# jhoobergs/Thesis-pbrt-v3

Hardware: AMD Instinct MI355X
Metric: Mrays/s (higher is better)
Workload: dtype f32; 1 GPU; Sponza-class atrium STAND-IN (311,728 tris, matte+plastic, point light; the reference ships no Sponza geometry) 700x700, halton 1024 spp, path maxdepth 5, bvh; spp_total=1024, tiles=16x16 round-robin over 1 GPU(s), parallelism=tile-dp1, film_merge=none (single GPU)

## Files before the change

thesis-pbrt-v3_amd/csrc/capi_device.hip:

```cpp
#include <hip/hip_runtime.h>
#include <algorithm>
#include <cassert>
#include <chrono>
#include <cmath>
#include <cstring>
#include <functional>
#include <map>
#include <memory>
#include <string>
#include <vector>
#include "../../include/hprt.h"
#include "device/kernels.h"
#include "halton_tables.h"
#include "host_transform.h"
#include "hprt_internal.h"
#include "device_state.h"
#include "scene_layout.h"
#include "wide_bvh.h"

using namespace hprt;


namespace {

int CheckDevice(int device, int *chosen) {
    int n = 0;
    hipError_t e = hipGetDeviceCount(&n);
    if (e != hipSuccess || n <= 0) return SetError(HPRT_E_NO_DEVICE, "no HIP device available (hprt has no CPU fallback)");
    if (device < 0) { if (hipGetDevice(&device) != hipSuccess) device = 0; }
    if (device >= n) return SetError(HPRT_E_INVALID, "device ordinal out of range");
    if (hipSetDevice(device) != hipSuccess) return SetError(HPRT_E_DEVICE, "hipSetDevice failed");
    *chosen = device;
    return HPRT_OK;
}

struct PlaneAllocator {
    char *base; size_t off = 0, cap;
    template <typename T> T *take(size_t n) { off = (off + 255) & ~(size_t)255; T *p = (T *)(base + off); off += n * sizeof(T); return p; }
};
struct Workspace {
    PathStream path[2];
    HitStream hit;
    VertexStreams vs;
    float4 *Lfinal;
};
const size_t kPlaneBytesPerSlot = 16 * (2 * 4 + 1 + 2 + 2 + 1 + 3 + 1) + 1, kInstancePlaneBytesPerSlot = 8 + 8;
size_t PlaneBytesPerSlot(bool instances) { return kPlaneBytesPerSlot + (instances ? kInstancePlaneBytesPerSlot : 0); }
size_t PlaneBytes(size_t n, bool instances) { return n * PlaneBytesPerSlot(instances) + 32 * 256; }

void CarvePlanes(char *base, size_t n, bool instances, Workspace *w) {
    PlaneAllocator a{base, 0, 0};
    auto rays = [&](RayStream &r) { r.a = a.take<float4>(n); r.b = a.take<float4>(n); };
    for (int k = 0; k < 2; ++k) { rays(w->path[k].ray); w->path[k].beta = a.take<float4>(n); w->path[k].L = a.take<float4>(n); }
    w->hit.a = a.take<float4>(n); w->hit.b = instances ? a.take<float2>(n) : nullptr;
    rays(w->vs.shadow); w->vs.occluded = a.take<uint8_t>(n);
    rays(w->vs.mis); w->vs.misHit.a = a.take<float4>(n); w->vs.misHit.b = instances ? a.take<float2>(n) : nullptr;
    w->vs.pendLight = a.take<float4>(n); w->vs.pendMis = a.take<float4>(n); w->vs.pendBeta = a.take<float4>(n);
    w->Lfinal = a.take<float4>(n);
}

struct EventTimer {
    std::vector<hipEvent_t> pool; size_t used = 0;
    ~EventTimer() { for (hipEvent_t e : pool) (void)hipEventDestroy(e); }
    hipEvent_t get() {
        if (used == pool.size()) { hipEvent_t e; if (hipEventCreate(&e) != hipSuccess) return nullptr; pool.push_back(e); }
        return pool[used++];
    }
    void reset() { used = 0; }
};

void MakeCamera(const HprtRenderOptions &o, DevCamera *cam) {
    Xform camToScreen = xf_perspective(o.fov, 1e-2f, 1000.f);
    const float *sw = o.screen_window;
    Xform screenToRaster = xf_scale((float)o.xres, (float)o.yres, 1) * xf_scale(1 / (sw[1] - sw[0]), 1 / (sw[2] - sw[3]), 1) *
                           xf_translate(vec3(-sw[0], -sw[3], 0));
    Xform rasterToScreen = screenToRaster.inverse();
    Xform rasterToCamera = camToScreen.inverse() * rasterToScreen;
    cam->rasterToCamera = rasterToCamera.m;
    memcpy(cam->cameraToWorld.m, o.camera_to_world, 64);
    cam->lensRadius = o.lens_radius; cam->focalDistance = o.focal_distance;
    cam->dxCamera = xf_point(cam->rasterToCamera, vec3(1, 0, 0)) - xf_point(cam->rasterToCamera, vec3(0, 0, 0));
    cam->dyCamera = xf_point(cam->rasterToCamera, vec3(0, 1, 0)) - xf_point(cam->rasterToCamera, vec3(0, 0, 0));
}

int CheckDepth(int maxDepth) {
    if (5 + 8 * ((int64_t)maxDepth + 1) > 1000)
        return SetError(HPRT_E_UNSUPPORTED, "maxdepth above 123: a path could pass the 1,000 sampler dimensions of the reference's Halton tables");
    return HPRT_OK;
}

struct FrameSetup {
    FilmGeom fg; int ntx, nty; HaltonLayout hal; RenderParams rp;
    std::vector<uint32_t> pixelXY; std::vector<uint64_t> pixelOffset;
    std::vector<int32_t> localIndex;
    int W, H;
    uint64_t offX[128], offY[128];
};
int SetupFrame(const HprtRenderOptions &o, FrameSetup *f) {
    if (o.xres <= 0 || o.yres <= 0 || o.xres > 32768 || o.yres > 32768) return SetError(HPRT_E_INVALID, "film resolution out of range");
    if (o.filter_radius[0] != 0.5f || o.filter_radius[1] != 0.5f)
        return SetError(HPRT_E_UNSUPPORTED, "only the box filter with radius 0.5 is in the hot-path scope (SURVEY.md §2)");
    FilmGeom &fg = f->fg;
    fg.cx0 = (int)std::ceil(o.xres * o.crop[0]); fg.cx1 = (int)std::ceil(o.xres * o.crop[1]);
    fg.cy0 = (int)std::ceil(o.yres * o.crop[2]); fg.cy1 = (int)std::ceil(o.yres * o.crop[3]);
    fg.rx = o.filter_radius[0]; fg.ry = o.filter_radius[1];
    fg.sx0 = (int)std::floor((float)fg.cx0 + 0.5f - fg.rx); fg.sy0 = (int)std::floor((float)fg.cy0 + 0.5f - fg.ry);
    fg.sx1 = (int)std::ceil((float)fg.cx1 - 0.5f + fg.rx); fg.sy1 = (int)std::ceil((float)fg.cy1 - 0.5f + fg.ry);
    fg.maxSampleLuminance = o.max_sample_luminance;
    f->W = fg.cx1 - fg.cx0; f->H = fg.cy1 - fg.cy0;
    if (f->W <= 0 || f->H <= 0) return SetError(HPRT_E_INVALID, "empty crop window");
    f->ntx = (fg.sx1 - fg.sx0 + 15) / 16; f->nty = (fg.sy1 - fg.sy0 + 15) / 16;
    f->hal = MakeHaltonLayout(fg.sx1 - fg.sx0, fg.sy1 - fg.sy0);
    const uint64_t base = (uint64_t)HaltonPixelOffset(f->hal, 0, 0), stride = (uint64_t)std::max(1, f->hal.sampleStride);
    for (int m = 0; m < 128; ++m) {
        f->offX[m] = (uint64_t)HaltonPixelOffset(f->hal, m, 0);
        f->offY[m] = ((uint64_t)HaltonPixelOffset(f->hal, 0, m) + stride - base) % stride;
    }
    return HPRT_OK;
}
void AddTilePixels(FrameSetup *f, int tile) {
    const FilmGeom &fg = f->fg;
    int tx = tile % f->ntx, ty = tile / f->ntx;
    int x0 = fg.sx0 + tx * 16, x1 = std::min(x0 + 16, fg.sx1), y0 = fg.sy0 + ty * 16, y1 = std::min(y0 + 16, fg.sy1);
    const uint64_t stride = (uint64_t)std::max(1, f->hal.sampleStride);
    for (int y = y0; y < y1; ++y)
        for (int x = x0; x < x1; ++x) {
            f->localIndex[(size_t)(y - fg.cy0) * f->W + (x - fg.cx0)] = (int32_t)f->pixelXY.size();
            f->pixelXY.push_back((uint32_t)x | ((uint32_t)y << 16));
            f->pixelOffset.push_back(f->hal.sampleStride > 1 ? (f->offX[((x % 128) + 128) % 128] + f->offY[((y % 128) + 128) % 128]) % stride : 0ull);
        }
}

}

extern "C" {

int hprt_scene_create(const HprtSceneDesc *d, int device, HprtScene **out) try {
    if (!d || !out) return SetError(HPRT_E_INVALID, "hprt_scene_create: null argument");
    SceneLayout L;
    if (int rc = BuildSceneLayout(*d, &L)) return rc;
    int dev;
    if (int rc = CheckDevice(device, &dev)) return rc;
    std::unique_ptr<HprtScene> sc(new HprtScene());
    sc->device = dev; sc->nPrims = L.nPrims;
    sc->topOrder = std::move(L.topOrder); sc->objectOrder = std::move(L.objectOrder); sc->objectPrimBase = std::move(L.objectPrimBase);
    sc->instanceObject = std::move(L.instanceObject); sc->instanced = L.instanced; sc->hasSubstrateBin = L.hasSubstrateBin;
    const std::vector<uint16_t> &perms = HaltonPermutations();
    std::vector<int32_t> primes(PrimeTable().begin(), PrimeTable().end()), primeSums(PrimeSumTable().begin(), PrimeSumTable().end());
    std::vector<uint64_t> magic(primes.size());
    for (size_t i = 0; i < primes.size(); ++i) magic[i] = 0xffffffffffffffffull / (uint64_t)primes[i] + 1ull;
    HIP_TRY(upload(sc->nodes, L.pairs)); HIP_TRY(upload(sc->tris, L.tris)); HIP_TRY(upload(sc->primVtx, L.primVtx));
    HIP_TRY(upload(sc->primN, L.primN)); HIP_TRY(upload(sc->vUV, L.vUV)); HIP_TRY(upload(sc->vS, L.vS));
    HIP_TRY(upload(sc->shapes, L.shapes)); HIP_TRY(upload(sc->materials, L.materials)); HIP_TRY(upload(sc->lights, L.lights));
    HIP_TRY(upload(sc->spheres, L.spheres)); HIP_TRY(upload(sc->instances, L.instances)); HIP_TRY(upload(sc->topEntry, L.topEntry));
    HIP_TRY(upload(sc->topEntryWide, L.topEntryWide)); HIP_TRY(upload(sc->lightFunc, L.lightFunc)); HIP_TRY(upload(sc->lightCdf, L.lightCdf));
    HIP_TRY(upload(sc->perms, perms)); HIP_TRY(upload(sc->primes, primes)); HIP_TRY(upload(sc->primeSums, primeSums));
    HIP_TRY(upload(sc->primeMagic, magic));
    HIP_TRY(upload(sc->textures, L.textures)); HIP_TRY(upload(sc->mipLevels, L.mipLevels)); HIP_TRY(upload(sc->texels, L.texels)); HIP_TRY(upload(sc->weightLut, L.weightLut));
    HIP_TRY(upload(sc->wide, L.wide)); HIP_TRY(upload(sc->leafBox, L.leafBox));
    HIP_TRY(upload(sc->envLights, L.envLights)); HIP_TRY(upload(sc->envData, L.envData));
    HIP_TRY(sc->counters.alloc(sizeof(DevCounters)));
    HIP_TRY(hipMemset(sc->counters.p, 0, sizeof(DevCounters)));
    HIP_TRY(sc->deepStack.alloc((size_t)HPRT_SPILL_STACK * HPRT_DEEP_THREADS * sizeof(uint2)));
    HIP_TRY(sc->workCounter.alloc(256));
    DevScene &dv = sc->dev;
    dv.pairs = sc->nodes.as<DevPair>(); dv.nPairs = (uint32_t)L.pairs.size();
    dv.wide = L.wide.empty() ? nullptr : sc->wide.as<DevWide>(); dv.nWide = (uint32_t)L.wide.size(); dv.leafBox = sc->leafBox.as<float4>();
    dv.tris = sc->tris.as<float4>(); dv.nPrims = L.nPrims;
    dv.primVtx = sc->primVtx.as<uint32_t>();
    dv.primN = sc->primN.as<float4>(); dv.vUV = sc->vUV.as<float>(); dv.vS = sc->vS.as<float>();
    dv.shapes = sc->shapes.as<DevShape>(); dv.nShapes = d->n_shapes;
    dv.materials = sc->materials.as<DevMaterial>();
    dv.lights = sc->lights.as<DevLight>(); dv.nLights = d->n_lights;
    dv.spheres = sc->spheres.as<DevSphere>(); dv.nSpheres = (uint32_t)L.spheres.size();
    dv.envLights = sc->envLights.as<DevEnvLight>(); dv.envData = sc->envData.as<float>(); dv.nEnvLights = (uint32_t)L.envLights.size();
    dv.textures = d->n_textures ? sc->textures.as<DevTexture>() : nullptr; dv.mipLevels = sc->mipLevels.as<DevMipLevel>();
    dv.texels = sc->texels.as<float>(); dv.weightLut = sc->weightLut.as<float>();
    dv.instances = sc->instances.as<DevInstance>(); dv.nInstances = d->n_instances;
    dv.topEntry = L.topEntry.empty() ? nullptr : sc->topEntry.as<float4>(); dv.nTopPrims = (uint32_t)L.topEntry.size();
    dv.topEntryWide = L.topEntryWide.empty() ? nullptr : sc->topEntryWide.as<float4>();
    dv.lightFunc = sc->lightFunc.as<float>(); dv.lightCdf = sc->lightCdf.as<float>(); dv.lightFuncInt = L.funcInt;
    dv.deepStack = sc->deepStack.as<uint2>();
    dv.perms = sc->perms.as<uint16_t>(); dv.primes = sc->primes.as<int32_t>(); dv.primeSums = sc->primeSums.as<int32_t>();
    dv.primeMagic = sc->primeMagic.as<uint64_t>();
    dv.worldRadius = L.worldRadius;
    dv.spatial = 0; dv.voxFunc = dv.voxCdf = dv.voxFuncInt = nullptr;
    dv.voxSlot = nullptr; dv.voxRequest = nullptr; dv.voxRequestCount = nullptr;
    for (int a = 0; a < 3; ++a) { dv.voxN[a] = L.voxN[a]; dv.wbMin[a] = L.wbMin[a]; dv.wbMax[a] = L.wbMax[a]; }
    if (L.lightStrategy == 2) {
        const uint64_t nVox = (uint64_t)dv.voxN[0] * (uint64_t)dv.voxN[1] * (uint64_t)dv.voxN[2];
        const uint64_t denseMaxFloats = [] { const char *e = getenv("HPRT_VOXEL_DENSE_MAX_MB"); return e ? (uint64_t)atoll(e) * (1ull << 18) : (1ull << 28); }();
        const uint64_t rowFloats = 2ull * d->n_lights + 2ull;
        const bool dense = nVox * rowFloats <= denseMaxFloats;
        uint64_t rows = nVox;
        if (!dense) {
            const uint64_t poolFloats = [] { const char *e = getenv("HPRT_VOXEL_POOL_MB"); return (e ? (uint64_t)atoll(e) : 4096ull) * (1ull << 18); }();
            rows = std::max<uint64_t>(1, std::min<uint64_t>(nVox, poolFloats / rowFloats));
        }
        HIP_TRY(sc->voxFunc.alloc(rows * d->n_lights * sizeof(float)));
        HIP_TRY(sc->voxCdf.alloc(rows * (d->n_lights + 1ull) * sizeof(float)));
        HIP_TRY(sc->voxFuncInt.alloc(rows * sizeof(float)));
        std::vector<float> ri(5 * 128);
        VoxelSamplePoints(ri.data());
        HIP_TRY(upload(sc->voxRi, ri));
        dv.spatial = 1;
        dv.voxFunc = sc->voxFunc.as<float>(); dv.voxCdf = sc->voxCdf.as<float>(); dv.voxFuncInt = sc->voxFuncInt.as<float>();
        sc->nVoxels = (uint32_t)nVox; sc->voxRows = (uint32_t)rows; sc->voxRowsUsed = 0;
        if (dense) LaunchVoxelDistributions(nullptr, dv, sc->voxRi.as<float>(), (uint32_t)nVox, sc->voxFunc.as<float>(), sc->voxCdf.as<float>(), sc->voxFuncInt.as<float>());
        else {
            HIP_TRY(sc->voxSlot.alloc(nVox * sizeof(int32_t)));
            HIP_TRY(hipMemset(sc->voxSlot.p, 0xff, nVox * sizeof(int32_t)));
            HIP_TRY(sc->voxRequest.alloc(nVox * sizeof(uint32_t)));
            HIP_TRY(sc->voxRequestCount.alloc(256));
            HIP_TRY(hipMemset(sc->voxRequestCount.p, 0, 256));
            dv.voxSlot = sc->voxSlot.as<int32_t>(); dv.voxRequest = sc->voxRequest.as<uint32_t>(); dv.voxRequestCount = sc->voxRequestCount.as<uint32_t>();
        }
        HIP_TRY(hipGetLastError());
        HIP_TRY(hipDeviceSynchronize());
    }
    HIP_TRY(hipHostMalloc((void **)&sc->hostCounts, (4096 + 256) * sizeof(uint32_t)));
    *out = sc.release();
    return HPRT_OK;
} catch (...) { return hprt::HandleException(); }

__attribute__((visibility("default"))) int hprt_debug_scene_walk(HprtScene *s) { return s && s->walk == HprtScene::Walk::Bvh && hprt::WideWalkInUse(s->dev) ? 1 : 0; }
__attribute__((visibility("default"))) int hprt_debug_shade_counts(HprtScene *s, int on, uint64_t *out2) {
    if (!s) return HPRT_E_INVALID;
    if (out2) { out2[0] = s->shadeDeferred; out2[1] = s->shadeRetried; }
    if (on && !s->shadeCountsOn) s->shadeDeferred = s->shadeRetried = s->shadeSpeculated = s->shadeRepaired = s->shadeFull = 0;
    s->shadeCountsOn = on != 0;
    return HPRT_OK;
}
__attribute__((visibility("default"))) int hprt_debug_speculated_counts(HprtScene *s, uint64_t *out3) {
    if (!s || !out3) return HPRT_E_INVALID;
    out3[0] = s->shadeSpeculated; out3[1] = s->shadeRepaired; out3[2] = s->shadeFull;
    return HPRT_OK;
}
static int g_speculateLight = -1;
static bool SpeculateLightEnabled() {
    static const bool fromEnv = [] { const char *e = getenv("HPRT_SPECULATE_LIGHT"); return !(e && atoi(e) == 0); }();
    return g_speculateLight < 0 ? fromEnv : g_speculateLight != 0;
}
__attribute__((visibility("default"))) int hprt_debug_speculate_light(int on) { const int was = SpeculateLightEnabled() ? 1 : 0; g_speculateLight = on; return was; }
__attribute__((visibility("default"))) int hprt_debug_poison_workspace(HprtScene *s, int byte) { if (!s) return HPRT_E_INVALID; s->poisonByte = byte < 0 ? -1 : (byte & 255); return HPRT_OK; }
__attribute__((visibility("default"))) int hprt_debug_capture_rays(HprtScene *s, int bounce, int kind, float *d_out7, size_t cap) {
    if (!s || kind < 0 || kind > 2 || cap > 0x7fffffffull) return HPRT_E_INVALID;
    s->capture.bounce = bounce; s->capture.kind = kind; s->capture.out7 = d_out7; s->capture.cap = cap; s->capture.n = 0;
    return HPRT_OK;
}
static int ApiStreams(HprtScene *s, size_t n, RayStream *rays, HitStream *hits);
static bool CountsKdShare(const HprtScene *s) {
    return s->walk == HprtScene::Walk::RbspKd || s->walk == HprtScene::Walk::BspPaperKd || s->walk == HprtScene::Walk::RbspKdInst ||
           s->walk == HprtScene::Walk::BspPaperKdInst;
}
static void Trace(HprtScene *s, hipStream_t st, bool anyHit, bool count, const uint32_t *queue, const uint32_t *countPtr, uint32_t countImm,
                  uint32_t gridItems, const RayStream &rays, const HitStream &hits, uint8_t *occ, DevCounters *counters, uint32_t *workCounter,
                  uint4 *rayStats = nullptr) {
    switch (s->walk) {
    case HprtScene::Walk::Kd: LaunchKdTrace(st, s->dev, s->kd, anyHit, count, queue, countPtr, countImm, gridItems, rays, hits, occ, counters, workCounter, rayStats); break;
    case HprtScene::Walk::Rbsp: LaunchRbspTrace(st, s->dev, s->rbsp, anyHit, count, queue, countPtr, countImm, gridItems, rays, hits, occ, counters, workCounter, rayStats); break;
    case HprtScene::Walk::RbspKd:
        LaunchRbspKdTrace(st, s->dev, DevRbspKd{s->rbsp, s->kdShare.as<unsigned long long>()}, anyHit, count, queue, countPtr, countImm, gridItems, rays,
                          hits, occ, counters, workCounter, rayStats);
        break;
    case HprtScene::Walk::BspPaper:
        LaunchBspPaperTrace(st, s->dev, s->bsppaper, anyHit, count, queue, countPtr, countImm, gridItems, rays, hits, occ, counters, workCounter, rayStats);
        break;
    case HprtScene::Walk::BspPaperKd:
        LaunchBspPaperKdTrace(st, s->dev, DevBspPaperKd{s->bsppaper, s->kdShare.as<unsigned long long>()}, anyHit, count, queue, countPtr, countImm,
                              gridItems, rays, hits, occ, counters, workCounter, rayStats);
        break;
    case HprtScene::Walk::KdInst:
        LaunchKdInstTrace(st, s->dev, s->kdinst, anyHit, count, queue, countPtr, countImm, gridItems, rays, hits, occ, counters, workCounter, rayStats);
        break;
    case HprtScene::Walk::RbspInst:
    case HprtScene::Walk::RbspKdInst:
        LaunchRbspInstTrace(st, s->dev, s->rbspinst, s->walk == HprtScene::Walk::RbspKdInst, anyHit, count, queue, countPtr, countImm, gridItems, rays, hits, occ,
                            counters, workCounter, rayStats);
        break;
    case HprtScene::Walk::BspPaperInst:
    case HprtScene::Walk::BspPaperKdInst:
        LaunchBspPaperInstTrace(st, s->dev, s->bsppaperinst, s->walk == HprtScene::Walk::BspPaperKdInst, anyHit, count, queue, countPtr, countImm, gridItems, rays,
                                hits, occ, counters, workCounter, rayStats);
        break;
    case HprtScene::Walk::Bvh: LaunchTrace(st, s->dev, anyHit, count, queue, countPtr, countImm, gridItems, rays, hits, occ, counters, workCounter, rayStats); break;
    }
}
__attribute__((visibility("default"))) int hprt_debug_trace_queued(HprtScene *s, size_t n, const float *d_rays7, const uint32_t *d_queue, int anyHit,
                                                                    float *d_scratch7, float ms[2]) try {
    if (!s || !d_rays7 || !d_queue || !d_scratch7 || !ms || n == 0 || n > 0x7ffffff0ull) return SetError(HPRT_E_INVALID, "hprt_debug_trace_queued: bad argument");
    HIP_TRY(hipSetDevice(s->device));
    SceneCall call(s, nullptr);
    RayStream rays; HitStream hits;
    if (int rc = ApiStreams(s, n, &rays, &hits)) return rc;
    DevBuf occ; HIP_TRY(occ.alloc(n));
    hipEvent_t e[3];
    for (auto &x : e) HIP_TRY(hipEventCreate(&x));
    LaunchPackRays(nullptr, d_rays7, (uint32_t)n, rays);
    HIP_TRY(hipEventRecord(e[0], nullptr));
    LaunchCaptureRays(nullptr, d_queue, (uint32_t)n, rays, d_scratch7, (uint32_t)n);
    HIP_TRY(hipEventRecord(e[1], nullptr));
    HitStream none; none.a = nullptr; none.b = nullptr;
    Trace(s, nullptr, anyHit != 0, false, d_queue, nullptr, (uint32_t)n, (uint32_t)n, rays, anyHit ? none : hits, anyHit ? occ.as<uint8_t>() : nullptr, nullptr, s->workCounter.as<uint32_t>());
    HIP_TRY(hipEventRecord(e[2], nullptr));
    HIP_TRY(hipDeviceSynchronize());
    HIP_TRY(hipEventElapsedTime(&ms[0], e[0], e[1])); HIP_TRY(hipEventElapsedTime(&ms[1], e[1], e[2]));
    for (auto &x : e) (void)hipEventDestroy(x);
    return HPRT_OK;
} catch (...) { return hprt::HandleException(); }
__attribute__((visibility("default"))) long long hprt_debug_captured(HprtScene *s) { return s ? (long long)s->capture.n : -1; }
__attribute__((visibility("default"))) int hprt_debug_stream_copy(int device, size_t bytes, int iters, double *best_gbs, double *mean_gbs) try {
    if (!best_gbs || !mean_gbs || iters < 1 || iters > 1000 || bytes < (1u << 20) || bytes > (64ull << 30)) return SetError(HPRT_E_INVALID, "hprt_debug_stream_copy: bad argument");
    int dev = 0;
    if (int rc = CheckDevice(device, &dev)) return rc;
    HIP_TRY(hipSetDevice(dev));
    DevBuf a, b;
    HIP_TRY(a.alloc(bytes)); HIP_TRY(b.alloc(bytes));
    HIP_TRY(hipMemset(a.p, 1, bytes)); HIP_TRY(hipMemset(b.p, 2, bytes));
    const size_t n = bytes / 16;
    hipEvent_t e0, e1;
    HIP_TRY(hipEventCreate(&e0)); HIP_TRY(hipEventCreate(&e1));
    LaunchStreamCopy(nullptr, a.as<float4>(), b.as<float4>(), n);
    HIP_TRY(hipDeviceSynchronize());
    double best = 0, sum = 0;
    for (int i = 0; i < iters; ++i) {
        HIP_TRY(hipEventRecord(e0, nullptr));
        LaunchStreamCopy(nullptr, a.as<float4>(), b.as<float4>(), n);
        HIP_TRY(hipEventRecord(e1, nullptr));
        HIP_TRY(hipEventSynchronize(e1));
        float ms = 0; HIP_TRY(hipEventElapsedTime(&ms, e0, e1));
        const double g = 2.0 * (double)(n * 16) / ((double)ms * 1e-3) / 1e9;
        best = std::max(best, g); sum += g;
    }
    (void)hipEventDestroy(e0); (void)hipEventDestroy(e1);
    *best_gbs = best; *mean_gbs = sum / iters;
    return HPRT_OK;
} catch (...) { return hprt::HandleException(); }
__attribute__((visibility("default"))) int hprt_debug_gather_probe(int device, int log2_records, int iters_per_lane, int launches, double *best_grecords_s, double *mean_grecords_s) try {
    if (!best_grecords_s || !mean_grecords_s || log2_records < 8 || log2_records > 26 || iters_per_lane < 1 || iters_per_lane > 100000 || launches < 1 || launches > 100)
        return SetError(HPRT_E_INVALID, "hprt_debug_gather_probe: bad argument");
    int dev = 0;
    if (int rc = CheckDevice(device, &dev)) return rc;
    HIP_TRY(hipSetDevice(dev));
    hipDeviceProp_t prop;
    HIP_TRY(hipGetDeviceProperties(&prop, dev));
    const uint32_t blocks = (uint32_t)prop.multiProcessorCount * 6u * 4u;
    DevBuf table, sink;
    const size_t bytes = (size_t)64 << log2_records;
    HIP_TRY(table.alloc(bytes)); HIP_TRY(sink.alloc(16));
    HIP_TRY(hipMemset(table.p, 0x5b, bytes));
    hipEvent_t e0, e1;
    HIP_TRY(hipEventCreate(&e0)); HIP_TRY(hipEventCreate(&e1));
    LaunchGatherProbe(nullptr, table.as<uint4>(), (uint32_t)log2_records, std::max(1, iters_per_lane / 10), blocks, sink.as<uint32_t>());
    HIP_TRY(hipDeviceSynchronize());
    double best = 0, sum = 0;
    for (int i = 0; i < launches; ++i) {
        HIP_TRY(hipEventRecord(e0, nullptr));
        LaunchGatherProbe(nullptr, table.as<uint4>(), (uint32_t)log2_records, iters_per_lane, blocks, sink.as<uint32_t>());
        HIP_TRY(hipEventRecord(e1, nullptr));
        HIP_TRY(hipEventSynchronize(e1));
        float ms = 0; HIP_TRY(hipEventElapsedTime(&ms, e0, e1));
        const double g = (double)blocks * 256.0 * (double)iters_per_lane / ((double)ms * 1e-3) / 1e9;
        best = std::max(best, g); sum += g;
    }
    (void)hipEventDestroy(e0); (void)hipEventDestroy(e1);
    *best_grecords_s = best; *mean_grecords_s = sum / launches;
    return HPRT_OK;
} catch (...) { return hprt::HandleException(); }

__global__ void k_debug_math(int fn, const float *x, const float *y, size_t n, double *o0, double *o1) {
    const size_t i = (size_t)blockIdx.x * blockDim.x + threadIdx.x;
    if (i >= n) return;
    double a = 0, b = 0;
    if (fn == 0) { float s, c; det_sincosf(x[i], &s, &c); a = (double)s; b = (double)c; }
    else if (fn == 1) a = (double)det_acosf(x[i]);
    else if (fn == 2) a = (double)det_atan2f(y[i], x[i]);
    else if (fn == 3) a = (double)det_logf(x[i]);
    else det_sincos_glibc_d((double)x[i], &a, &b);
    o0[i] = a; o1[i] = b;
}
__attribute__((visibility("default"))) int hprt_debug_device_math(int device, int fn, const float *x, const float *y, size_t n, double *out0, double *out1) try {
    if (fn < 0 || fn > 4 || !x || !y || !out0 || !out1 || n == 0 || n > ((size_t)1 << 28)) return SetError(HPRT_E_INVALID, "hprt_debug_device_math: bad argument");
    HIP_TRY(hipSetDevice(device));
    float *dx = nullptr, *dy = nullptr; double *d0 = nullptr, *d1 = nullptr;
    auto release = [&]() { (void)hipFree(dx); (void)hipFree(dy); (void)hipFree(d0); (void)hipFree(d1); };
    hipError_t e = hipMalloc((void **)&dx, n * 4);
    if (e == hipSuccess) e = hipMalloc((void **)&dy, n * 4);
    if (e == hipSuccess) e = hipMalloc((void **)&d0, n * 8);
    if (e == hipSuccess) e = hipMalloc((void **)&d1, n * 8);
    if (e == hipSuccess) e = hipMemcpy(dx, x, n * 4, hipMemcpyHostToDevice);
    if (e == hipSuccess) e = hipMemcpy(dy, y, n * 4, hipMemcpyHostToDevice);
    if (e == hipSuccess) {
        k_debug_math<<<dim3((unsigned)((n + 255) / 256)), dim3(256)>>>(fn, dx, dy, n, d0, d1);
        e = hipGetLastError();
    }
    if (e == hipSuccess) e = hipMemcpy(out0, d0, n * 8, hipMemcpyDeviceToHost);
// ... 245 lines not shown
    auto sameLayout = [kd](const BspPaperTree &b) {
        return b.kdAware == kd ? std::string() : std::string(b.kdAware ? "its tree holds BSPKdNode's flags, the handle is not kd-aware" : "its tree holds BSPNode's flags, the handle is kd-aware");
    };
    if (t->top.kdAware != kd) return SetError(HPRT_E_INVALID, "the top-level tree's node layout is not the handle's");
    const TwoLevelView<BspPaperTree> view{kd ? "bsppaperkd tree" : "bsppaper tree", *t, kd ? CheckBspPaperKdTree : CheckBspPaperTree,
                                          kd ? (uint32_t)BSPPAPERKD_OFF : (uint32_t)BSPPAPER_OFF, kd ? (uint32_t)BSPPAPERKD_MASK : (uint32_t)BSPPAPER_MASK,
                                          kd ? (uint32_t)BSPPAPERKD_LEAF : 1u, kd ? (uint32_t)BSPPAPERKD_TODO_MAX : (uint32_t)BSPPAPER_TODO_MAX, sameLayout,
                                          [](const BspPaperTree &b) -> const std::vector<float> & { return b.axes; }};
    DevBspPaperInst &d = s->bsppaperinst;
    if (int rc = AttachTwoLevel(s, view, d)) return rc;
    if (kd)
        if (int rc = ResetKdShare(s)) return rc;
    d.axes = s->treeAxes.as<float4>();
    d.kdCounters = kd ? s->kdShare.as<unsigned long long>() : nullptr;
    s->walk = kd ? HprtScene::Walk::BspPaperKdInst : HprtScene::Walk::BspPaperInst;
    return HPRT_OK;
} catch (...) { return hprt::HandleException(); }

int hprt_scene_kd_counters(HprtScene *s, uint64_t out[2]) try {
    if (!s || !out) return SetError(HPRT_E_INVALID, "hprt_scene_kd_counters: null argument");
    HIP_TRY(hipSetDevice(s->device));
    SceneCall call(s, nullptr);
    out[0] = out[1] = 0;
    if (!CountsKdShare(s)) return HPRT_OK;
    unsigned long long c[2];
    HIP_TRY(hipMemcpy(c, s->kdShare.p, sizeof(c), hipMemcpyDeviceToHost));
    out[0] = c[0]; out[1] = c[1];
    return HPRT_OK;
} catch (...) { return hprt::HandleException(); }

void hprt_scene_destroy(HprtScene *s) {
    if (!s) return;
    (void)hipSetDevice(s->device);
    delete s;
}

static void ReadCounters(HprtScene *s, bool anyHit, uint64_t out[4]) {
    DevCounters c;
    (void)hipMemcpy(&c, s->counters.p, sizeof(c), hipMemcpyDeviceToHost);
    if (!anyHit) { out[0] = c.nodesFetched; out[1] = c.nodesEntered; out[2] = c.triTests; out[3] = c.sphereTests; }
    else { out[0] = c.nodesFetchedP; out[1] = c.nodesEnteredP; out[2] = c.triTestsP; out[3] = c.sphereTestsP; }
}
static int ApiStreams(HprtScene *s, size_t n, RayStream *rays, HitStream *hits) {
    HIP_TRY(s->apiRays.alloc(32 * n + 256));
    HIP_TRY(s->apiHits.alloc(24 * n + 256));
    rays->a = s->apiRays.as<float4>(); rays->b = rays->a + n;
    hits->a = s->apiHits.as<float4>(); hits->b = (float2 *)(hits->a + n);
    return HPRT_OK;
}

int hprt_intersect_device(HprtScene *s, size_t n, const float *d_rays7, float *d_t, int32_t *d_prim, float *d_bary3, void *stream) try {
    if (!s || (n && (!d_rays7 || !d_t || !d_prim))) return SetError(HPRT_E_INVALID, "hprt_intersect_device: null argument");
    if (n > 0x7ffffff0ull) return SetError(HPRT_E_INVALID, "too many rays in one call");
    if (n == 0) return HPRT_OK;
    HIP_TRY(hipSetDevice(s->device));
    hipStream_t st = (hipStream_t)stream;
    SceneCall call(s, st);
    RayStream rays; HitStream hits;
    int rc = ApiStreams(s, n, &rays, &hits);
    if (rc != HPRT_OK) return rc;
    LaunchPackRays(st, d_rays7, (uint32_t)n, rays);
    Trace(s, st, false, false, nullptr, nullptr, (uint32_t)n, (uint32_t)n, rays, hits, nullptr, nullptr, s->workCounter.as<uint32_t>());
    LaunchUnpackHits(st, hits, (uint32_t)n, d_t, d_prim, d_bary3);
    call.leave_async();
    HIP_TRY(hipGetLastError());
    return HPRT_OK;
} catch (...) { return hprt::HandleException(); }
int hprt_occluded_device(HprtScene *s, size_t n, const float *d_rays7, uint8_t *d_occ, void *stream) try {
    if (!s || (n && (!d_rays7 || !d_occ))) return SetError(HPRT_E_INVALID, "hprt_occluded_device: null argument");
    if (n > 0x7ffffff0ull) return SetError(HPRT_E_INVALID, "too many rays in one call");
    if (n == 0) return HPRT_OK;
    HIP_TRY(hipSetDevice(s->device));
    hipStream_t st = (hipStream_t)stream;
    SceneCall call(s, st);
    RayStream rays; HitStream hits;
    int rc = ApiStreams(s, n, &rays, &hits);
    if (rc != HPRT_OK) return rc;
    LaunchPackRays(st, d_rays7, (uint32_t)n, rays);
    HitStream none; none.a = nullptr; none.b = nullptr;
    Trace(s, st, true, false, nullptr, nullptr, (uint32_t)n, (uint32_t)n, rays, none, d_occ, nullptr, s->workCounter.as<uint32_t>());
    call.leave_async();
    HIP_TRY(hipGetLastError());
    return HPRT_OK;
} catch (...) { return hprt::HandleException(); }


static int TraceHost(HprtScene *s, bool anyHit, size_t n, const float *o, const float *d, const float *tmax, float *t_out,
                     int32_t *prim_out, int32_t *inst_out, float *bary_out, uint8_t *occ_out, uint64_t counters[4]) {
    if (!s || (n && (!o || !d || !tmax))) return SetError(HPRT_E_INVALID, "trace: null argument");
    if (n > 0x7ffffff0ull) return SetError(HPRT_E_INVALID, "too many rays in one call");
    if (n == 0) { if (counters) memset(counters, 0, 32); return HPRT_OK; }
    HIP_TRY(hipSetDevice(s->device));
    SceneCall call(s, nullptr);
    std::vector<float4> ra(n), rb(n);
    for (size_t i = 0; i < n; ++i) {
        ra[i] = make_float4(o[3 * i], o[3 * i + 1], o[3 * i + 2], tmax[i]);
        rb[i] = make_float4(d[3 * i], d[3 * i + 1], d[3 * i + 2], 0.f);
    }
    RayStream rays; HitStream hits;
    int rc = ApiStreams(s, n, &rays, &hits);
    if (rc != HPRT_OK) return rc;
    HIP_TRY(hipMemcpy(rays.a, ra.data(), 16 * n, hipMemcpyHostToDevice));
    HIP_TRY(hipMemcpy(rays.b, rb.data(), 16 * n, hipMemcpyHostToDevice));
    HIP_TRY(hipMemset(s->counters.p, 0, sizeof(DevCounters)));
    if (CountsKdShare(s)) HIP_TRY(hipMemset(s->kdShare.p, 0, 2 * sizeof(unsigned long long)));
    const bool count = counters != nullptr;
    if (!anyHit) {
        Trace(s, nullptr, false, count, nullptr, nullptr, (uint32_t)n, (uint32_t)n, rays, hits, nullptr, s->counters.as<DevCounters>(), s->workCounter.as<uint32_t>());
        HIP_TRY(hipGetLastError()); HIP_TRY(hipDeviceSynchronize());
        std::vector<float4> ha(n); std::vector<float2> hb(n);
        HIP_TRY(hipMemcpy(ha.data(), hits.a, 16 * n, hipMemcpyDeviceToHost));
        HIP_TRY(hipMemcpy(hb.data(), hits.b, 8 * n, hipMemcpyDeviceToHost));
        for (size_t i = 0; i < n; ++i) {
            if (t_out) t_out[i] = hit_t(hb[i]);
            if (prim_out) prim_out[i] = hit_prim(hit_word(ha[i]));
            if (inst_out) inst_out[i] = hit_inst(hb[i]);
            if (bary_out) { bary_out[3 * i] = hit_b0(ha[i]); bary_out[3 * i + 1] = hit_b1(ha[i]); bary_out[3 * i + 2] = hit_b2(ha[i]); }
        }
    } else {
        DevBuf outOcc;
        HIP_TRY(outOcc.alloc(n));
        HitStream none; none.a = nullptr; none.b = nullptr;
        Trace(s, nullptr, true, count, nullptr, nullptr, (uint32_t)n, (uint32_t)n, rays, none, outOcc.as<uint8_t>(), s->counters.as<DevCounters>(), s->workCounter.as<uint32_t>());
        HIP_TRY(hipGetLastError()); HIP_TRY(hipDeviceSynchronize());
        if (occ_out) HIP_TRY(hipMemcpy(occ_out, outOcc.p, n, hipMemcpyDeviceToHost));
    }
    if (counters) ReadCounters(s, anyHit, counters);
    return HPRT_OK;
}
int hprt_intersect(HprtScene *s, size_t n, const float *o, const float *d, const float *tmax, float *t_out, int32_t *prim_out,
                   float *bary_out, uint64_t counters[4]) try {
    return TraceHost(s, false, n, o, d, tmax, t_out, prim_out, nullptr, bary_out, nullptr, counters);
} catch (...) { return hprt::HandleException(); }
int hprt_intersect_instanced(HprtScene *s, size_t n, const float *o, const float *d, const float *tmax, float *t_out, int32_t *prim_out,
                             int32_t *inst_out, float *bary_out, uint64_t counters[4]) try {
    return TraceHost(s, false, n, o, d, tmax, t_out, prim_out, inst_out, bary_out, nullptr, counters);
} catch (...) { return hprt::HandleException(); }
int hprt_occluded(HprtScene *s, size_t n, const float *o, const float *d, const float *tmax, uint8_t *occ, uint64_t counters[4]) try {
    return TraceHost(s, true, n, o, d, tmax, nullptr, nullptr, nullptr, nullptr, occ, counters);
} catch (...) { return hprt::HandleException(); }

namespace {

constexpr size_t kSpecCountsAt = 1024;
struct BatchTimers { double extendMs = 0, occludedMs = 0; uint64_t extendLaunches = 0, occludedLaunches = 0, extendRays = 0, occludedRays = 0; };

int RunBatch(HprtScene *s, hipStream_t st, const RenderParams &rpIn, const Workspace &w, const QueueSet &qa, const QueueSet &qb,
             const BinSet &bins, uint32_t s0, uint32_t nSlots, bool count, EventTimer &ev, BatchTimers *bt, HprtRenderStats *stats,
             uint32_t *pixelStats = nullptr, const IrregularSink *irregular = nullptr) {
    uint4 *rayStats = pixelStats ? s->rayStats.as<uint4>() : nullptr;
    RenderParams rp = rpIn;
    rp.speculate = SpeculateLightEnabled() && !pixelStats && !rayStats && nSlots <= SPEC_MAX_PATHS ? 1 : 0;
    assert(!rp.speculate || nSlots <= SPEC_MAX_PATHS);
    uint32_t *specCounts = rp.speculate && s->shadeCountsOn ? s->queueCounts.as<uint32_t>() + kSpecCountsAt : nullptr;
    if (specCounts) HIP_TRY(hipMemsetAsync(specCounts, 0, 2 * sizeof(uint32_t), st));
    uint32_t *pixelKd = pixelStats && CountsKdShare(s) ? s->pixelKdLocal.as<uint32_t>() : nullptr;
    uint32_t *wcPath = s->workCounter.as<uint32_t>();
    LaunchGenerate(st, s->dev, rp, w.path[0], s0, nSlots, irregular);
    const uint32_t *activeQ = nullptr; uint32_t active = nSlots;
    QueueSet q[2] = {qa, qb};
    DevCounters *ctr = s->counters.as<DevCounters>();
    std::vector<std::pair<hipEvent_t, hipEvent_t>> evExt, evOcc;
    auto tracePath = [&](int bounce) -> int {
        const PathStream &in = w.path[bounce & 1];
        hipEvent_t e0 = ev.get(), e1 = ev.get();
        HIP_TRY(hipEventRecord(e0, st));
        Trace(s, st, false, count, activeQ, nullptr, active, active, in.ray, w.hit, nullptr, ctr, wcPath, rayStats);
        if (pixelStats) LaunchPixelStats(st, rayStats, bounce == 0 ? nullptr : in.beta, activeQ, nullptr, active, active, rp.nPix, false, pixelStats);
        if (pixelKd) LaunchPixelKdStats(st, rayStats, bounce == 0 ? nullptr : in.beta, activeQ, nullptr, active, active, rp.nPix, false, pixelKd);
        HIP_TRY(hipEventRecord(e1, st));
        evExt.push_back({e0, e1}); bt->extendRays += active; ++bt->extendLaunches;
        stats->rays += active;
        return HPRT_OK;
    };
    if (active > 0) { int rc = tracePath(0); if (rc != HPRT_OK) return rc; }
    for (int bounce = 0; active > 0; ++bounce) {
        const QueueSet &cur = q[bounce & 1];
        const PathStream &in = w.path[bounce & 1], &out = w.path[(bounce + 1) & 1];
        HIP_TRY(hipMemsetAsync(cur.nextCount, 0, 256 * sizeof(uint32_t), st));
        HIP_TRY(hipMemsetAsync(bins.count, 0, 8 * BIN_STRIDE * sizeof(uint32_t), st));
        LaunchBin(st, s->dev, in, w.hit, activeQ, nullptr, active, active, rp.maxDepth, bounce, bins, w.Lfinal);
        HIP_TRY(hipMemcpyAsync(bins.count + 5 * BIN_STRIDE, bins.count + 2 * BIN_STRIDE, sizeof(uint32_t), hipMemcpyDeviceToDevice, st));
        static const int order[5] = {BIN_MATTE, BIN_PLASTIC, BIN_SUBSTRATE, BIN_GENERIC, BIN_TEXTURED};
        for (int k = 0; k < (s->dev.textures ? 5 : 4); ++k) {
            const int mode = order[k];
            if (mode == (int)BIN_SUBSTRATE && !s->hasSubstrateBin) continue;
            LaunchShade(st, mode, s->dev, rp, in, w.hit, active, s0, out, w.vs, cur, bins, w.Lfinal, bounce == 0);
        }
        HIP_TRY(hipMemcpyAsync(s->hostCounts + 4096, cur.nextCount, 256 * sizeof(uint32_t), hipMemcpyDeviceToHost, st));
        if (s->shadeCountsOn) {
            HIP_TRY(hipMemcpyAsync(s->hostCounts + 12, bins.count + 2 * BIN_STRIDE, sizeof(uint32_t), hipMemcpyDeviceToHost, st));
            HIP_TRY(hipMemcpyAsync(s->hostCounts + 13, bins.count + 5 * BIN_STRIDE, sizeof(uint32_t), hipMemcpyDeviceToHost, st));
        }
        if (s->dev.voxSlot) {
            HIP_TRY(hipMemcpyAsync(s->hostCounts + 16, bins.count + 6 * BIN_STRIDE, 2 * BIN_STRIDE * sizeof(uint32_t), hipMemcpyDeviceToHost, st));
            HIP_TRY(hipMemcpyAsync(s->hostCounts + 15, s->dev.voxRequestCount, sizeof(uint32_t), hipMemcpyDeviceToHost, st));
            HIP_TRY(hipStreamSynchronize(st));
            const uint32_t nRetry[2] = {s->hostCounts[16], s->hostCounts[16 + BIN_STRIDE]}, nReq = s->hostCounts[15];
            if (s->shadeCountsOn) s->shadeRetried += (uint64_t)nRetry[0] + nRetry[1];
            if (nRetry[0] + nRetry[1] > 0) {
                if ((uint64_t)s->voxRowsUsed + nReq > s->voxRows)
                    return SetError(HPRT_E_UNSUPPORTED, "spatial light distribution: the paths touch more voxels than the row pool holds (" + std::to_string(s->voxRows) +
                                                        " rows of " + std::to_string(s->dev.nLights) + " lights; HPRT_VOXEL_POOL_MB raises it, or use \"power\" / \"uniform\")");
                LaunchVoxelFill(st, s->dev, s->voxRi.as<float>(), nReq, s->voxRowsUsed, s->voxFunc.as<float>(), s->voxCdf.as<float>(), s->voxFuncInt.as<float>());
                s->voxRowsUsed += nReq;
                HIP_TRY(hipMemsetAsync(s->dev.voxRequestCount, 0, sizeof(uint32_t), st));
                for (int r = 0; r < 2; ++r)
                    if (nRetry[r]) LaunchShade(st, 2 + r, s->dev, rp, in, w.hit, nRetry[r], s0, out, w.vs, cur, bins, w.Lfinal, bounce == 0, true);
                HIP_TRY(hipMemcpyAsync(s->hostCounts + 4096, cur.nextCount, 256 * sizeof(uint32_t), hipMemcpyDeviceToHost, st));
            }
        }
        HIP_TRY(hipStreamSynchronize(st));
        if (s->shadeCountsOn) s->shadeDeferred += s->hostCounts[12] - s->hostCounts[13];
        const uint32_t nNext = s->hostCounts[4096], nShadow = s->hostCounts[4096 + 64], nMis = s->hostCounts[4096 + 128], nResolve = s->hostCounts[4096 + 192];
        if (s->capture.out7 && s->capture.bounce == bounce && s0 == 0) {
            const uint32_t *cq = s->capture.kind == 0 ? cur.next : s->capture.kind == 1 ? cur.shadow : cur.mis;
            const uint32_t cn = s->capture.kind == 0 ? nNext : s->capture.kind == 1 ? nShadow : nMis;
            const RayStream &cs = s->capture.kind == 0 ? out.ray : s->capture.kind == 1 ? w.vs.shadow : w.vs.mis;
            LaunchCaptureRays(st, cq, cn, cs, s->capture.out7, (uint32_t)s->capture.cap);
            s->capture.n = std::min<size_t>(cn, s->capture.cap);
        }
        if (nShadow) {
            hipEvent_t a = ev.get(), b = ev.get();
            HIP_TRY(hipEventRecord(a, st));
            HitStream none; none.a = nullptr; none.b = nullptr;
            Trace(s, st, true, count, cur.shadow, nullptr, nShadow, nShadow, w.vs.shadow, none, w.vs.occluded, ctr, wcPath, rayStats);
            if (pixelStats) LaunchPixelStats(st, rayStats, w.vs.pendBeta, cur.shadow, nullptr, nShadow, nShadow, rp.nPix, true, pixelStats);
            if (pixelKd) LaunchPixelKdStats(st, rayStats, w.vs.pendBeta, cur.shadow, nullptr, nShadow, nShadow, rp.nPix, true, pixelKd);
            HIP_TRY(hipEventRecord(b, st));
            evOcc.push_back({a, b}); bt->occludedRays += nShadow; ++bt->occludedLaunches;
            stats->shadow_rays += nShadow;
        }
        if (nMis) {
            hipEvent_t a = ev.get(), b = ev.get();
            HIP_TRY(hipEventRecord(a, st));
            Trace(s, st, false, count, cur.mis, nullptr, nMis, nMis, w.vs.mis, w.vs.misHit, nullptr, ctr, wcPath, rayStats);
            if (pixelStats) LaunchPixelStats(st, rayStats, w.vs.pendBeta, cur.mis, nullptr, nMis, nMis, rp.nPix, false, pixelStats);
            if (pixelKd) LaunchPixelKdStats(st, rayStats, w.vs.pendBeta, cur.mis, nullptr, nMis, nMis, rp.nPix, false, pixelKd);
            HIP_TRY(hipEventRecord(b, st));
            evExt.push_back({a, b}); bt->extendRays += nMis; ++bt->extendLaunches;
            stats->rays += nMis;
        }
        activeQ = cur.next; active = nNext;
        if (active > 0 && bounce > rp.maxDepth) return SetError(HPRT_E_DEVICE, "internal error: paths are still active beyond maxdepth");
        if (nResolve) LaunchResolve(st, s->dev, w.vs, out.L, w.Lfinal, cur.resolve, cur.resolveCount, nResolve);
        if (rp.speculate && nShadow) LaunchRepair(st, w.vs, out.L, w.Lfinal, cur.shadow, nShadow, specCounts);
        if (s->shadeCountsOn) s->shadeFull += nResolve;
        if (active > 0) { int rc = tracePath(bounce + 1); if (rc != HPRT_OK) return rc; }
    }
    HIP_TRY(hipGetLastError());
    if (specCounts) HIP_TRY(hipMemcpyAsync(s->hostCounts + 256, specCounts, 2 * sizeof(uint32_t), hipMemcpyDeviceToHost, st));
    HIP_TRY(hipStreamSynchronize(st));
    if (specCounts) { s->shadeSpeculated += s->hostCounts[256]; s->shadeRepaired += s->hostCounts[257]; }
    for (auto &p : evExt) { float ms = 0; if (hipEventElapsedTime(&ms, p.first, p.second) == hipSuccess) bt->extendMs += ms; }
    for (auto &p : evOcc) { float ms = 0; if (hipEventElapsedTime(&ms, p.first, p.second) == hipSuccess) bt->occludedMs += ms; }
    ev.reset();
    return HPRT_OK;
}

constexpr size_t kQueueWordsPerSlot = 8 + 1 + 2 * N_BINS;
int EnsureWorkspace(HprtScene *s, size_t nSlots, Workspace *ps, QueueSet *qa, QueueSet *qb, BinSet *bins) {
    const bool instances = s->dev.nInstances != 0u;
    HIP_TRY(s->planes.alloc(PlaneBytes(nSlots, instances)));
    CarvePlanes(s->planes.as<char>(), nSlots, instances, ps);
    HIP_TRY(s->queues.alloc(kQueueWordsPerSlot * nSlots * sizeof(uint32_t) + 4096));
    HIP_TRY(s->queueCounts.alloc(2048 * sizeof(uint32_t)));
    uint32_t *qbase = s->queues.as<uint32_t>(), *cbase = s->queueCounts.as<uint32_t>();
    QueueSet *qs[2] = {qa, qb};
    for (int k = 0; k < 2; ++k) {
        qs[k]->next = qbase + (4 * k + 0) * nSlots; qs[k]->shadow = qbase + (4 * k + 1) * nSlots;
        qs[k]->mis = qbase + (4 * k + 2) * nSlots; qs[k]->resolve = qbase + (4 * k + 3) * nSlots;
        qs[k]->nextCount = cbase + 256 * k; qs[k]->shadowCount = cbase + 256 * k + 64; qs[k]->misCount = cbase + 256 * k + 128; qs[k]->resolveCount = cbase + 256 * k + 192;
    }
    bins->aux = qbase + 8 * nSlots;
    for (int k = 0; k < (int)N_BINS; ++k) bins->q[k] = reinterpret_cast<uint2 *>(qbase + (9 + 2 * k) * nSlots + (nSlots & 1u));
    bins->count = cbase + 512;
    bins->retry[0] = bins->retry[1] = nullptr;
    if (s->dev.voxSlot) {
        HIP_TRY(s->retryQueues.alloc(2 * nSlots * sizeof(uint2) + 256));
        bins->retry[0] = s->retryQueues.as<uint2>(); bins->retry[1] = bins->retry[0] + nSlots;
    }
    return HPRT_OK;
}

int PoisonWorkspace(HprtScene *s) {
    if (s->poisonByte < 0) return HPRT_OK;
    hprt::DevBuf *bufs[] = {&s->planes, &s->queues, &s->Lall, &s->deepStack, &s->rayStats, &s->irregular};
    for (hprt::DevBuf *b : bufs) if (b->p && b->bytes) HIP_TRY(hipMemset(b->p, s->poisonByte, b->bytes));
    HIP_TRY(hipDeviceSynchronize());
    return HPRT_OK;
}

int ChooseBatch(HprtScene *s, int32_t sppChunk, uint32_t nPix, uint32_t spp, uint32_t *out) {
    uint32_t chunk;
    if (sppChunk > 0) chunk = (uint32_t)sppChunk;
    else {
        size_t freeB = 0, totalB = 0;
        HIP_TRY(hipMemGetInfo(&freeB, &totalB));
        freeB += s->planes.bytes + s->queues.bytes;
        const size_t perPath = PlaneBytesPerSlot(s->dev.nInstances != 0u) + kQueueWordsPerSlot * sizeof(uint32_t);
        static const size_t capM = [] { const char *e = getenv("HPRT_BATCH_MPATHS"); return e ? (size_t)atoi(e) : (size_t)256; }();
        const size_t budget = std::min<size_t>(capM << 20, std::max<size_t>(freeB / 2 / perPath, 1ull << 20));
        chunk = std::max<uint32_t>(1u, (uint32_t)(budget / std::max<uint32_t>(nPix, 1u)));
        if ((uint64_t)chunk * nPix > 0x7fffffffull) chunk = (uint32_t)(0x7fffffffull / nPix);
        chunk = std::max(1u, std::min(chunk, spp));
        const uint32_t nBatches = (spp + chunk - 1) / chunk;
        chunk = (spp + nBatches - 1) / nBatches;
    }
    chunk = std::min(chunk, spp);
    if ((uint64_t)chunk * nPix > 0x7fffffffull) chunk = (uint32_t)(0x7fffffffull / nPix);
    *out = chunk;
    return HPRT_OK;
}

struct ExtraEntry { uint32_t dest; uint32_t srcTile; uint32_t srcPos; uint32_t sample; uint32_t srcPix; uint8_t pre; };

}

int hprt_render(HprtScene *s, const HprtRenderDesc *desc, float *d_film_xyzw, void *stream, HprtRenderStats *stats) try {
    if (!s || !desc) return SetError(HPRT_E_INVALID, "hprt_render: null argument");
    HIP_TRY(hipSetDevice(s->device));
    hipStream_t st = (hipStream_t)stream;
    SceneCall call(s, st);
    const HprtRenderOptions &o = desc->opt;
    int rc0;
    if (o.spp <= 0 || o.max_depth < 0) return SetError(HPRT_E_INVALID, "spp must be positive and max_depth non-negative");
    if ((rc0 = CheckDepth(o.max_depth)) != HPRT_OK) return rc0;
    FrameSetup f;
    int rc = SetupFrame(o, &f);
    if (rc != HPRT_OK) return rc;
    HprtRenderStats localStats; if (!stats) stats = &localStats;
    memset(stats, 0, sizeof(*stats));
    const int nTiles = f.ntx * f.nty;
    int tb = std::max(0, desc->tile_begin), te = desc->tile_end <= 0 ? nTiles : std::min(desc->tile_end, nTiles), ts = std::max(1, desc->tile_stride);
    f.localIndex.assign((size_t)f.W * f.H, -1);
    f.pixelXY.reserve((size_t)f.W * f.H / (size_t)ts + 256); f.pixelOffset.reserve((size_t)f.W * f.H / (size_t)ts + 256);
    std::vector<uint8_t> tileIsLocal(nTiles, 0);
    for (int t = tb; t < te; t += ts) { tileIsLocal[t] = 1; AddTilePixels(&f, t); }
    const uint32_t nPix = (uint32_t)f.pixelXY.size();
    const uint32_t spp = (uint32_t)o.spp;
    s->filmPixels = (size_t)f.W * f.H;
    s->filmW = f.W; s->filmH = f.H;
    s->nForeignRecords = 0; s->foreignExported = (desc->flags & HPRT_RENDER_EXPORT_FOREIGN) != 0;
    float *film = d_film_xyzw;
    if (!film) { HIP_TRY(s->film.alloc(16 * s->filmPixels)); film = s->film.as<float>(); }
    s->lastFilm = film;
    HIP_TRY(hipMemsetAsync(film, 0, 16 * s->filmPixels, st));
    if (nPix == 0) { HIP_TRY(hipStreamSynchronize(st)); return HPRT_OK; }
    const size_t lallBytes = 3ull * spp * nPix * sizeof(float);
    if (lallBytes > (96ull << 30)) return SetError(HPRT_E_UNSUPPORTED, "per-sample radiance store would exceed 96 GiB; render in several tile ranges");
    uint32_t chunk = 0;
    if ((rc = ChooseBatch(s, desc->spp_chunk, nPix, spp, &chunk)) != HPRT_OK) return rc;
    const size_t maxSlots = (size_t)chunk * nPix;
    Workspace ps; QueueSet qa, qb; BinSet bins;
    rc = EnsureWorkspace(s, maxSlots, &ps, &qa, &qb, &bins);
    if (rc != HPRT_OK) return rc;
    HIP_TRY(s->Lall.alloc(lallBytes));
    if ((rc = PoisonWorkspace(s)) != HPRT_OK) return rc;
    float *LallR = s->Lall.as<float>(), *LallG = LallR + (size_t)spp * nPix, *LallB = LallG + (size_t)spp * nPix;
    HIP_TRY(upload(s->pixelXY, f.pixelXY)); HIP_TRY(upload(s->pixelOffset, f.pixelOffset));
    RenderParams rp;
    MakeCamera(o, &rp.cam);
    rp.hal.baseScale1 = f.hal.baseScales[1]; rp.hal.baseExp0 = f.hal.baseExponents[0]; rp.hal.sampleStride = f.hal.sampleStride;
    rp.hal.samplePixelCenter = o.sample_pixel_center;
    rp.pixelXY = s->pixelXY.as<uint32_t>(); rp.pixelOffset = s->pixelOffset.as<uint64_t>(); rp.nPix = nPix;
    rp.maxDepth = o.max_depth; rp.rrThreshold = o.rr_threshold;
    rp.invSqrtSpp = 1 / std::sqrt((float)spp);
    const bool wantPixelStats = (desc->flags & HPRT_RENDER_PIXEL_STATS) != 0;
    const bool count = (desc->flags & HPRT_RENDER_COUNT_WORK) != 0 || wantPixelStats;
    rp.speculate = 0;
    rp.cullMis = (!count || (desc->flags & HPRT_RENDER_COUNT_TRACED) != 0) && !(desc->flags & HPRT_RENDER_TRACE_ALL) ? 1 : 0;
    uint32_t *pixelStats = nullptr;
    if (wantPixelStats) {
        HIP_TRY(s->rayStats.alloc(sizeof(uint4) * maxSlots));
        HIP_TRY(s->pixelStatsLocal.alloc(6ull * nPix * sizeof(uint32_t)));
        HIP_TRY(hipMemsetAsync(s->pixelStatsLocal.p, 0, 6ull * nPix * sizeof(uint32_t), st));
        HIP_TRY(s->pixelStatsFilm.alloc(7ull * s->filmPixels * sizeof(uint64_t)));
        HIP_TRY(hipMemsetAsync(s->pixelStatsFilm.p, 0, 7ull * s->filmPixels * sizeof(uint64_t), st));
        pixelStats = s->pixelStatsLocal.as<uint32_t>();
        if (CountsKdShare(s)) {
            HIP_TRY(s->pixelKdLocal.alloc(2ull * nPix * sizeof(uint32_t)));
            HIP_TRY(hipMemsetAsync(s->pixelKdLocal.p, 0, 2ull * nPix * sizeof(uint32_t), st));
            HIP_TRY(s->pixelKdFilm.alloc(2ull * s->filmPixels * sizeof(uint64_t)));
            HIP_TRY(hipMemsetAsync(s->pixelKdFilm.p, 0, 2ull * s->filmPixels * sizeof(uint64_t), st));
        }
    }
    s->pixelStatsValid = false; s->pixelKdValid = false;
    HIP_TRY(hipMemsetAsync(s->counters.p, 0, sizeof(DevCounters), st));
    if (CountsKdShare(s)) HIP_TRY(hipMemsetAsync(s->kdShare.p, 0, 2 * sizeof(unsigned long long), st));

    auto wall0 = std::chrono::high_resolution_clock::now();
    static const uint32_t capHint = [] { const char *e = getenv("HPRT_IRREGULAR_CAP"); return e ? (uint32_t)std::max(1, atoi(e)) : (1u << 24); }();
    uint32_t irrCap = (uint32_t)std::min<uint64_t>((uint64_t)nPix * spp, capHint);
    HIP_TRY(s->irregularCount.alloc(16));
    HIP_TRY(s->irregular.alloc((size_t)irrCap * sizeof(IrregularSample)));
    HIP_TRY(hipMemsetAsync(s->irregularCount.p, 0, 16, st));
    const IrregularSink sink = {f.fg, s->irregularCount.as<uint32_t>(), irrCap, s->irregular.as<IrregularSample>()};
    EventTimer ev; BatchTimers bt;
    for (uint32_t s0 = 0; s0 < spp; s0 += chunk) {
        const uint32_t c = std::min(chunk, spp - s0), nSlots = c * nPix;
        rc = RunBatch(s, st, rp, ps, qa, qb, bins, s0, nSlots, count, ev, &bt, stats, pixelStats, &sink);
        if (rc != HPRT_OK) return rc;
        LaunchStoreRadiance(st, ps.Lfinal, LallR, LallG, LallB, nPix, s0, nSlots);
    }
    HIP_TRY(hipMemcpyAsync(s->hostCounts + 8, s->irregularCount.p, 4, hipMemcpyDeviceToHost, st));
    HIP_TRY(hipStreamSynchronize(st));
    uint32_t nIrr = s->hostCounts[8];
    if (nIrr > irrCap) {
        if ((uint64_t)nIrr * sizeof(IrregularSample) > (8ull << 30)) return SetError(HPRT_E_UNSUPPORTED, "too many irregular film samples");
        irrCap = nIrr;
        HIP_TRY(s->irregular.alloc((size_t)irrCap * sizeof(IrregularSample)));
        HIP_TRY(hipMemsetAsync(s->irregularCount.p, 0, 16, st));
        LaunchFindIrregular(st, s->dev, rp, f.fg, spp, s->irregularCount.as<uint32_t>(), irrCap, s->irregular.as<IrregularSample>());
        HIP_TRY(hipMemcpyAsync(s->hostCounts + 8, s->irregularCount.p, 4, hipMemcpyDeviceToHost, st));
        HIP_TRY(hipStreamSynchronize(st));
        if (s->hostCounts[8] != nIrr) return SetError(HPRT_E_DEVICE, "internal error: irregular film samples counted differently");
    }
    std::vector<IrregularSample> irr(nIrr);
    if (nIrr) HIP_TRY(hipMemcpy(irr.data(), s->irregular.p, (size_t)nIrr * sizeof(IrregularSample), hipMemcpyDeviceToHost));
    std::vector<ExtraEntry> own, foreign;
    for (const IrregularSample &r : irr) {
        const uint32_t pxy = f.pixelXY[r.pix];
        const int qx = (int)(pxy & 0xffffu), qy = (int)(pxy >> 16);
        const int qtx = (qx - f.fg.sx0) / 16, qty = (qy - f.fg.sy0) / 16;
        const uint32_t qTile = (uint32_t)(qty * f.ntx + qtx);
        const uint32_t qPos = (uint32_t)((qy - (f.fg.sy0 + qty * 16)) * 16 + (qx - (f.fg.sx0 + qtx * 16)));
        for (int y = r.y0; y < r.y1; ++y)
            for (int x = r.x0; x < r.x1; ++x) {
                if (x == qx && y == qy) continue;
                const int dtx = (x - f.fg.sx0) / 16, dty = (y - f.fg.sy0) / 16;
                const uint32_t filmIdx = (uint32_t)((size_t)(y - f.fg.cy0) * f.W + (x - f.fg.cx0));
                ExtraEntry e; e.srcTile = qTile; e.srcPos = qPos; e.sample = r.sample; e.srcPix = r.pix;
                if (dtx == qtx && dty == qty) {
                    e.dest = (uint32_t)f.localIndex[filmIdx];
                    e.pre = (qy < y || (qy == y && qx < x)) ? 1 : 0;
                    own.push_back(e);
                } else { e.dest = filmIdx; e.pre = 0; foreign.push_back(e); }
            }
    }
    std::sort(own.begin(), own.end(), [](const ExtraEntry &a, const ExtraEntry &b) {
        if (a.dest != b.dest) return a.dest < b.dest;
        if (a.srcPos != b.srcPos) return a.srcPos < b.srcPos;
        return a.sample < b.sample;
    });
    std::sort(foreign.begin(), foreign.end(), [](const ExtraEntry &a, const ExtraEntry &b) {
        if (a.dest != b.dest) return a.dest < b.dest;
        if (a.srcTile != b.srcTile) return a.srcTile < b.srcTile;
        if (a.srcPos != b.srcPos) return a.srcPos < b.srcPos;
        return a.sample < b.sample;
    });
    FilmExtras ex; memset(&ex, 0, sizeof(ex));
    std::vector<uint32_t> groupDest, groupTile;
    {
        std::vector<uint32_t> begin(nPix + 1, 0), src(own.size()), smp(own.size()); std::vector<uint8_t> pre(own.size());
        for (const ExtraEntry &e : own) ++begin[e.dest + 1];
        for (uint32_t i = 0; i < nPix; ++i) begin[i + 1] += begin[i];
        for (size_t i = 0; i < own.size(); ++i) { src[i] = own[i].srcPix; smp[i] = own[i].sample; pre[i] = own[i].pre; }
        HIP_TRY(upload(s->exOwnBegin, begin)); HIP_TRY(upload(s->exOwnSrc, src)); HIP_TRY(upload(s->exOwnSample, smp)); HIP_TRY(upload(s->exOwnPre, pre));
        ex.ownBegin = s->exOwnBegin.as<uint32_t>(); ex.ownSrcPix = s->exOwnSrc.as<uint32_t>(); ex.ownSample = s->exOwnSample.as<uint32_t>(); ex.ownIsPre = s->exOwnPre.as<uint8_t>();
        std::vector<uint32_t> dest, destBegin, groupBegin, fsrc(foreign.size()), fsmp(foreign.size());
        for (size_t i = 0; i < foreign.size(); ++i) {
            const bool newDest = i == 0 || foreign[i].dest != foreign[i - 1].dest;
            const bool newGroup = newDest || foreign[i].srcTile != foreign[i - 1].srcTile;
            if (newDest) { dest.push_back(foreign[i].dest); destBegin.push_back((uint32_t)groupBegin.size()); }
            if (newGroup) { groupBegin.push_back((uint32_t)i); groupDest.push_back(foreign[i].dest); groupTile.push_back(foreign[i].srcTile); }
            fsrc[i] = foreign[i].srcPix; fsmp[i] = foreign[i].sample;
        }
        destBegin.push_back((uint32_t)groupBegin.size()); groupBegin.push_back((uint32_t)foreign.size());
        HIP_TRY(upload(s->exFDest, dest)); HIP_TRY(upload(s->exFDestBegin, destBegin)); HIP_TRY(upload(s->exFGroupBegin, groupBegin));
        HIP_TRY(upload(s->exFSrc, fsrc)); HIP_TRY(upload(s->exFSample, fsmp));
        ex.nForeignDest = (uint32_t)dest.size();
        ex.foreignDestFilmIndex = s->exFDest.as<uint32_t>(); ex.foreignDestBegin = s->exFDestBegin.as<uint32_t>(); ex.foreignGroupBegin = s->exFGroupBegin.as<uint32_t>();
        ex.foreignSrcPix = s->exFSrc.as<uint32_t>(); ex.foreignSample = s->exFSample.as<uint32_t>();
    }
    LaunchFilmOwn(st, rp, f.fg, LallR, LallG, LallB, spp, ex, film);
    if (desc->flags & HPRT_RENDER_EXPORT_FOREIGN) {
        const uint32_t nGroups = (uint32_t)groupDest.size();
        HIP_TRY(upload(s->exGroupDest, groupDest)); HIP_TRY(upload(s->exGroupTile, groupTile));
        HIP_TRY(s->foreignRecords.alloc(std::max<size_t>(1, nGroups) * sizeof(FilmRecord)));
        LaunchFilmForeignExport(st, rp, f.fg, LallR, LallG, LallB, ex, nGroups, s->exGroupDest.as<uint32_t>(), s->exGroupTile.as<uint32_t>(),
                                s->foreignRecords.as<FilmRecord>());
        s->nForeignRecords = nGroups;
    } else
        LaunchFilmForeign(st, rp, f.fg, LallR, LallG, LallB, ex, film);
    if (pixelStats) {
        LaunchPixelStatsToFilm(st, pixelStats, rp.pixelXY, nPix, spp, f.fg.cx0, f.fg.cy0, f.W, s->pixelStatsFilm.as<unsigned long long>());
        s->pixelStatsValid = true;
        if (CountsKdShare(s)) {
            LaunchPixelKdStatsToFilm(st, s->pixelKdLocal.as<uint32_t>(), rp.pixelXY, nPix, f.fg.cx0, f.fg.cy0, f.W, s->filmPixels,
                                     s->pixelKdFilm.as<unsigned long long>());
            s->pixelKdValid = true;
        }
    }
    HIP_TRY(hipGetLastError());
    HIP_TRY(hipStreamSynchronize(st));
    stats->render_seconds = std::chrono::duration<double>(std::chrono::high_resolution_clock::now() - wall0).count();
    stats->camera_rays = (uint64_t)nPix * spp;
    stats->extend_seconds = bt.extendMs * 1e-3; stats->occluded_seconds = bt.occludedMs * 1e-3;
    stats->extend_launches = bt.extendLaunches; stats->occluded_launches = bt.occludedLaunches;
    stats->extend_rays = bt.extendRays; stats->occluded_rays = bt.occludedRays;
    if (count) {
        DevCounters c;
        HIP_TRY(hipMemcpy(&c, s->counters.p, sizeof(c), hipMemcpyDeviceToHost));
        stats->nodes_fetched = c.nodesFetched; stats->nodes_entered = c.nodesEntered; stats->tri_tests = c.triTests; stats->sphere_tests = c.sphereTests;
        stats->nodes_fetched_p = c.nodesFetchedP; stats->nodes_entered_p = c.nodesEnteredP; stats->tri_tests_p = c.triTestsP; stats->sphere_tests_p = c.sphereTestsP;
    }
    return HPRT_OK;
} catch (...) { return hprt::HandleException(); }

int hprt_scene_reserve(HprtScene *s, const HprtRenderDesc *desc) try {
    if (!s || !desc) return SetError(HPRT_E_INVALID, "hprt_scene_reserve: null argument");
    const HprtRenderOptions &o = desc->opt;
    if (o.spp <= 0 || o.max_depth < 0) return SetError(HPRT_E_INVALID, "spp must be positive and max_depth non-negative");
    HIP_TRY(hipSetDevice(s->device));
    SceneCall call(s, nullptr);
    FrameSetup f;
    int rc = SetupFrame(o, &f);
    if (rc != HPRT_OK) return rc;
    const int nTiles = f.ntx * f.nty;
    const int tb = std::max(0, desc->tile_begin), te = desc->tile_end <= 0 ? nTiles : std::min(desc->tile_end, nTiles), ts = std::max(1, desc->tile_stride);
    uint64_t nPix64 = 0;
    for (int t = tb; t < te; t += ts) {
        const int tx = t % f.ntx, ty = t / f.ntx;
        const int x0 = f.fg.sx0 + tx * 16, x1 = std::min(x0 + 16, f.fg.sx1), y0 = f.fg.sy0 + ty * 16, y1 = std::min(y0 + 16, f.fg.sy1);
        nPix64 += (uint64_t)(x1 - x0) * (uint64_t)(y1 - y0);
    }
    if (nPix64 == 0) return HPRT_OK;
    const uint32_t nPix = (uint32_t)nPix64, spp = (uint32_t)o.spp;
    const size_t lallBytes = 3ull * spp * nPix * sizeof(float);
    if (lallBytes > (96ull << 30)) return SetError(HPRT_E_UNSUPPORTED, "per-sample radiance store would exceed 96 GiB; render in several tile ranges");
    uint32_t chunk = 0;
    if ((rc = ChooseBatch(s, desc->spp_chunk, nPix, spp, &chunk)) != HPRT_OK) return rc;
    Workspace ps; QueueSet qa, qb; BinSet bins;
    if ((rc = EnsureWorkspace(s, (size_t)chunk * nPix, &ps, &qa, &qb, &bins)) != HPRT_OK) return rc;
    HIP_TRY(s->Lall.alloc(lallBytes));
    HIP_TRY(s->pixelXY.alloc((size_t)nPix * sizeof(uint32_t))); HIP_TRY(s->pixelOffset.alloc((size_t)nPix * sizeof(uint64_t)));
    HIP_TRY(hipDeviceSynchronize());
    return HPRT_OK;
} catch (...) { return hprt::HandleException(); }

int hprt_pixel_stats_read(HprtScene *s, uint64_t *out7, size_t n_pixels) try {
    if (!s || !out7) return SetError(HPRT_E_INVALID, "hprt_pixel_stats_read: null argument");
    SceneCall call(s, nullptr);
    if (!s->pixelStatsValid) return SetError(HPRT_E_INVALID, "no per-pixel statistics: render with HPRT_RENDER_PIXEL_STATS first");
    if (n_pixels != s->filmPixels) return SetError(HPRT_E_INVALID, "hprt_pixel_stats_read: pixel count differs from the last render's film");
    HIP_TRY(hipSetDevice(s->device));
    HIP_TRY(hipMemcpy(out7, s->pixelStatsFilm.p, 7 * n_pixels * sizeof(uint64_t), hipMemcpyDeviceToHost));
    return HPRT_OK;
} catch (...) { return hprt::HandleException(); }
int hprt_pixel_kd_stats_read(HprtScene *s, uint64_t *out2, size_t n_pixels) try {
    if (!s || !out2) return SetError(HPRT_E_INVALID, "hprt_pixel_kd_stats_read: null argument");
    SceneCall call(s, nullptr);
    if (!s->pixelKdValid && (s->walk == HprtScene::Walk::RbspInst || s->walk == HprtScene::Walk::BspPaperInst) && s->pixelStatsValid) {
        if (n_pixels != s->filmPixels) return SetError(HPRT_E_INVALID, "hprt_pixel_kd_stats_read: pixel count differs from the last render's film");
        memset(out2, 0, 2 * n_pixels * sizeof(uint64_t));
        return HPRT_OK;
    }
    if (!s->pixelKdValid) return SetError(HPRT_E_INVALID, "no per-pixel kd statistics: render an rbspkd or bsppaperkd scene with HPRT_RENDER_PIXEL_STATS first");
    if (n_pixels != s->filmPixels) return SetError(HPRT_E_INVALID, "hprt_pixel_kd_stats_read: pixel count differs from the last render's film");
    HIP_TRY(hipSetDevice(s->device));
    HIP_TRY(hipMemcpy(out2, s->pixelKdFilm.p, 2 * n_pixels * sizeof(uint64_t), hipMemcpyDeviceToHost));
    return HPRT_OK;
} catch (...) { return hprt::HandleException(); }
int hprt_film_read(HprtScene *s, float *xyzw_out, size_t n_pixels) try {
    if (!s || !xyzw_out) return SetError(HPRT_E_INVALID, "hprt_film_read: null argument");
    SceneCall call(s, nullptr);
    if (!s->film.p || s->lastFilm != s->film.as<float>() || n_pixels != s->filmPixels)
        return SetError(HPRT_E_INVALID, "hprt_film_read: the last render did not write a library-owned film of that size (render with d_film_xyzw == NULL first)");
    HIP_TRY(hipSetDevice(s->device));
    HIP_TRY(hipMemcpy(xyzw_out, s->film.p, 16 * n_pixels, hipMemcpyDeviceToHost));
    return HPRT_OK;
} catch (...) { return hprt::HandleException(); }

int hprt_sample_radiance(HprtScene *s, const HprtRenderOptions *opt, size_t n, const int32_t *px, const int32_t *py, const int64_t *sample,
                         float *L_out) try {
    if (!s || !opt || (n && (!px || !py || !sample || !L_out))) return SetError(HPRT_E_INVALID, "hprt_sample_radiance: null argument");
    if (n == 0) return HPRT_OK;
    if (n > (1u << 26)) return SetError(HPRT_E_INVALID, "hprt_sample_radiance: too many samples in one call");
    if (opt->max_depth < 0) return SetError(HPRT_E_INVALID, "max_depth must be non-negative");
    if (int rcd = CheckDepth(opt->max_depth)) return rcd;
    HIP_TRY(hipSetDevice(s->device));
    SceneCall call(s, nullptr);
    FrameSetup f;
    int rc = SetupFrame(*opt, &f);
    if (rc != HPRT_OK) return rc;
    std::vector<uint32_t> xy(n); std::vector<uint64_t> off(n);
    for (size_t i = 0; i < n; ++i) {
        if (px[i] < f.fg.sx0 || px[i] >= f.fg.sx1 || py[i] < f.fg.sy0 || py[i] >= f.fg.sy1 || sample[i] < 0)
            return SetError(HPRT_E_INVALID, "hprt_sample_radiance: pixel outside the sample bounds");
        xy[i] = (uint32_t)px[i] | ((uint32_t)py[i] << 16);
        off[i] = (uint64_t)HaltonPixelOffset(f.hal, px[i], py[i]) + (uint64_t)sample[i] * (uint64_t)f.hal.sampleStride;
    }
    Workspace ps; QueueSet qa, qb; BinSet bins;
    rc = EnsureWorkspace(s, n, &ps, &qa, &qb, &bins);
    if (rc != HPRT_OK) return rc;
    HIP_TRY(upload(s->pixelXY, xy)); HIP_TRY(upload(s->pixelOffset, off));
    HIP_TRY(s->Lall.alloc(12 * n));
    if ((rc = PoisonWorkspace(s)) != HPRT_OK) return rc;
    RenderParams rp;
    MakeCamera(*opt, &rp.cam);
    rp.hal.baseScale1 = f.hal.baseScales[1]; rp.hal.baseExp0 = f.hal.baseExponents[0]; rp.hal.sampleStride = f.hal.sampleStride;
    rp.hal.samplePixelCenter = opt->sample_pixel_center;
    rp.pixelXY = s->pixelXY.as<uint32_t>(); rp.pixelOffset = s->pixelOffset.as<uint64_t>(); rp.nPix = (uint32_t)n;
    rp.maxDepth = opt->max_depth; rp.rrThreshold = opt->rr_threshold;
    rp.invSqrtSpp = 1 / std::sqrt((float)std::max(1, opt->spp)); rp.cullMis = 1; rp.speculate = 0;
    EventTimer ev; BatchTimers bt; HprtRenderStats stats; memset(&stats, 0, sizeof(stats));
    rc = RunBatch(s, nullptr, rp, ps, qa, qb, bins, 0, (uint32_t)n, false, ev, &bt, &stats);
    if (rc != HPRT_OK) return rc;
    float *LR = s->Lall.as<float>();
    LaunchStoreRadiance(nullptr, ps.Lfinal, LR, LR + n, LR + 2 * n, (uint32_t)n, 0, (uint32_t)n);
    HIP_TRY(hipGetLastError()); HIP_TRY(hipDeviceSynchronize());
    std::vector<float> planes(3 * n);
    HIP_TRY(hipMemcpy(planes.data(), LR, 12 * n, hipMemcpyDeviceToHost));
    for (size_t i = 0; i < n; ++i) { L_out[3 * i] = planes[i]; L_out[3 * i + 1] = planes[n + i]; L_out[3 * i + 2] = planes[2 * n + i]; }
    return HPRT_OK;
} catch (...) { return hprt::HandleException(); }

}
```

thesis-pbrt-v3_amd/csrc/device/kernels.h:

```cpp
#pragma once
#include <hip/hip_runtime.h>
#include <algorithm>
#include <type_traits>
#include "dev_shading.h"

namespace hprt {

struct RayStream { float4 *a, *b; };
struct HitStream { float4 *a; float2 *b; };
__device__ __forceinline__ void hit_store(const HitStream &h, uint32_t slot, int32_t word, float b0, float b1, float b2, float t, int32_t inst) {
    h.a[slot] = make_float4(b0, b1, b2, __int_as_float(word));
    if (h.b) h.b[slot] = make_float2(t, __int_as_float(inst));
}
__device__ __forceinline__ void hit_store_miss(const HitStream &h, uint32_t slot, float tMax) { hit_store(h, slot, -1, 0.f, 0.f, 0.f, tMax, -1); }
__device__ __forceinline__ float4 hit_load(const HitStream &h, uint32_t slot) { return h.a[slot]; }
__device__ __forceinline__ float2 hit_load_aux(const HitStream &h, uint32_t slot) { return h.b[slot]; }
__device__ __forceinline__ float2 hit_no_aux() { return make_float2(0.f, __int_as_float(-1)); }
__host__ __device__ __forceinline__ int32_t hit_word(const float4 &rec) { return __builtin_bit_cast(int32_t, rec.w); }
__host__ __device__ __forceinline__ float hit_b0(const float4 &rec) { return rec.x; }
__host__ __device__ __forceinline__ float hit_b1(const float4 &rec) { return rec.y; }
__host__ __device__ __forceinline__ float hit_b2(const float4 &rec) { return rec.z; }
__host__ __device__ __forceinline__ float hit_t(const float2 &aux) { return aux.x; }
__host__ __device__ __forceinline__ int32_t hit_inst(const float2 &aux) { return __builtin_bit_cast(int32_t, aux.y); }
struct PathStream {
    RayStream ray;
    float4 *beta;
    float4 *L;
};
struct VertexStreams {
    RayStream shadow; uint8_t *occluded;
    RayStream mis; HitStream misHit;
    float4 *pendLight;
    float4 *pendMis;
    float4 *pendBeta;
};
enum : uint32_t { SPEC_RECORD = 0x80000000u, SPEC_END = 0x40000000u, SPEC_ID_MASK = 0x0fffffffu, SPEC_MAX_PATHS = 1u << 28 };
struct QueueSet {
    uint32_t *next, *shadow, *mis, *resolve;
    uint32_t *nextCount, *shadowCount, *misCount, *resolveCount;
};
enum : uint32_t { BIN_STRIDE = 64u };
struct BinSet { uint2 *q[5]; uint32_t *aux; uint32_t *count; uint2 *retry[2]; };
struct RenderParams {
    DevCamera cam;
    DevHalton hal;
    const uint32_t *pixelXY;
    const uint64_t *pixelOffset;
    uint32_t nPix;
    int32_t maxDepth;
    float rrThreshold;
    float invSqrtSpp;
    int32_t cullMis;
    int32_t speculate;
};
struct FilmGeom {
    int32_t cx0, cy0, cx1, cy1;
    int32_t sx0, sy0, sx1, sy1;
    float rx, ry;
    float maxSampleLuminance;
};
struct IrregularSample { uint32_t pix, sample; int16_t x0, x1, y0, y1; };
struct IrregularSink { FilmGeom fg; uint32_t *count; uint32_t capacity; IrregularSample *out; };
struct FilmExtras {
    const uint32_t *ownBegin; const uint32_t *ownSrcPix; const uint32_t *ownSample; const uint8_t *ownIsPre;
    uint32_t nForeignDest;
    const uint32_t *foreignDestFilmIndex; const uint32_t *foreignDestBegin; const uint32_t *foreignGroupBegin;
    const uint32_t *foreignSrcPix; const uint32_t *foreignSample;
};

struct FilmRecord { uint32_t dest, srcTile; float xyz[3]; float w; };

bool WideWalkInUse(const DevScene &sc);
void LaunchTrace(hipStream_t st, const DevScene &sc, bool anyHit, bool count, const uint32_t *queue, const uint32_t *countPtr,
                 uint32_t countImm, uint32_t gridItems, const RayStream &rays, const HitStream &hits, uint8_t *occ,
                 DevCounters *counters, uint32_t *workCounter, uint4 *rayStats = nullptr);
template <uint32_t BLOCK, uint32_t WAVES, uint32_t QUAD_WAVES, typename Launch>
void LaunchTreeWalk(hipStream_t st, const DevScene &sc, bool anyHit, bool count, uint32_t gridItems, uint32_t *workCounter, Launch launch) {
    if (gridItems == 0) return;
    (void)hipMemsetAsync(workCounter, 0, sizeof(uint32_t), st);
    const bool quad = sc.nSpheres != 0u;
    const dim3 grid(std::min((uint32_t)(((size_t)gridItems + BLOCK - 1) / BLOCK), 256u * (quad ? QUAD_WAVES : WAVES))), block(BLOCK);
    auto pickQuad = [&](auto a, auto c) { if (quad) launch(grid, block, a, c, std::true_type{}); else launch(grid, block, a, c, std::false_type{}); };
    auto pickCount = [&](auto a) { if (count) pickQuad(a, std::true_type{}); else pickQuad(a, std::false_type{}); };
    if (anyHit) pickCount(std::true_type{}); else pickCount(std::false_type{});
}
void LaunchPixelStats(hipStream_t st, const uint4 *rayStats, const float4 *ids, const uint32_t *queue, const uint32_t *countPtr,
                      uint32_t countImm, uint32_t gridItems, uint32_t nPix, bool anyHit, uint32_t *pix);
void LaunchPixelStatsToFilm(hipStream_t st, const uint32_t *pix, const uint32_t *pixelXY, uint32_t nPix, uint32_t spp, int cx0, int cy0, int width,
                            unsigned long long *out7);
void LaunchGenerate(hipStream_t st, const DevScene &sc, const RenderParams &rp, const PathStream &out, uint32_t s0, uint32_t nSlots,
                    const IrregularSink *irr = nullptr);
void LaunchBin(hipStream_t st, const DevScene &sc, const PathStream &in, const HitStream &hit, const uint32_t *queue,
               const uint32_t *countPtr, uint32_t countImm, uint32_t gridItems, int32_t maxDepth, int32_t bounces, const BinSet &bins,
               float4 *Lfinal);
void LaunchShade(hipStream_t st, int mode, const DevScene &sc, const RenderParams &rp, const PathStream &in, const HitStream &hit,
                 uint32_t gridItems, uint32_t s0, const PathStream &out, const VertexStreams &vs, const QueueSet &q,
                 const BinSet &bins, float4 *Lfinal, bool firstBounce, bool retryPass = false);
void LaunchResolve(hipStream_t st, const DevScene &sc, const VertexStreams &vs, float4 *L, float4 *Lfinal, const uint32_t *queue,
                   const uint32_t *countPtr, uint32_t gridItems);
void LaunchRepair(hipStream_t st, const VertexStreams &vs, float4 *L, float4 *Lfinal, const uint32_t *queue, uint32_t n, uint32_t *counts);
void LaunchStoreRadiance(hipStream_t st, const float4 *Lfinal, float *LallR, float *LallG, float *LallB, uint32_t nPix, uint32_t s0,
                         uint32_t nSlots);
void LaunchPackRays(hipStream_t st, const float *rays7, uint32_t n, const RayStream &out);
void LaunchUnpackHits(hipStream_t st, const HitStream &hits, uint32_t n, float *t, int32_t *prim, float *bary3);
void LaunchFindIrregular(hipStream_t st, const DevScene &sc, const RenderParams &rp, const FilmGeom &fg, uint32_t spp, uint32_t *count,
                         uint32_t capacity, IrregularSample *out);
void LaunchFilmOwn(hipStream_t st, const RenderParams &rp, const FilmGeom &fg, const float *LallR, const float *LallG, const float *LallB,
                   uint32_t spp, const FilmExtras &ex, float *film);
void LaunchFilmForeign(hipStream_t st, const RenderParams &rp, const FilmGeom &fg, const float *LallR, const float *LallG,
                       const float *LallB, const FilmExtras &ex, float *film);
void LaunchFilmForeignExport(hipStream_t st, const RenderParams &rp, const FilmGeom &fg, const float *LallR, const float *LallG,
                             const float *LallB, const FilmExtras &ex, uint32_t nGroups, const uint32_t *groupDest, const uint32_t *groupTile,
                             FilmRecord *out);
void LaunchVoxelDistributions(hipStream_t st, const DevScene &sc, const float *ri, uint32_t nVox, float *func, float *cdf, float *funcInt);
void LaunchVoxelFill(hipStream_t st, const DevScene &sc, const float *ri, uint32_t n, uint32_t rowBase, float *func, float *cdf, float *funcInt);
void LaunchStreamCopy(hipStream_t st, const float4 *src, float4 *dst, size_t n);
void LaunchGatherProbe(hipStream_t st, const uint4 *records, uint32_t log2Records, int itersPerLane, uint32_t blocks, uint32_t *sink);
void LaunchCaptureRays(hipStream_t st, const uint32_t *queue, uint32_t n, const RayStream &rays, float *out7, uint32_t cap);
void LaunchFilmApplyRecords(hipStream_t st, const FilmRecord *rec, const uint32_t *destBegin, uint32_t nDest, float *film);

}
```

thesis-pbrt-v3_amd/csrc/device/kernels.hip:

```cpp
#include <hip/hip_runtime.h>
#include <algorithm>
#include <cstdio>
#include <cstdlib>
#include <string>
#include "dev_shading.h"
#include "kernels.h"
#ifndef HPRT_QUAD_ANY_WAVES
#define HPRT_QUAD_ANY_WAVES 5
#endif
#define HPRT_QUAD_CLOSEST_WAVES 4
#ifndef HPRT_LDS_STACK_QUAD_ANY
#define HPRT_LDS_STACK_QUAD_ANY 12
#endif
#define HPRT_LDS_STACK_INST_ANY 7
#define HPRT_LDS_STACK_INST_CLOSEST 9
#ifndef HPRT_ANY_WAVES
#define HPRT_ANY_WAVES 7
#endif
#ifndef HPRT_CLOSEST_WAVES
#define HPRT_CLOSEST_WAVES 6
#endif
#ifndef HPRT_LDS_STACK_CLOSEST
#define HPRT_LDS_STACK_CLOSEST 12
#endif

namespace hprt {

typedef unsigned int u32x4 __attribute__((ext_vector_type(4)));
typedef unsigned int u32x2 __attribute__((ext_vector_type(2)));
typedef float f32x2 __attribute__((ext_vector_type(2)));

__device__ __forceinline__ uint32_t wave_append(uint32_t *counter, bool pred) {
    const unsigned long long mask = __ballot(pred);
    if (mask == 0ull) return 0u;
    const uint32_t lane = __lane_id();
    const uint32_t prefix = __builtin_amdgcn_mbcnt_hi((uint32_t)(mask >> 32), __builtin_amdgcn_mbcnt_lo((uint32_t)mask, 0u));
    const int leader = __ffsll((long long)mask) - 1;
    uint32_t base = 0u;
    if ((int)lane == leader) base = atomicAdd(counter, (uint32_t)__popcll(mask));
    base = __shfl(base, leader);
    return base + prefix;
}

struct BlockAppendLds { uint32_t waveCount[4][16]; uint32_t base[4]; };
template <int NQ>
__device__ __forceinline__ void block_append(BlockAppendLds *lds, uint32_t *const counter[NQ], const bool pred[NQ], uint32_t pos[NQ]) {
    const uint32_t lane = __lane_id(), wave = threadIdx.x >> 6, nWaves = (blockDim.x + 63) >> 6;
    unsigned long long mask[NQ];
#pragma unroll
    for (int k = 0; k < NQ; ++k) {
        mask[k] = __ballot(pred[k]);
        if (lane == 0) lds->waveCount[k][wave] = (uint32_t)__popcll(mask[k]);
    }
    __syncthreads();
    if (threadIdx.x < NQ) {
        const int k = threadIdx.x;
        uint32_t total = 0;
        for (uint32_t w = 0; w < nWaves; ++w) { const uint32_t c = lds->waveCount[k][w]; lds->waveCount[k][w] = total; total += c; }
        lds->base[k] = total ? atomicAdd(counter[k], total) : 0u;
    }
    __syncthreads();
#pragma unroll
    for (int k = 0; k < NQ; ++k)
        pos[k] = lds->base[k] + lds->waveCount[k][wave] +
                 __builtin_amdgcn_mbcnt_hi((uint32_t)(mask[k] >> 32), __builtin_amdgcn_mbcnt_lo((uint32_t)mask[k], 0u));
}

struct TraceTune { int refillBelow, parkLimit, stepLimit, sphereLimit, primMin; };
static TraceTune DefaultTraceTune(bool anyHit) {
    TraceTune t = anyHit ? TraceTune{40, 24, 10, 4, 3} : TraceTune{52, 24, 6, 4, 8};
    if (const char *e = getenv(anyHit ? "HPRT_TRACE_TUNE_ANY" : "HPRT_TRACE_TUNE"))
        sscanf(e, "%d,%d,%d,%d,%d", &t.refillBelow, &t.parkLimit, &t.stepLimit, &t.sphereLimit, &t.primMin);
    return t;
}

__device__ __forceinline__ bool slab_test(float lox, float hix, float loy, float hiy, float loz, float hiz, vec3 ro, vec3 invDir,
                                          bool negX, bool negY, bool negZ, float robust, float *tEntry) {
    float tMin = ((negX ? hix : lox) - ro.x) * invDir.x;
    float tMax = ((negX ? lox : hix) - ro.x) * invDir.x;
    const float tyMin = ((negY ? hiy : loy) - ro.y) * invDir.y;
    float tyMax = ((negY ? loy : hiy) - ro.y) * invDir.y;
    tMax *= robust; tyMax *= robust;
    bool ok = !(tMin > tyMax || tyMin > tMax);
    if (tyMin > tMin) tMin = tyMin;
    if (tyMax < tMax) tMax = tyMax;
    const float tzMin = ((negZ ? hiz : loz) - ro.z) * invDir.z;
    float tzMax = ((negZ ? loz : hiz) - ro.z) * invDir.z;
    tzMax *= robust;
    ok = ok && !(tMin > tzMax || tzMin > tMax);
    if (tzMin > tMin) tMin = tzMin;
    if (tzMax < tMax) tMax = tzMax;
    *tEntry = tMin;
    return ok && (tMax > 0);
}

__device__ __forceinline__ void slab_test_pair(f32x2 nx, f32x2 fx, f32x2 ny, f32x2 fy, f32x2 nz, f32x2 fz, float rox, float roy, float roz,
                                               float ivx, float ivy, float ivz, float robust, bool *s0, bool *s1, float *t0, float *t1) {
    f32x2 tMin = (nx - rox) * ivx;
    f32x2 tMax = (fx - rox) * ivx;
    const f32x2 tyMin = (ny - roy) * ivy;
    f32x2 tyMax = (fy - roy) * ivy;
    tMax = tMax * robust; tyMax = tyMax * robust;
    const f32x2 tzMin = (nz - roz) * ivz;
    f32x2 tzMax = (fz - roz) * ivz;
    tzMax = tzMax * robust;
    bool ok0 = !(tMin.x > tyMax.x || tyMin.x > tMax.x), ok1 = !(tMin.y > tyMax.y || tyMin.y > tMax.y);
    if (tyMin.x > tMin.x) tMin.x = tyMin.x;
    if (tyMin.y > tMin.y) tMin.y = tyMin.y;
    if (tyMax.x < tMax.x) tMax.x = tyMax.x;
    if (tyMax.y < tMax.y) tMax.y = tyMax.y;
    ok0 = ok0 && !(tMin.x > tzMax.x || tzMin.x > tMax.x); ok1 = ok1 && !(tMin.y > tzMax.y || tzMin.y > tMax.y);
    if (tzMin.x > tMin.x) tMin.x = tzMin.x;
    if (tzMin.y > tMin.y) tMin.y = tzMin.y;
    if (tzMax.x < tMax.x) tMax.x = tzMax.x;
    if (tzMax.y < tMax.y) tMax.y = tzMax.y;
    *t0 = tMin.x; *t1 = tMin.y;
    *s0 = ok0 && (tMax.x > 0); *s1 = ok1 && (tMax.y > 0);
}

__device__ unsigned long long g_traceProf[32];
#ifdef HPRT_SHADE_PROF
__device__ unsigned long long g_shadeProf[4 * 8];
__device__ unsigned long long g_shadeLanes[4 * 8 * 2];
#define SP_MARK(k) do { asm volatile("s_waitcnt vmcnt(0) lgkmcnt(0)" ::: "memory"); const unsigned long long t_ = clock64(); spT[k] += t_ - spLast; spLast = t_; \
                        const unsigned long long m_ = __ballot(1); if (__lane_id() == (uint32_t)(__ffsll((long long)m_) - 1)) { atomicAdd(&g_shadeLanes[(MODE * 8 + k) * 2], (unsigned long long)__popcll(m_)); atomicAdd(&g_shadeLanes[(MODE * 8 + k) * 2 + 1], 1ull); } } while (0)
#else
#define SP_MARK(k) do { } while (0)
#endif

template <bool ANY_HIT, int MODE, bool INST, bool QUAD>
__global__ __launch_bounds__(HPRT_TRACE_BLOCK, MODE == 0 ? (QUAD ? (ANY_HIT ? HPRT_QUAD_ANY_WAVES : HPRT_QUAD_CLOSEST_WAVES) : ANY_HIT ? HPRT_ANY_WAVES : HPRT_CLOSEST_WAVES) : 1024 / HPRT_TRACE_BLOCK) void k_trace(DevScene sc, const uint32_t *queue, const uint32_t *countPtr,
                                                            uint32_t countImm, RayStream rays, HitStream hits, uint8_t *occ,
                                                            DevCounters *counters, uint4 *rayStats, uint32_t *workCounter, uint32_t chunk,
                                                            TraceTune tune) {
    constexpr bool COUNT = MODE == 1, PROF = MODE == 2;
    constexpr bool PACKED = !QUAD;
    constexpr bool FREE_ORDER = ANY_HIT && MODE == 0;
#ifdef HPRT_DEFER_LEAF
    constexpr bool DEFER = FREE_ORDER && !INST && !QUAD;
#else
    constexpr bool DEFER = false;
#endif
    int pend = REF_NONE;
    constexpr bool HPRT_INLINE_PRETEST = true;
    unsigned long long pf[13] = {0, 0, 0, 0, 0, 0, 0, 0, 0, 0, 0, 0, 0};
    unsigned int pfPush = 0u, pfSpill = 0u;
    const unsigned long long pfStart = PROF ? clock64() : 0ull;
    constexpr int LDS_N = MODE != 0 ? HPRT_LDS_STACK
                        : !INST ? (QUAD ? (ANY_HIT ? HPRT_LDS_STACK_QUAD_ANY : HPRT_LDS_STACK) : ANY_HIT ? HPRT_LDS_STACK_ANY : HPRT_LDS_STACK_CLOSEST)
                                : (QUAD ? HPRT_LDS_STACK_QUAD_ANY : ANY_HIT ? HPRT_LDS_STACK_INST_ANY : HPRT_LDS_STACK_INST_CLOSEST);
    __shared__ uint2 stackMem[LDS_N * HPRT_TRACE_BLOCK];
    uint2 *const ldsStack = &stackMem[threadIdx.x];
    __shared__ float worldRayMem[INST ? 6 * HPRT_TRACE_BLOCK : 1];
    float *const worldRay = &worldRayMem[INST ? threadIdx.x : 0];
    const uint32_t n = countPtr ? *countPtr : countImm;
    const uint32_t lane = __lane_id();
    const auto pairRsrc = __builtin_amdgcn_make_buffer_rsrc((void *)sc.pairs, 0, (int)(sc.nPairs * 64u), 0x00020000);
    const auto triRsrc = __builtin_amdgcn_make_buffer_rsrc((void *)sc.tris, 0, (int)(sc.nPrims * 48u), 0x00020000);
    const auto entryRsrc = __builtin_amdgcn_make_buffer_rsrc((void *)(INST ? sc.topEntry : nullptr), 0, (int)(INST ? sc.nTopPrims * 16u : 0u), 0x00020000);
    const float robust = 1 + 2 * gamma_n(3);
    TraceCount cnt = {0u, 0u, 0u, 0u, 0u};
    unsigned int snapEntered = 0u, snapLeaf = 0u, snapPrim = 0u;
    bool active = false, hit = false;
    uint32_t slot = 0;
    vec3 ro, invDir;
    float rayTMax = 0.f;
    RayShear shear; shear.k0 = shear.k1 = false; shear.Sx = shear.Sy = shear.Sz = 0.f;
    bool ngX = false, ngY = false, ngZ = false;
    uint32_t negMask = 0u;
    int sp = 0, cur = REF_NONE;
    int32_t prim = -1; float hb0 = 0.f, hb1 = 0.f, hb2 = 0.f;
    uint32_t wait = 0u, waitInfo = 0u;
    int inst = -1, hitInst = -1;
    bool instHit = false;
    uint32_t instPrim = 0u;
    float savedTMax = 0.f;
    auto deepSlot = [&](int entry) -> volatile unsigned long long * {
        return (volatile unsigned long long *)sc.deepStack + (size_t)(entry - LDS_N) * HPRT_DEEP_THREADS + (blockIdx.x * HPRT_TRACE_BLOCK + threadIdx.x);
    };
    bool moreWork = n > 0 && sc.nPairs > 0;

    auto pop = [&]() -> int {
        while (sp > 0) {
            --sp;
            uint2 e;
            if (sp < LDS_N) e = ldsStack[sp * HPRT_TRACE_BLOCK]; else { const unsigned long long w = *deepSlot(sp); e = make_uint2((uint32_t)w, (uint32_t)(w >> 32)); }
            if (INST && (int)e.x == REF_EXIT) { savedTMax = __uint_as_float(e.y); return REF_EXIT; }
            if (COUNT) ++cnt.fetched;
            if (FREE_ORDER || __uint_as_float(e.y) < rayTMax) { if (COUNT) { ++cnt.entered; if ((int)e.x < 0) ++cnt.leaf; } return (int)e.x; }
        }
        return REF_NONE;
    };

    uint32_t localNext = 0u, localEnd = 0u;
    uint32_t window = 0u, windowBase = 0xffffffffu;
    if (sc.nPairs == 0 && n > 0) {
        for (uint32_t i = blockIdx.x * blockDim.x + threadIdx.x; i < n; i += gridDim.x * blockDim.x) {
// ... 524 lines not shown
                                    if (tag & TAG_LAST) leave = true; else cur = (int)((~(pi + 1u)) & ~WIDE_LEAF_FIRST);
                                } else {
                                    bool ok = true;
                                    if (c & WIDE_LEAF_FIRST) {
                                        if (!entrySingle) { x0 = __builtin_amdgcn_raw_buffer_load_b128(boxRsrc, pi * 32, 0, 0); x1 = __builtin_amdgcn_raw_buffer_load_b128(boxRsrc, pi * 32 + 16, 0, 0); }
                                        if (PROF) ++pfLeaf;
                                        ok = leaf_reached(entrySingle, x0, x1);
                                        if (PROF && ok) ++pfLeafOk;
                                    }
                                    if (ok) { hit = true; cur = REF_NONE; } else leave = true;
                                }
                            } else if (tag & TAG_LAST) leave = true;
                            else if (!ANY_HIT) cur = (int)((~(pi + 1u)) & ~WIDE_LEAF_FIRST);
                            else {
                                cur = (int)((~(pi + 1u)) & ~WIDE_LEAF_BOXED);
                            }
                        } else if (INST && (tag & TAG_KIND_MASK) == TAG_INSTANCE) {
                            inst = (int)v2.w;
                            instPrim = pi | ((tag & TAG_LAST) ? 0x80000000u : 0u);
                            instHit = false;
                            mat4 W;
                            int root;
                            if (tag & TAG_INST_INLINE) {
                                W.m[0][0] = __uint_as_float(v0.x); W.m[0][1] = __uint_as_float(v0.y); W.m[0][2] = __uint_as_float(v0.z); W.m[0][3] = __uint_as_float(ve.x);
                                W.m[1][0] = __uint_as_float(v1.x); W.m[1][1] = __uint_as_float(v1.y); W.m[1][2] = __uint_as_float(v1.z); W.m[1][3] = __uint_as_float(ve.y);
                                W.m[2][0] = __uint_as_float(v2.x); W.m[2][1] = __uint_as_float(v2.y); W.m[2][2] = __uint_as_float(v2.z); W.m[2][3] = __uint_as_float(ve.z);
                                W.m[3][0] = 0.f; W.m[3][1] = 0.f; W.m[3][2] = 0.f; W.m[3][3] = 1.f;
                                root = (int)ve.w;
                            } else { const DevInstance &in = sc.instances[inst]; W = in.w2i; root = (int)in.pad[0]; }
                            vec3 oErr;
                            vec3 o2 = xf_point_err(W, ro, &oErr);
                            const vec3 d2 = xf_vector(W, vec3(worldRay[3 * HPRT_TRACE_BLOCK], worldRay[4 * HPRT_TRACE_BLOCK], worldRay[5 * HPRT_TRACE_BLOCK]));
                            const float lengthSquared = d2.x * d2.x + d2.y * d2.y + d2.z * d2.z;
                            float tm = rayTMax;
                            if (lengthSquared > 0) {
                                const float dt = dot(vabs(d2), oErr) / lengthSquared;
                                o2 = o2 + d2 * dt;
                                tm -= dt;
                            }
                            savedTMax = rayTMax;
                            push(REF_EXIT, 0.f);
                            rayTMax = tm;
                            set_ray(o2, d2);
                            cur = root;
                        } else if (QUAD) {
                            DRay rr; rr.o = ro; rr.tMax = rayTMax; rr.d = ray_dir();
                            const bool maybe = sphere_may_hit(sc.spheres[v2.w], rr);
                            if (maybe) { wait = 1u; waitInfo = v2.w | ((tag & TAG_LAST) ? 0x80000000u : 0u) | ((tag & TAG_BIN_MASK) == (BIN_TEXTURED << TAG_BIN_SHIFT) ? 0x40000000u : 0u) | (boxKnown ? 0x20000000u : 0u); }
                            else if (tag & TAG_LAST) leave = true;
                            else cur = (int)((~(pi + 1u)) & ~(boxKnown ? WIDE_LEAF_FIRST : WIDE_LEAF_BOXED));
                        }
                        if (leave) cur = pop();
                    }
                    continue;
                }
                if (!QUAD) break;
                const bool slow = active && wait != 0u;
                const int nWait = __popcll(__ballot(slow));
                if (nWait == 0) break;
                const bool canWalk = __ballot(active && cur >= 0) != 0ull;
                if (nWait < tune.sphereLimit && canWalk) break;
                const unsigned long long pfT3 = PROF ? clock64() : 0ull;
                if (wait == 1u) {
                    const uint32_t pi = ~((uint32_t)cur | (WIDE_LEAF_BOXED | WIDE_LEAF_FIRST));
                    wait = 0u;
                    DRay rr; rr.o = ro; rr.tMax = rayTMax; rr.d = ray_dir();
                    DRay robj; vec3 ph; float phi, t;
                    bool done = false, leave = false;
                    if (sphere_test(sc.spheres[waitInfo & 0x1fffffffu], rr, &robj, &ph, &phi, &t)) {
                        bool ok = true;
                        if (ANY_HIT && !(waitInfo & 0x20000000u)) {
                            const u32x4 x0 = __builtin_amdgcn_raw_buffer_load_b128(boxRsrc, pi * 32, 0, 0), x1 = __builtin_amdgcn_raw_buffer_load_b128(boxRsrc, pi * 32 + 16, 0, 0);
                            float tEn;
                            ok = slab_test(__uint_as_float(x0.x), __uint_as_float(x0.w), __uint_as_float(x0.y), __uint_as_float(x1.x), __uint_as_float(x0.z), __uint_as_float(x1.y),
                                           ro, invDir, ngX, ngY, ngZ, robust, &tEn) && tEn < rayTMax;
                        }
                        if (!ok) leave = true;
                        else if (ANY_HIT) { hit = true; done = true; }
                        else {
                            hit = true; rayTMax = t;
                            hit_store(hits, slot, (int32_t)(pi | (((waitInfo & 0x40000000u) ? BIN_TEXTURED : BIN_GENERIC) << HIT_BIN_SHIFT)), 0.f, 0.f, 0.f, t, INST ? inst : -1);
                            if (INST) instHit = inst >= 0;
                        }
                    }
                    if (done) cur = REF_NONE;
                    else if (leave || (waitInfo & 0x80000000u)) cur = pop();
                    else cur = (int)((~(pi + 1u)) & ~(((waitInfo & 0x20000000u) || !ANY_HIT) ? WIDE_LEAF_FIRST : WIDE_LEAF_BOXED));
                }
                if (PROF) pfSphere += clock64() - pfT3;
            }
            if (PROF) { pf[3] += clock64() - pfT2 - pfSphere; pf[4] += pfSphere; }
            if (active && cur == REF_NONE) {
                if (ANY_HIT) occ[slot] = hit ? 1 : 0;
                else if (!hit) hit_store_miss(hits, slot, rayTMax);
                active = false;
            }
            const int busy = __popcll(__ballot(active));
            if (busy == 0) break;
            if (moreWork && busy < tune.refillBelow) break;
        }
    }
    if (PROF) {
        for (int off = 32; off > 0; off >>= 1) { pfPush += __shfl_down(pfPush, off); pfSpill += __shfl_down(pfSpill, off); pfLeaf += __shfl_down(pfLeaf, off); pfLeafOk += __shfl_down(pfLeafOk, off); }
        if (lane == 0) {
            pf[0] = clock64() - pfStart; pf[11] = pfLeaf; pf[12] = pfLeafOk;
            for (int k = 0; k < 13; ++k) atomicAdd(&g_traceProf[(ANY_HIT ? 16 : 0) + k], pf[k]);
            atomicAdd(&g_traceProf[(ANY_HIT ? 16 : 0) + 13], 1ull);
            atomicAdd(&g_traceProf[(ANY_HIT ? 16 : 0) + 14], (unsigned long long)pfPush); atomicAdd(&g_traceProf[(ANY_HIT ? 16 : 0) + 15], (unsigned long long)pfSpill);
        }
    }
}

__device__ __forceinline__ void footprint(const FilmGeom &fg, int px, int py, float fx, float fy, int *x0, int *x1, int *y0, int *y1) {
    const int tx0 = fg.sx0 + ((px - fg.sx0) / 16) * 16, ty0 = fg.sy0 + ((py - fg.sy0) / 16) * 16;
    const int tx1 = sel_min(tx0 + 16, fg.sx1), ty1 = sel_min(ty0 + 16, fg.sy1);
    const int bx0 = sel_max((int)ceilf((float)tx0 - 0.5f - fg.rx), fg.cx0), by0 = sel_max((int)ceilf((float)ty0 - 0.5f - fg.ry), fg.cy0);
    const int bx1 = sel_min((int)floorf((float)tx1 - 0.5f + fg.rx) + 1, fg.cx1), by1 = sel_min((int)floorf((float)ty1 - 0.5f + fg.ry) + 1, fg.cy1);
    const float dxf = fx - 0.5f, dyf = fy - 0.5f;
    *x0 = sel_max((int)ceilf(dxf - fg.rx), bx0); *y0 = sel_max((int)ceilf(dyf - fg.ry), by0);
    *x1 = sel_min((int)floorf(dxf + fg.rx) + 1, bx1); *y1 = sel_min((int)floorf(dyf + fg.ry) + 1, by1);
}
__global__ __launch_bounds__(256) void k_generate(DevScene sc, RenderParams rp, PathStream out, uint32_t s0, uint32_t nSlots, IrregularSink irr) {
    const uint32_t slot = blockIdx.x * blockDim.x + threadIdx.x;
    bool irregular = false;
    IrregularSample rec;
    if (slot < nSlots) {
        const uint32_t pix = slot % rp.nPix, sIdx = slot / rp.nPix;
        const uint32_t pxy = rp.pixelXY[pix];
        const int px = (int)(pxy & 0xffffu), py = (int)(pxy >> 16);
        const uint64_t index = (uint64_t)rp.pixelOffset[pix] + (uint64_t)(s0 + sIdx) * (uint64_t)rp.hal.sampleStride;
        const float u0 = halton_dim(sc, rp.hal, index, 0), u1 = halton_dim(sc, rp.hal, index, 1);
        const float fx = (float)px + u0, fy = (float)py + u1;
        float lu = 0.f, lv = 0.f;
        if (rp.cam.lensRadius > 0) { lu = halton_dim(sc, rp.hal, index, 3); lv = halton_dim(sc, rp.hal, index, 4); }
        DRay ray;
        camera_ray(rp.cam, fx, fy, lu, lv, &ray);
        out.ray.a[slot] = make_float4(ray.o.x, ray.o.y, ray.o.z, ray.tMax);
        out.ray.b[slot] = make_float4(ray.d.x, ray.d.y, ray.d.z, __uint_as_float(5u));
        if (irr.count) {
            int x0, x1, y0, y1;
            footprint(irr.fg, px, py, fx, fy, &x0, &x1, &y0, &y1);
            irregular = !(x0 == px && x1 == px + 1 && y0 == py && y1 == py + 1);
            rec.pix = pix; rec.sample = s0 + sIdx; rec.x0 = (int16_t)x0; rec.x1 = (int16_t)x1; rec.y0 = (int16_t)y0; rec.y1 = (int16_t)y1;
        }
    }
    if (irr.count) {
        const uint32_t pos = wave_append(irr.count, irregular);
        if (irregular && pos < irr.capacity) irr.out[pos] = rec;
    }
}

#define HPRT_BIN_ITEMS 4
__global__ __launch_bounds__(1024) void k_bin(DevScene sc, PathStream in, HitStream hit, const uint32_t *queue, const uint32_t *countPtr,
                                              uint32_t countImm, int32_t maxDepth, int32_t bounces, BinSet bins, float4 *Lfinal) {
    __shared__ uint32_t waveCount[N_BINS][HPRT_BIN_ITEMS * 16];
    __shared__ uint32_t binBase[N_BINS];
    const uint32_t n = countPtr ? *countPtr : countImm;
    const uint32_t first = blockIdx.x * (HPRT_BIN_ITEMS * 1024u);
    if (first >= n) return;
    const uint32_t lane = __lane_id(), wave = threadIdx.x >> 6;
    int bin[HPRT_BIN_ITEMS];
    uint32_t slot[HPRT_BIN_ITEMS];
    float4 hitA[HPRT_BIN_ITEMS];
#pragma unroll
    for (int k = 0; k < HPRT_BIN_ITEMS; ++k) {
        const uint32_t i = first + k * 1024u + threadIdx.x;
        slot[k] = i < n ? (queue ? queue[i] : i) : 0u;
    }
#pragma unroll
    for (int k = 0; k < HPRT_BIN_ITEMS; ++k) {
        const uint32_t i = first + k * 1024u + threadIdx.x;
        if (i < n) hitA[k] = hit_load(hit, slot[k]);
    }
    unsigned long long mask[HPRT_BIN_ITEMS][N_BINS];
#pragma unroll
    for (int k = 0; k < HPRT_BIN_ITEMS; ++k) {
        const uint32_t i = first + k * 1024u + threadIdx.x;
        bin[k] = -1;
        if (i < n) {
            const int32_t word = hit_word(hitA[k]);
            if (word >= 0) {
                const int code = (int)(((uint32_t)word >> HIT_BIN_SHIFT) & 7u);
                const bool generic = code == (int)BIN_GENERIC || code == (int)BIN_TEXTURED;
                if (bounces >= maxDepth) { if (generic && (bounces == 0 || (__float_as_uint(in.ray.b[slot[k]].w) >> 31))) bin[k] = code; }
                else bin[k] = code;
            }
            if (word < 0 && sc.nEnvLights != 0u && (bounces == 0 || (__float_as_uint(in.ray.b[slot[k]].w) >> 31))) bin[k] = 2;
            if (bin[k] < 0) {
                if (bounces == 0) Lfinal[slot[k]] = make_float4(0.f, 0.f, 0.f, 1.f);
                else {
                    const float4 b4 = in.beta[slot[k]];
                    float4 L4 = in.L[slot[k]];
                    if (word >= 0 && (__float_as_uint(in.ray.b[slot[k]].w) >> 31)) { L4.x += b4.x * 0.f; L4.y += b4.y * 0.f; L4.z += b4.z * 0.f; }
                    Lfinal[__float_as_uint(b4.w)] = L4;
                }
            }
        }
#pragma unroll
        for (int b = 0; b < (int)N_BINS; ++b) {
            mask[k][b] = __ballot(bin[k] == b);
            if (lane == 0) waveCount[b][k * 16 + wave] = (uint32_t)__popcll(mask[k][b]);
        }
    }
    __syncthreads();
    if (wave < N_BINS) {
        const uint32_t c = waveCount[wave][lane];
        uint32_t incl = c;
#pragma unroll
        for (int off = 1; off < 64; off <<= 1) { const uint32_t t = __shfl_up(incl, off); if ((int)lane >= off) incl += t; }
        waveCount[wave][lane] = incl - c;
        if (lane == 63) binBase[wave] = incl ? atomicAdd(bins.count + wave * BIN_STRIDE, incl) : 0u;
    }
    __syncthreads();
#pragma unroll
    for (int k = 0; k < HPRT_BIN_ITEMS; ++k) {
        if (bin[k] < 0) continue;
        const int b = bin[k];
        const unsigned long long m = b == 0 ? mask[k][0] : b == 1 ? mask[k][1] : b == 2 ? mask[k][2] : b == 3 ? mask[k][3] : mask[k][4];
        const uint32_t pos = binBase[b] + waveCount[b][k * 16 + wave] + __builtin_amdgcn_mbcnt_hi((uint32_t)(m >> 32), __builtin_amdgcn_mbcnt_lo((uint32_t)m, 0u));
        bins.q[b][pos] = make_uint2(slot[k], (uint32_t)hit_word(hitA[k]));
    }
}

#ifndef HPRT_SHADE_WAVES_MATTE
#define HPRT_SHADE_WAVES_MATTE 4
#endif
#ifndef HPRT_SHADE_WAVES_PLASTIC
#define HPRT_SHADE_WAVES_PLASTIC 4
#endif
#ifndef HPRT_SHADE_WAVES_GENERIC
#define HPRT_SHADE_WAVES_GENERIC 3
#endif
#ifndef HPRT_SHADE_WAVES_SUBSTRATE
#define HPRT_SHADE_WAVES_SUBSTRATE 4
#endif
template <int MODE, int BS, bool TEX = false, bool INSTS = false>
__global__ __launch_bounds__(BS, MODE == 0 ? HPRT_SHADE_WAVES_MATTE : MODE == 1 ? HPRT_SHADE_WAVES_PLASTIC : MODE == 3 ? HPRT_SHADE_WAVES_SUBSTRATE : HPRT_SHADE_WAVES_GENERIC) void k_shade(DevScene sc, RenderParams rp, PathStream in, HitStream hit, uint32_t s0,
                                               PathStream out, VertexStreams vs, QueueSet q, BinSet bins, float4 *Lfinal, uint32_t firstBounce, uint32_t retryPass) {
    __shared__ HaltonLds hl;
    __shared__ BlockAppendLds al;
    constexpr int BIN = MODE == 2 ? (TEX ? (int)BIN_TEXTURED : (int)BIN_GENERIC) : MODE == 3 ? (int)BIN_SUBSTRATE : MODE;
    constexpr int RETRY = BIN == (int)BIN_TEXTURED ? 1 : 0;
    const uint32_t n = retryPass ? bins.count[(6 + RETRY) * BIN_STRIDE] : bins.count[BIN * BIN_STRIDE];
    if (blockIdx.x * blockDim.x >= n) return;
    const uint32_t i = blockIdx.x * blockDim.x + threadIdx.x;
#ifdef HPRT_SHADE_PROF
    unsigned long long spT[8] = {0, 0, 0, 0, 0, 0, 0, 0}, spLast = clock64();
    bool spFull = false;
#endif
    bool wantNext = false, wantShadow = false, wantMis = false, wantResolve = false, defer = false, voxelMiss = false;
    bool speculated = false;
    uint32_t slot = 0;
    uint32_t j = 0;
    float4 rayA = make_float4(0.f, 0.f, 0.f, 0.f), rayB = rayA, hitA = rayA, beta4 = rayA, L4 = rayA, tv0 = rayA, tv1 = rayA, tv2 = rayA;
    float2 hitB = hit_no_aux();
    int32_t word = -1;
    const bool oneLight = sc.nLights == 1u && !sc.spatial;
    DevLight light0 = {};
    if (oneLight) light0 = sc.lights[0];
    if (i < n) {
        const uint2 e = (retryPass ? bins.retry[RETRY] : bins.q[BIN])[i];
        slot = e.x;
        word = retryPass ? hit_word(hit_load(hit, slot)) : (int32_t)e.y;
        if (retryPass) j = e.y;
        else {
            j = (BIN == (int)BIN_MATTE ? 0u : BIN == (int)BIN_PLASTIC ? bins.count[0] : BIN == (int)BIN_SUBSTRATE ? bins.count[0] + bins.count[BIN_STRIDE]
                 : BIN == (int)BIN_GENERIC ? bins.count[0] + bins.count[BIN_STRIDE] + bins.count[4 * BIN_STRIDE]
                 : bins.count[0] + bins.count[BIN_STRIDE] + bins.count[4 * BIN_STRIDE] + bins.count[5 * BIN_STRIDE]) + i;
            if (BIN == (int)BIN_GENERIC && i >= bins.count[5 * BIN_STRIDE]) j = bins.aux[i];
        }
        const int32_t p = hit_prim(word);
        if (MODE != 2 || p >= 0) { tv0 = sc.tris[3 * p]; tv1 = sc.tris[3 * p + 1]; tv2 = sc.tris[3 * p + 2]; }
        hitA = hit_load(hit, slot); rayA = in.ray.a[slot]; rayB = in.ray.b[slot];
        if ((MODE == 2 || INSTS) && hit.b) hitB = hit_load_aux(hit, slot);
        beta4 = firstBounce ? make_float4(1.f, 1.f, 1.f, __uint_as_float(slot)) : in.beta[slot];
        L4 = firstBounce ? make_float4(0.f, 0.f, 0.f, 1.f) : in.L[slot];
    }
    halton_lds_load(sc, &hl);
    if (i < n) {
        SP_MARK(6);
        const uint32_t st = __float_as_uint(rayB.w);
        int dim = (int)(st & 0xffffu);
        const int bounces = (int)((st >> 16) & 0x7fffu);
        const bool specularBounce = (st >> 31) != 0u;
        const uint32_t pathId = __float_as_uint(beta4.w);
        const uint32_t pix = pathId % rp.nPix, sIdx = pathId / rp.nPix;
        const uint64_t index = (uint64_t)rp.pixelOffset[pix] + (uint64_t)(s0 + sIdx) * (uint64_t)rp.hal.sampleStride;
        const int32_t prim = hit_prim(word);
        const vec3 rayO(rayA.x, rayA.y, rayA.z);
        const vec3 rayD(rayB.x, rayB.y, rayB.z);
        rgb beta(beta4.x, beta4.y, beta4.z);
        rgb L(L4.x, L4.y, L4.z), Ldark(0.f);
        float etaScale = L4.w;
        const bool found = prim >= 0;
        DevSI si;
        DevTexGeom tg;
        constexpr bool texScene = MODE == 2 && TEX;
        if (found) {
            const float4 v0 = tv0;
            const int inst = (MODE == 2 || INSTS) ? hit_inst(hitB) : -1;
            DRay r0; r0.o = rayO; r0.d = rayD; r0.tMax = rayA.w;
            if ((MODE == 2 || INSTS) && inst >= 0) {
                const DevInstance &in = sc.instances[inst];
                vec3 oErr;
                r0.o = xf_point_err(in.w2i, rayO, &oErr);
                r0.d = xf_vector(in.w2i, rayD);
                const float lengthSquared = r0.d.x * r0.d.x + r0.d.y * r0.d.y + r0.d.z * r0.d.z;
                if (lengthSquared > 0) {
                    const float dt = dot(vabs(r0.d), oErr) / lengthSquared;
                    r0.o = r0.o + r0.d * dt;
                    r0.tMax -= dt;
                }
            }
            if (MODE != 2 || (__float_as_uint(v0.w) & TAG_KIND_MASK) == 0u)
                fill_triangle(sc, (uint32_t)prim, tv0, tv1, tv2, hit_b0(hitA), hit_b1(hitA), hit_b2(hitA), r0.d, &si, texScene ? &tg : nullptr);
            else {
                float tt;
                fill_sphere(sc, (int)__float_as_uint(tv1.w), r0, &si, &tt, texScene ? &tg : nullptr);
            }
            if ((MODE == 2 || INSTS) && inst >= 0 && !sc.instances[inst].identity) {
                const DevInstance &in = sc.instances[inst];
                vec3 pErr;
                si.p = xf_point_err_in(in.i2w, si.p, si.pErr, &pErr); si.pErr = pErr;
                si.n = normalize(xf_normal(in.w2i, si.n));
                si.wo = normalize(xf_vector(in.i2w, si.wo));
                si.ns = normalize(xf_normal(in.w2i, si.ns));
                si.sdpdu = xf_vector(in.i2w, si.sdpdu);
                si.ns = face_forward(si.ns, si.n);
                if (texScene) { tg.dpdu = xf_vector(in.i2w, tg.dpdu); tg.dpdv = xf_vector(in.i2w, tg.dpdv); }
            }
            if (MODE == 2 && (bounces == 0 || specularBounce)) {
                const int al = prim_area_light(sc, prim);
                if (al >= 0) {
                    rgb Le = area_L(sc.lights[al], si.n, -rayD);
                    rgb add = beta * Le;
                    L = rgb(L.r + add.r, L.g + add.g, L.b + add.b);
                } else if (specularBounce) {
                    L = rgb(L.r + beta.r * 0.f, L.g + beta.g * 0.f, L.b + beta.b * 0.f);
                }
            } else if (MODE != 2 && specularBounce) L = rgb(L.r + beta.r * 0.f, L.g + beta.g * 0.f, L.b + beta.b * 0.f);
        }
        SP_MARK(0);
        if (MODE == 2 && !found && (bounces == 0 || specularBounce))
            for (uint32_t e = 0; e < sc.nEnvLights; ++e) { const rgb add = beta * env_Le(sc, sc.envLights[e], rayD); L = rgb(L.r + add.r, L.g + add.g, L.b + add.b); }
        if (found && bounces < rp.maxDepth) {
#ifdef HPRT_SHADE_PROF
            spFull = true;
#endif
            DevBsdf bsdf;
            bool useKd = false, useKs = false, useOp = false;
            rgb kdTex, ksTex, opTex;
            if (texScene) {
                const DevMaterial m = sc.materials[si_material(sc, si)];
                const int opTexId = m.type == 6 ? m.opTex : -1;
                if (m.KdTex >= 0 || m.KsTex >= 0 || opTexId >= 0) {
                    DevUvDiff uvd; uvd.dudx = uvd.dvdx = uvd.dudy = uvd.dvdy = 0.f;
                    if (bounces == 0) {
                        const float u0 = halton_dim(sc, rp.hal, index, 0, &hl), u1 = halton_dim(sc, rp.hal, index, 1, &hl);
                        const uint32_t pxy = rp.pixelXY[pix];
                        const float fx = (float)(int)(pxy & 0xffffu) + u0, fy = (float)(int)(pxy >> 16) + u1;
                        float lu = 0.f, lv = 0.f;
                        if (rp.cam.lensRadius > 0) { lu = halton_dim(sc, rp.hal, index, 3, &hl); lv = halton_dim(sc, rp.hal, index, 4, &hl); }
                        DevRayDiff rd;
                        camera_ray_diff(rp.cam, fx, fy, lu, lv, &rd);
                        const float s = rp.invSqrtSpp;
                        rd.rxO = rayO + (rd.rxO - rayO) * s; rd.ryO = rayO + (rd.ryO - rayO) * s;
                        rd.rxD = rayD + (rd.rxD - rayD) * s; rd.ryD = rayD + (rd.ryD - rayD) * s;
                        compute_differentials(si, tg, rd, &uvd);
                    }
#pragma unroll 1
                    for (int k = 0; k < 3; ++k) {
                        const int id = k == 0 ? m.KdTex : k == 1 ? m.KsTex : opTexId;
                        if (id < 0) continue;
                        const rgb r = eval_image_texture(sc, id, tg, uvd);
                        if (k == 0) { kdTex = r; useKd = true; } else if (k == 1) { ksTex = r; useKs = true; } else { opTex = r; useOp = true; }
                    }
                }
            }
            bsdf_init(sc, si, &bsdf, useKd ? &kdTex : nullptr, useKs ? &ksTex : nullptr, useOp ? &opTex : nullptr);
            if (MODE == 0) { bsdf.hasS = false; bsdf.Rs = rgb(0.f); bsdf.alpha = 0.f; }
            if (MODE != 2) { bsdf.hasR = false; bsdf.hasT = false; bsdf.oren = false; bsdf.kind = 0; }
            if (MODE == 3) { bsdf.kind = 2; bsdf.hasD = false; }
            SP_MARK(1);
            if (bsdf_num(bsdf) > 0 && sc.nLights > 0) {
                float pickPdf;
                int lightNum = 0;
                if (oneLight) pickPdf = (sc.lightFuncInt > 0) ? sc.lightFunc[0] / (sc.lightFuncInt * 1) : 0;
                else lightNum = light_pick(sc, si.p, sc.nLights > 1u ? halton_dim(sc, rp.hal, index, dim, &hl) : 0.f, &pickPdf, &voxelMiss);
                dim += 1;
                if (voxelMiss) defer = true;
                if (pickPdf != 0) {
                    const DevLight light = oneLight ? light0 : sc.lights[lightNum];
                    const bool isDelta = light.type < 2;
                    float ul0 = 0.f, ul1 = 0.f, us0 = 0.f, us1 = 0.f;
                    if (!isDelta) {
                        ul0 = halton_dim(sc, rp.hal, index, dim, &hl); ul1 = halton_dim(sc, rp.hal, index, dim + 1, &hl);
                        us0 = halton_dim(sc, rp.hal, index, dim + 2, &hl); us1 = halton_dim(sc, rp.hal, index, dim + 3, &hl);
                    }
                    dim += 4;
                    vec3 wi;
                    float lightPdf = 0, scatteringPdf = 0;
                    DevIt it; it.p = si.p; it.pErr = si.pErr; it.n = si.n;
                    DevIt pl;
                    if (MODE != 2 && !isDelta && (light.type >= 3 || sphere_ref_inside(sc.spheres[light.sphere], it))) defer = true;
                    SP_MARK(2);
                    if (!defer) {
                    rgb Li = light_sample<MODE == 2>(sc, light, it, ul0, ul1, &wi, &lightPdf, &pl);
                    rgb pendLight(0.f), pendMis(0.f);
                    if (lightPdf > 0 && !is_black(Li)) {
                        rgb f = bsdf_f(bsdf, si.wo, wi) * absdot(wi, si.ns);
                        scatteringPdf = bsdf_pdf(bsdf, si.wo, wi);
                        if (!is_black(f)) {
                            vec3 origin = offset_ray_origin(it.p, it.pErr, it.n, pl.p - it.p);
                            vec3 target = offset_ray_origin(pl.p, pl.pErr, pl.n, origin - pl.p);
                            vec3 d = target - origin;
                            vs.shadow.a[j] = make_float4(origin.x, origin.y, origin.z, 1 - HPRT_SHADOW_EPS);
                            vs.shadow.b[j] = make_float4(d.x, d.y, d.z, 0.f);
                            if (isDelta) pendLight = f * Li / lightPdf;
                            else { float w = power_heuristic(lightPdf, scatteringPdf); pendLight = f * Li * w / lightPdf; }
                            wantShadow = true;
                        }
                    }
                    SP_MARK(3);
                    if (!isDelta) {
                        int sampledType = 0;
                        rgb f = bsdf_sample(bsdf, si.wo, &wi, us0, us1, &scatteringPdf, &sampledType);
                        f = f * absdot(wi, si.ns);
                        if (!is_black(f) && scatteringPdf > 0) {
                            const vec3 o = offset_ray_origin(si.p, si.pErr, si.n, wi);
                            DRay mr; mr.o = o; mr.d = wi; mr.tMax = HPRT_INF;
                            float tb0, tb1, tb2, tt;
                            if (!rp.cullMis || (MODE == 2 && light.type == 4) ||
                                (MODE == 2 && light.type == 3 ? triangle_may_hit(sc, light.prim, mr, &tb0, &tb1, &tb2, &tt)
                                                              : sphere_may_hit(sc.spheres[light.sphere], mr))) {
                                const float lp = light_pdf<MODE == 2>(sc, light, it, wi);
                                if (lp != 0) {
                                    const float w = power_heuristic(scatteringPdf, lp);
                                    vs.mis.a[j] = make_float4(o.x, o.y, o.z, HPRT_INF);
                                    vs.mis.b[j] = make_float4(wi.x, wi.y, wi.z, 0.f);
                                    rgb Lemit(light.I[0], light.I[1], light.I[2]);
                                    if (MODE == 2 && light.type == 4) Lemit = env_Le(sc, sc.envLights[light.shape], wi);
                                    pendMis = f * Lemit * rgb(1.f) * w / scatteringPdf;
                                    wantMis = true;
                                }
                            }
                        }
                    }
                    if (rp.speculate && wantShadow && !wantMis) {
                        rgb LdLit(0.f);
                        LdLit = LdLit + pendLight;
                        const rgb addLit = beta * (LdLit / pickPdf), addDark = beta * (rgb(0.f) / pickPdf);
                        Ldark = rgb(L.r + addDark.r, L.g + addDark.g, L.b + addDark.b);
                        L = rgb(L.r + addLit.r, L.g + addLit.g, L.b + addLit.b);
                        speculated = true;
                    } else if (wantShadow || wantMis) {
                        vs.pendLight[j] = make_float4(pendLight.r, pendLight.g, pendLight.b,
                                                      __uint_as_float((uint32_t)lightNum | (wantShadow ? 0x40000000u : 0u) | (wantMis ? 0x80000000u : 0u)));
                        if (wantMis || sc.spatial) vs.pendMis[j] = make_float4(pendMis.r, pendMis.g, pendMis.b, pickPdf);
                        vs.pendBeta[j] = make_float4(beta.r, beta.g, beta.b, beta4.w);
                        wantResolve = true;
                    }
                    }
                }
            }
            if (!defer && !wantResolve && !speculated && bsdf_num(bsdf) > 0) L = rgb(L.r + beta.r * 0.f, L.g + beta.g * 0.f, L.b + beta.b * 0.f);
            SP_MARK(4);
            if (!defer) {
            const float ub0 = halton_dim(sc, rp.hal, index, dim, &hl), ub1 = halton_dim(sc, rp.hal, index, dim + 1, &hl);
            dim += 2;
            vec3 wo = -rayD, wi;
            float pdf = 0; int flags = 0;
            rgb f = bsdf_sample(bsdf, wo, &wi, ub0, ub1, &pdf, &flags, true);
            if (!(is_black(f) || pdf == 0.f)) {
                beta = beta * (f * absdot(wi, si.ns) / pdf);
                vec3 o = offset_ray_origin(si.p, si.pErr, si.n, wi);
                bool alive = true;
                if (MODE == 2 && (flags & BX_SPECULAR) && (flags & BX_TRANSMISSION)) {
                    const float eta = bsdf.eta;
                    etaScale *= (dot(wo, si.n) > 0) ? (eta * eta) : 1 / (eta * eta);
                }
                rgb rrBeta = beta * etaScale;
                if (max_value(rrBeta) < rp.rrThreshold && bounces > 3) {
                    float qv = sel_max(.05f, 1 - max_value(rrBeta));
                    float u = halton_dim(sc, rp.hal, index, dim, &hl);
                    dim += 1;
                    if (u < qv) alive = false;
                    else beta = beta / (1 - qv);
                }
                if (rp.cullMis && bounces + 1 >= rp.maxDepth && !(flags & BX_SPECULAR)) alive = false;
                if (alive) {
                    out.ray.a[j] = make_float4(o.x, o.y, o.z, HPRT_INF);
                    out.ray.b[j] = make_float4(wi.x, wi.y, wi.z, __uint_as_float((uint32_t)dim | ((uint32_t)(bounces + 1) << 16) | ((flags & BX_SPECULAR) ? 0x80000000u : 0u)));
                    out.beta[j] = make_float4(beta.r, beta.g, beta.b, beta4.w);
                    wantNext = true;
                }
            }
            }
        }
        if (!defer) {
            if (speculated) vs.pendBeta[j] = make_float4(Ldark.r, Ldark.g, Ldark.b, __uint_as_float(pathId | SPEC_RECORD | (wantNext ? 0u : SPEC_END)));
            if (wantNext || wantResolve) out.L[j] = make_float4(L.r, L.g, L.b, wantNext ? etaScale : 0.f);
            else Lfinal[pathId] = make_float4(L.r, L.g, L.b, 0.f);
        }
    }
    SP_MARK(5);
#ifdef HPRT_SHADE_PROF
    {
        const unsigned long long m = __ballot(spFull);
        if (m != 0ull && __lane_id() == (uint32_t)(__ffsll((long long)m) - 1)) {
            for (int k = 0; k < 7; ++k) atomicAdd(&g_shadeProf[MODE * 8 + k], spT[k]);
            atomicAdd(&g_shadeProf[MODE * 8 + 7], 1ull);
        }
    }
#endif
    if (MODE != 2) {
        const bool toGeneric = defer && !voxelMiss;
        const uint32_t p2 = wave_append(bins.count + 2 * BIN_STRIDE, toGeneric);
        if (toGeneric) { bins.q[2][p2] = make_uint2(slot, (uint32_t)word); bins.aux[p2] = j; }
    }
    if (sc.voxSlot) {
        const uint32_t pr = wave_append(bins.count + (6 + RETRY) * BIN_STRIDE, voxelMiss && !retryPass);
        if (voxelMiss && !retryPass) bins.retry[RETRY][pr] = make_uint2(slot, j);
    }
    uint32_t *const ctr[4] = {q.nextCount, q.shadowCount, q.misCount, q.resolveCount};
    const bool pred[4] = {wantNext, wantShadow, wantMis, wantResolve};
    uint32_t pos[4];
    block_append<4>(&al, ctr, pred, pos);
    if (wantNext) q.next[pos[0]] = j;
    if (wantShadow) q.shadow[pos[1]] = j;
    if (wantMis) q.mis[pos[2]] = j;
    if (wantResolve) q.resolve[pos[3]] = j;
}

__global__ __launch_bounds__(256) void k_resolve(DevScene sc, VertexStreams vs, float4 *Lio, float4 *Lfinal, const uint32_t *queue,
                                                 const uint32_t *countPtr) {
    const uint32_t n = *countPtr;
    const uint32_t i = blockIdx.x * blockDim.x + threadIdx.x;
    if (i >= n) return;
    const uint32_t j = queue[i];
    const float4 pl = vs.pendLight[j], pb = vs.pendBeta[j], L4 = Lio[j];
    const uint32_t info = __float_as_uint(pl.w);
    const int lightNum = (int)(info & 0x3fffffffu);
    float4 pm = make_float4(0.f, 0.f, 0.f, 0.f);
    if ((info & 0x80000000u) || sc.spatial) pm = vs.pendMis[j];
    const float pickPdf = sc.spatial ? pm.w : ((sc.lightFuncInt > 0) ? sc.lightFunc[lightNum] / (sc.lightFuncInt * (int)sc.nLights) : 0);
    rgb Ld(0.f);
    if ((info & 0x40000000u) && !vs.occluded[j]) Ld = Ld + rgb(pl.x, pl.y, pl.z);
    if (info & 0x80000000u) {
        const float4 mh = hit_load(vs.misHit, j);
        const int32_t prim = hit_prim(hit_word(mh));
        if (prim < 0) {
            if (sc.lights[lightNum].type == 4) Ld = Ld + rgb(pm.x, pm.y, pm.z);
        } else if (prim_area_light(sc, prim) == lightNum) {
            const float4 ma = vs.mis.a[j], mb = vs.mis.b[j];
            DRay r; r.o = vec3(ma.x, ma.y, ma.z); r.d = vec3(mb.x, mb.y, mb.z); r.tMax = HPRT_INF;
            const DevLight light = sc.lights[lightNum];
            DevSI li;
            bool filled;
            if (light.type == 3) { fill_triangle(sc, (uint32_t)prim, hit_b0(mh), hit_b1(mh), hit_b2(mh), r.d, &li); filled = true; }
            else { float tt; filled = fill_sphere(sc, (int)__float_as_uint(sc.tris[3 * prim + 1].w), r, &li, &tt); }
            if (filled && (light.twoSided || dot(li.n, -r.d) > 0)) Ld = Ld + rgb(pm.x, pm.y, pm.z);
        }
    }
    rgb add = rgb(pb.x, pb.y, pb.z) * (Ld / pickPdf);
    const float4 Lnew = make_float4(L4.x + add.r, L4.y + add.g, L4.z + add.b, L4.w);
    if (L4.w != 0.f) Lio[j] = Lnew;
    else Lfinal[__float_as_uint(pb.w)] = Lnew;
}

template <bool COUNT>
__global__ __launch_bounds__(256) void k_repair(VertexStreams vs, float4 *Lio, float4 *Lfinal, const uint32_t *queue, uint32_t n, uint32_t *counts) {
    const uint32_t i = blockIdx.x * blockDim.x + threadIdx.x;
    if (i >= n) return;
    const uint32_t j = queue[i];
    const bool occluded = vs.occluded[j] != 0;
    if (!COUNT && !occluded) return;
    const float4 rec = vs.pendBeta[j];
    const uint32_t w = __float_as_uint(rec.w);
    if (!(w & SPEC_RECORD)) return;
    if (COUNT) atomicAdd(counts, 1u);
    if (!occluded) return;
    if (COUNT) atomicAdd(counts + 1, 1u);
    if (w & SPEC_END) Lfinal[w & SPEC_ID_MASK] = make_float4(rec.x, rec.y, rec.z, 0.f);
    else {
        float *const Lj = reinterpret_cast<float *>(Lio + j);
        Lj[0] = rec.x; Lj[1] = rec.y; Lj[2] = rec.z;
    }
}

__global__ __launch_bounds__(256) void k_store_radiance(const float4 *Lfinal, float *LallR, float *LallG, float *LallB, uint32_t nPix,
                                                         uint32_t s0, uint32_t nSlots) {
    const uint32_t slot = blockIdx.x * blockDim.x + threadIdx.x;
    if (slot >= nSlots) return;
    const float4 L4 = Lfinal[slot];
    rgb L(L4.x, L4.y, L4.z);
    const float y = luminance(L);
    if (is_nan(L.r) || is_nan(L.g) || is_nan(L.b)) L = rgb(0.f);
    else if ((double)y < -1e-5) L = rgb(0.f);
    else if (is_inf(y)) L = rgb(0.f);
    const size_t o = (size_t)s0 * nPix + slot;
    LallR[o] = L.r; LallG[o] = L.g; LallB[o] = L.b;
}

__global__ __launch_bounds__(256) void k_find_irregular(DevScene sc, RenderParams rp, FilmGeom fg, uint32_t spp, uint32_t *count,
                                                        uint32_t capacity, IrregularSample *out) {
    const size_t g = (size_t)blockIdx.x * blockDim.x + threadIdx.x;
    const size_t total = (size_t)rp.nPix * spp;
    bool irregular = false;
    IrregularSample rec;
    if (g < total) {
        const uint32_t pix = (uint32_t)(g % rp.nPix), s = (uint32_t)(g / rp.nPix);
        const uint32_t pxy = rp.pixelXY[pix];
        const int px = (int)(pxy & 0xffffu), py = (int)(pxy >> 16);
        const uint64_t index = (uint64_t)rp.pixelOffset[pix] + (uint64_t)s * (uint64_t)rp.hal.sampleStride;
        const float fx = (float)px + halton_dim(sc, rp.hal, index, 0), fy = (float)py + halton_dim(sc, rp.hal, index, 1);
        int x0, x1, y0, y1;
        footprint(fg, px, py, fx, fy, &x0, &x1, &y0, &y1);
        irregular = !(x0 == px && x1 == px + 1 && y0 == py && y1 == py + 1);
        rec.pix = pix; rec.sample = s; rec.x0 = (int16_t)x0; rec.x1 = (int16_t)x1; rec.y0 = (int16_t)y0; rec.y1 = (int16_t)y1;
    }
    const uint32_t pos = wave_append(count, irregular);
    if (irregular && pos < capacity) out[pos] = rec;
}

__device__ __forceinline__ rgb clamp_luminance(rgb L, float maxY) {
    float y = luminance(L);
    if (y > maxY) { float s = maxY / luminance(L); L = L * s; }
    return L;
}
__device__ __forceinline__ void rgb_to_xyz(rgb c, float xyz[3]) {
    xyz[0] = 0.412453f * c.r + 0.357580f * c.g + 0.180423f * c.b;
    xyz[1] = 0.212671f * c.r + 0.715160f * c.g + 0.072169f * c.b;
    xyz[2] = 0.019334f * c.r + 0.119193f * c.g + 0.950227f * c.b;
}
__global__ __launch_bounds__(256) void k_film_own(RenderParams rp, FilmGeom fg, const float *LallR, const float *LallG,
                                                  const float *LallB, uint32_t spp, FilmExtras ex, float *filmXYZW) {
    const uint32_t pix = blockIdx.x * blockDim.x + threadIdx.x;
    if (pix >= rp.nPix) return;
    rgb c(0.f); float w = 0.f;
    const uint32_t eBeg = ex.ownBegin ? ex.ownBegin[pix] : 0u, eEnd = ex.ownBegin ? ex.ownBegin[pix + 1] : 0u;
    uint32_t e = eBeg;
    for (; e < eEnd && ex.ownIsPre[e]; ++e) {
        const size_t o = (size_t)ex.ownSample[e] * rp.nPix + ex.ownSrcPix[e];
        c = c + clamp_luminance(rgb(LallR[o], LallG[o], LallB[o]), fg.maxSampleLuminance) * 1.0f * 1.0f;
        w += 1.f;
    }
    for (uint32_t s = 0; s < spp; ++s) {
        const size_t o = (size_t)s * rp.nPix + pix;
        c = c + clamp_luminance(rgb(LallR[o], LallG[o], LallB[o]), fg.maxSampleLuminance) * 1.0f * 1.0f;
        w += 1.f;
    }
    for (; e < eEnd; ++e) {
        const size_t o = (size_t)ex.ownSample[e] * rp.nPix + ex.ownSrcPix[e];
        c = c + clamp_luminance(rgb(LallR[o], LallG[o], LallB[o]), fg.maxSampleLuminance) * 1.0f * 1.0f;
        w += 1.f;
    }
    float xyz[3];
    rgb_to_xyz(c, xyz);
    const uint32_t pxy = rp.pixelXY[pix];
    const int px = (int)(pxy & 0xffffu), py = (int)(pxy >> 16);
    const size_t fo = 4 * ((size_t)(py - fg.cy0) * (size_t)(fg.cx1 - fg.cx0) + (size_t)(px - fg.cx0));
    filmXYZW[fo] = 0.f + xyz[0]; filmXYZW[fo + 1] = 0.f + xyz[1]; filmXYZW[fo + 2] = 0.f + xyz[2]; filmXYZW[fo + 3] = 0.f + w;
}
__global__ __launch_bounds__(64) void k_film_foreign(RenderParams rp, FilmGeom fg, const float *LallR, const float *LallG,
                                                     const float *LallB, FilmExtras ex, float *filmXYZW) {
    const uint32_t d = blockIdx.x * blockDim.x + threadIdx.x;
    if (d >= ex.nForeignDest) return;
    const size_t fo = 4 * (size_t)ex.foreignDestFilmIndex[d];
    for (uint32_t g = ex.foreignDestBegin[d]; g < ex.foreignDestBegin[d + 1]; ++g) {
        rgb c(0.f); float w = 0.f;
        for (uint32_t e = ex.foreignGroupBegin[g]; e < ex.foreignGroupBegin[g + 1]; ++e) {
            const size_t o = (size_t)ex.foreignSample[e] * rp.nPix + ex.foreignSrcPix[e];
            c = c + clamp_luminance(rgb(LallR[o], LallG[o], LallB[o]), fg.maxSampleLuminance) * 1.0f * 1.0f;
            w += 1.f;
        }
        float xyz[3];
        rgb_to_xyz(c, xyz);
        filmXYZW[fo] += xyz[0]; filmXYZW[fo + 1] += xyz[1]; filmXYZW[fo + 2] += xyz[2]; filmXYZW[fo + 3] += w;
    }
}

__global__ __launch_bounds__(64) void k_film_foreign_export(RenderParams rp, FilmGeom fg, const float *LallR, const float *LallG,
                                                            const float *LallB, FilmExtras ex, uint32_t nGroups, const uint32_t *groupDest,
                                                            const uint32_t *groupTile, FilmRecord *out) {
    const uint32_t g = blockIdx.x * blockDim.x + threadIdx.x;
    if (g >= nGroups) return;
    rgb c(0.f); float w = 0.f;
    for (uint32_t e = ex.foreignGroupBegin[g]; e < ex.foreignGroupBegin[g + 1]; ++e) {
        const size_t o = (size_t)ex.foreignSample[e] * rp.nPix + ex.foreignSrcPix[e];
        c = c + clamp_luminance(rgb(LallR[o], LallG[o], LallB[o]), fg.maxSampleLuminance) * 1.0f * 1.0f;
        w += 1.f;
    }
    FilmRecord r;
    r.dest = groupDest[g]; r.srcTile = groupTile[g];
    rgb_to_xyz(c, r.xyz);
    r.w = w;
    out[g] = r;
}
__global__ __launch_bounds__(64) void k_film_apply_records(const FilmRecord *rec, const uint32_t *destBegin, uint32_t nDest, float *filmXYZW) {
    const uint32_t d = blockIdx.x * blockDim.x + threadIdx.x;
    if (d >= nDest) return;
    const size_t fo = 4 * (size_t)rec[destBegin[d]].dest;
    for (uint32_t k = destBegin[d]; k < destBegin[d + 1]; ++k) {
        filmXYZW[fo] += rec[k].xyz[0]; filmXYZW[fo + 1] += rec[k].xyz[1]; filmXYZW[fo + 2] += rec[k].xyz[2]; filmXYZW[fo + 3] += rec[k].w;
    }
}

__global__ __launch_bounds__(256) void k_voxel_contrib(DevScene sc, const float *ri, uint32_t nVox, float *contrib, const uint32_t *voxList) {
    const size_t g = (size_t)blockIdx.x * blockDim.x + threadIdx.x;
    const uint32_t n = sc.nLights;
    if (g >= (size_t)nVox * n) return;
    const uint32_t row = (uint32_t)(g / n), j = (uint32_t)(g % n);
    const uint32_t v = voxList ? voxList[row] : row;
    int pi[3]; pi[2] = (int)(v % (uint32_t)sc.voxN[2]); pi[1] = (int)((v / (uint32_t)sc.voxN[2]) % (uint32_t)sc.voxN[1]); pi[0] = (int)(v / ((uint32_t)sc.voxN[2] * (uint32_t)sc.voxN[1]));
    float vMin[3], vMax[3];
#pragma unroll
    for (int a = 0; a < 3; ++a) {
        const float t0 = (float)pi[a] / (float)sc.voxN[a], t1 = (float)(pi[a] + 1) / (float)sc.voxN[a];
        vMin[a] = (1 - t0) * sc.wbMin[a] + t0 * sc.wbMax[a];
        vMax[a] = (1 - t1) * sc.wbMin[a] + t1 * sc.wbMax[a];
    }
    const DevLight light = sc.lights[j];
    float acc = 0.f;
    for (int i = 0; i < 128; ++i) {
        DevIt ref;
        ref.p = vec3((1 - ri[i]) * vMin[0] + ri[i] * vMax[0], (1 - ri[128 + i]) * vMin[1] + ri[128 + i] * vMax[1], (1 - ri[256 + i]) * vMin[2] + ri[256 + i] * vMax[2]);
        ref.pErr = vec3(); ref.n = vec3();
        vec3 wi; float pdf = 0.f; DevIt pl;
        const rgb Li = light_sample<true>(sc, light, ref, ri[384 + i], ri[512 + i], &wi, &pdf, &pl);
        if (pdf > 0) acc += luminance(Li) / pdf;
    }
    contrib[g] = acc;
}
__global__ __launch_bounds__(256) void k_voxel_dist(uint32_t nLights, uint32_t nVox, float *func, float *cdf, float *funcInt) {
    const uint32_t v = blockIdx.x * blockDim.x + threadIdx.x;
    if (v >= nVox) return;
    float *f = func + (size_t)v * nLights, *c = cdf + (size_t)v * (nLights + 1);
    float sum = 0.f;
    for (uint32_t i = 0; i < nLights; ++i) sum += f[i];
    const float avg = sum / (float)(128ull * nLights);
    const float minContrib = (avg > 0) ? (float)(.001 * (double)avg) : 1.f;
    for (uint32_t i = 0; i < nLights; ++i) f[i] = sel_max(f[i], minContrib);
    const int n = (int)nLights;
    c[0] = 0;
    for (int i = 1; i < n + 1; ++i) c[i] = c[i - 1] + f[i - 1] / n;
    const float fi = c[n];
    if (fi == 0) for (int i = 1; i < n + 1; ++i) c[i] = float(i) / float(n);
    else for (int i = 1; i < n + 1; ++i) c[i] /= fi;
    funcInt[v] = fi;
}

__global__ void k_fill_u32(uint32_t *p, uint32_t v, size_t n) {
    const size_t i = (size_t)blockIdx.x * blockDim.x + threadIdx.x;
    if (i < n) p[i] = v;
}

static inline uint32_t blocks_for(size_t n, uint32_t bs) { return (uint32_t)((n + bs - 1) / bs); }

static int g_wideWalk = -1;
static bool WideWalkEnabled() {
    static const bool fromEnv = [] { const char *e = getenv("HPRT_WIDE_WALK"); return !(e && atoi(e) == 0); }();
    return g_wideWalk < 0 ? fromEnv : g_wideWalk != 0;
}
static int g_traceProfileMode = -1;
static bool TraceProfileEnabled() {
    static const bool fromEnv = getenv("HPRT_TRACE_PROFILE") != nullptr;
    return g_traceProfileMode < 0 ? fromEnv : g_traceProfileMode != 0;
}
extern "C" __attribute__((visibility("default"))) int hprt_debug_trace_profile_mode(int on) { const int was = TraceProfileEnabled() ? 1 : 0; g_traceProfileMode = on; return was; }
bool WideWalkInUse(const DevScene &sc) { return sc.wide != nullptr && WideWalkEnabled(); }
extern "C" __attribute__((visibility("default"))) int hprt_debug_wide_walk(int on) { const int was = WideWalkEnabled() ? 1 : 0; g_wideWalk = on; return was; }
void LaunchTrace(hipStream_t st, const DevScene &sc, bool anyHit, bool count, const uint32_t *queue, const uint32_t *countPtr,
                 uint32_t countImm, uint32_t gridItems, const RayStream &rays, const HitStream &hits, uint8_t *occ,
                 DevCounters *counters, uint32_t *workCounter, uint4 *rayStats) {
    if (gridItems == 0) return;
    (void)hipMemsetAsync(workCounter, 0, sizeof(uint32_t), st);
    static const uint32_t blockCap = [] { const char *e = getenv("HPRT_TRACE_MAX_BLOCKS"); return e ? (uint32_t)std::max(1, atoi(e)) : 0xffffffffu; }();
    static const uint32_t anyPerCu = [] { const char *e = getenv("HPRT_TRACE_ANY_PER_CU"); return e ? (uint32_t)std::min((int)(HPRT_DEEP_THREADS / (256u * HPRT_TRACE_BLOCK)), std::max(1, atoi(e))) : (uint32_t)HPRT_ANY_WAVES; }();
    const bool profile = TraceProfileEnabled();
    const bool plain = !count && !profile;
    const bool hasQuad = sc.nSpheres != 0u;
    static const uint32_t closestPerCu = [] { const char *e = getenv("HPRT_TRACE_CLOSEST_PER_CU"); return e ? (uint32_t)std::min(7, std::max(1, atoi(e))) : (uint32_t)HPRT_CLOSEST_WAVES; }();
    const uint32_t perCu = !plain ? 4u : hasQuad ? (anyHit ? (uint32_t)HPRT_QUAD_ANY_WAVES : (uint32_t)HPRT_QUAD_CLOSEST_WAVES) : (anyHit ? anyPerCu : closestPerCu);
    const uint32_t maxBlocks = std::min(256u * perCu, blockCap);
    static_assert(HPRT_DEEP_THREADS >= 256u * HPRT_TRACE_BLOCK * HPRT_ANY_WAVES && HPRT_DEEP_THREADS >= 256u * HPRT_TRACE_BLOCK * HPRT_CLOSEST_WAVES &&
                  HPRT_DEEP_THREADS >= 256u * HPRT_TRACE_BLOCK * HPRT_QUAD_ANY_WAVES, "the deep-stack area must cover the largest trace grid");
    dim3 grid(std::min(blocks_for(gridItems, HPRT_TRACE_BLOCK), maxBlocks)), block(HPRT_TRACE_BLOCK);
    const uint32_t nWaves = grid.x * (HPRT_TRACE_BLOCK / 64);
    static const uint32_t chunkMax = [] { const char *e = getenv("HPRT_TRACE_CHUNK_MAX"); return e ? (uint32_t)atoi(e) : 512u; }();
    static const uint32_t chunkDiv = [] { const char *e = getenv("HPRT_TRACE_CHUNK_DIV"); return e ? (uint32_t)atoi(e) : 4u; }();
    uint32_t chunk = gridItems / (nWaves * chunkDiv);
    chunk = std::max(64u, std::min(chunkMax, chunk)) & ~63u;
    static const TraceTune tuneClosest = DefaultTraceTune(false), tuneAny = DefaultTraceTune(true);
    TraceTune tune = anyHit ? tuneAny : tuneClosest;
    static const bool tuneFromEnv = getenv("HPRT_TRACE_TUNE") != nullptr;
    if (!anyHit && !tuneFromEnv && sc.nPairs > 100000u) { tune.parkLimit = 32; tune.stepLimit = 14; tune.primMin = 12; }
    const bool inst = sc.nInstances != 0u, quad = sc.nSpheres != 0u;
    static const bool tuneAnyFromEnv = getenv("HPRT_TRACE_TUNE_ANY") != nullptr;
    if (inst && !anyHit && !tuneFromEnv) { tune.parkLimit = 32; tune.stepLimit = 10; tune.primMin = 12; }
    if (inst && anyHit && !tuneAnyFromEnv) { tune.refillBelow = 48; tune.parkLimit = 32; tune.stepLimit = 10; tune.primMin = 6; }
    if (!count && sc.wide != nullptr && WideWalkEnabled()) {
        static const uint32_t wClosestPerCu = [] { const char *e = getenv("HPRT_WALK4_CLOSEST_PER_CU"); return e ? (uint32_t)std::min((int)HPRT_WALK4_CLOSEST_WAVES, std::max(1, atoi(e))) : (uint32_t)HPRT_WALK4_CLOSEST_WAVES; }();
        static const uint32_t wAnyPerCu = [] { const char *e = getenv("HPRT_WALK4_ANY_PER_CU"); return e ? (uint32_t)std::min((int)HPRT_WALK4_ANY_WAVES, std::max(1, atoi(e))) : (uint32_t)HPRT_WALK4_ANY_WAVES; }();
        static const TraceTune wTuneClosest = [] { TraceTune t{52, 32, 8, 4, 12}; if (const char *e = getenv("HPRT_WALK4_TUNE")) sscanf(e, "%d,%d,%d,%d,%d", &t.refillBelow, &t.parkLimit, &t.stepLimit, &t.sphereLimit, &t.primMin); return t; }();
        static const TraceTune wTuneAny = [] { TraceTune t{52, 28, 6, 4, 4}; if (const char *e = getenv("HPRT_WALK4_TUNE_ANY")) sscanf(e, "%d,%d,%d,%d,%d", &t.refillBelow, &t.parkLimit, &t.stepLimit, &t.sphereLimit, &t.primMin); return t; }();
        const uint32_t wPerCu = profile ? 4u : quad ? (anyHit ? (uint32_t)HPRT_QUAD_ANY_WAVES : (uint32_t)HPRT_QUAD_CLOSEST_WAVES) : inst ? (anyHit ? (uint32_t)HPRT_WALK4_INST_ANY_WAVES : (uint32_t)HPRT_WALK4_INST_CLOSEST_WAVES) : anyHit ? wAnyPerCu : wClosestPerCu;
        const uint32_t wBlocks = std::min(256u * wPerCu, blockCap);
        dim3 wGrid(std::min(blocks_for(gridItems, HPRT_TRACE_BLOCK), wBlocks));
        const uint32_t wWaves = wGrid.x * (HPRT_TRACE_BLOCK / 64);
        uint32_t wChunk = gridItems / (wWaves * chunkDiv);
        wChunk = std::max(64u, std::min(chunkMax, wChunk)) & ~63u;
        TraceTune wTune = anyHit ? wTuneAny : wTuneClosest;
        static const bool wTuneEnv = getenv("HPRT_WALK4_TUNE") != nullptr, wTuneAnyEnv = getenv("HPRT_WALK4_TUNE_ANY") != nullptr;
        if (inst && !anyHit && !wTuneEnv) wTune = TraceTune{52, 40, 14, 4, 16};
        if (inst && anyHit && !wTuneAnyEnv) wTune = TraceTune{48, 40, 14, 4, 8};
#define HPRT_WALK4_LAUNCH(A, P, I, Q) hipLaunchKernelGGL((k_walk4<A, P, I, Q>), wGrid, block, 0, st, sc, queue, countPtr, countImm, rays, hits, occ, workCounter, wChunk, wTune)
#define HPRT_WALK4_PICK(A) do { if (profile) { if (inst) HPRT_WALK4_LAUNCH(A, true, true, true); else HPRT_WALK4_LAUNCH(A, true, false, true); } \
                                else if (inst) { if (quad) HPRT_WALK4_LAUNCH(A, false, true, true); else HPRT_WALK4_LAUNCH(A, false, true, false); } \
                                else { if (quad) HPRT_WALK4_LAUNCH(A, false, false, true); else HPRT_WALK4_LAUNCH(A, false, false, false); } } while (0)
        if (anyHit) HPRT_WALK4_PICK(true); else HPRT_WALK4_PICK(false);
#undef HPRT_WALK4_PICK
#undef HPRT_WALK4_LAUNCH
        return;
    }
#define HPRT_TRACE_LAUNCH(A, M, I, Q) hipLaunchKernelGGL((k_trace<A, M, I, Q>), grid, block, 0, st, sc, queue, countPtr, countImm, rays, hits, occ, counters, rayStats, workCounter, chunk, tune)
#define HPRT_TRACE_PICK(A, M) do { if (inst) { if (quad || M == 2) HPRT_TRACE_LAUNCH(A, M, true, true); else HPRT_TRACE_LAUNCH(A, M, true, (M == 2)); } \
                                   else { if (quad || M == 2) HPRT_TRACE_LAUNCH(A, M, false, true); else HPRT_TRACE_LAUNCH(A, M, false, (M == 2)); } } while (0)
    if (anyHit) {
        if (count) HPRT_TRACE_PICK(true, 1); else if (profile) HPRT_TRACE_PICK(true, 2); else HPRT_TRACE_PICK(true, 0);
    } else {
        if (count) HPRT_TRACE_PICK(false, 1); else if (profile) HPRT_TRACE_PICK(false, 2); else HPRT_TRACE_PICK(false, 0);
    }
#undef HPRT_TRACE_PICK
#undef HPRT_TRACE_LAUNCH
}
#ifdef HPRT_SHADE_PROF
extern "C" __attribute__((visibility("default"))) int hprt_debug_shade_profile(unsigned long long out[24 + 48]) {
    if (hipMemcpyFromSymbol(out, HIP_SYMBOL(g_shadeProf), sizeof(unsigned long long) * 24) != hipSuccess) return -1;
    return hipMemcpyFromSymbol(out + 24, HIP_SYMBOL(g_shadeLanes), sizeof(unsigned long long) * 48) == hipSuccess ? 0 : -1;
}
#endif
extern "C" __attribute__((visibility("default"))) int hprt_debug_trace_profile(unsigned long long out[32], int reset) {
    if (hipMemcpyFromSymbol(out, HIP_SYMBOL(g_traceProf), sizeof(unsigned long long) * 32) != hipSuccess) return -1;
    if (reset) { unsigned long long z[32] = {0}; if (hipMemcpyToSymbol(HIP_SYMBOL(g_traceProf), z, sizeof(z)) != hipSuccess) return -1; }
    return 0;
}
void LaunchGenerate(hipStream_t st, const DevScene &sc, const RenderParams &rp, const PathStream &out, uint32_t s0, uint32_t nSlots,
                    const IrregularSink *irr) {
    IrregularSink sink; memset(&sink, 0, sizeof(sink));
    if (irr) sink = *irr;
    if (nSlots) hipLaunchKernelGGL(k_generate, dim3(blocks_for(nSlots, 256)), dim3(256), 0, st, sc, rp, out, s0, nSlots, sink);
}
void LaunchBin(hipStream_t st, const DevScene &sc, const PathStream &in, const HitStream &hit, const uint32_t *queue,
               const uint32_t *countPtr, uint32_t countImm, uint32_t gridItems, int32_t maxDepth, int32_t bounces, const BinSet &bins,
               float4 *Lfinal) {
    if (gridItems) hipLaunchKernelGGL(k_bin, dim3(blocks_for(gridItems, HPRT_BIN_ITEMS * 1024)), dim3(1024), 0, st, sc, in, hit, queue, countPtr, countImm, maxDepth, bounces, bins, Lfinal);
}
void LaunchShade(hipStream_t st, int mode, const DevScene &sc, const RenderParams &rp, const PathStream &in, const HitStream &hit,
                 uint32_t gridItems, uint32_t s0, const PathStream &out, const VertexStreams &vs, const QueueSet &q,
                 const BinSet &bins, float4 *Lfinal, bool firstBounce, bool retryPass) {
    if (gridItems == 0) return;
    static const int shadeCfg = [] {
        const char *e = getenv("HPRT_SHADE_BLOCK");
        const std::string v = e ? e : "512";
        return v == "1024" ? 0 : v == "256" ? 2 : 1;
    }();
    const bool specialised = mode == (int)BIN_MATTE || mode == (int)BIN_PLASTIC || mode == (int)BIN_SUBSTRATE;
    const uint32_t bs = !specialised ? 256u : (shadeCfg == 0 ? 1024u : shadeCfg == 1 ? 512u : 256u);
    dim3 grid(blocks_for(gridItems, bs)), block(bs);
#define HPRT_SHADE_LAUNCH_I(M, B, I) hipLaunchKernelGGL((k_shade<M, B, false, I>), grid, block, 0, st, sc, rp, in, hit, s0, out, vs, q, bins, Lfinal, firstBounce ? 1u : 0u, retryPass ? 1u : 0u)
#define HPRT_SHADE_LAUNCH(M, B) do { if (M != 2 && sc.nInstances != 0u) HPRT_SHADE_LAUNCH_I(M, B, (M != 2)); else HPRT_SHADE_LAUNCH_I(M, B, false); } while (0)
#define HPRT_SHADE_PICK(M) switch (shadeCfg) { case 0: HPRT_SHADE_LAUNCH(M, 1024); break; case 1: HPRT_SHADE_LAUNCH(M, 512); break; default: HPRT_SHADE_LAUNCH(M, 256); break; }
    if (mode == 3) hipLaunchKernelGGL((k_shade<2, 256, true>), grid, block, 0, st, sc, rp, in, hit, s0, out, vs, q, bins, Lfinal, firstBounce ? 1u : 0u, retryPass ? 1u : 0u);
    else if (mode == 2) { HPRT_SHADE_LAUNCH(2, 256); }
    else if (mode == 0) { HPRT_SHADE_PICK(0) }
    else if (mode == (int)BIN_SUBSTRATE) { HPRT_SHADE_PICK(3) }
    else { HPRT_SHADE_PICK(1) }
#undef HPRT_SHADE_PICK
#undef HPRT_SHADE_LAUNCH
}
void LaunchResolve(hipStream_t st, const DevScene &sc, const VertexStreams &vs, float4 *L, float4 *Lfinal, const uint32_t *queue,
                   const uint32_t *countPtr, uint32_t gridItems) {
    if (gridItems) hipLaunchKernelGGL(k_resolve, dim3(blocks_for(gridItems, 256)), dim3(256), 0, st, sc, vs, L, Lfinal, queue, countPtr);
}
void LaunchRepair(hipStream_t st, const VertexStreams &vs, float4 *L, float4 *Lfinal, const uint32_t *queue, uint32_t n, uint32_t *counts) {
    if (n == 0) return;
    if (counts) hipLaunchKernelGGL(k_repair<true>, dim3(blocks_for(n, 256)), dim3(256), 0, st, vs, L, Lfinal, queue, n, counts);
    else hipLaunchKernelGGL(k_repair<false>, dim3(blocks_for(n, 256)), dim3(256), 0, st, vs, L, Lfinal, queue, n, counts);
}
void LaunchStoreRadiance(hipStream_t st, const float4 *Lfinal, float *LallR, float *LallG, float *LallB, uint32_t nPix, uint32_t s0,
                         uint32_t nSlots) {
    if (nSlots) hipLaunchKernelGGL(k_store_radiance, dim3(blocks_for(nSlots, 256)), dim3(256), 0, st, Lfinal, LallR, LallG, LallB, nPix, s0, nSlots);
}
__global__ __launch_bounds__(256) void k_pack_rays(const float *r7, uint32_t n, RayStream out) {
    const uint32_t i = blockIdx.x * blockDim.x + threadIdx.x;
    if (i >= n) return;
    const size_t N = n;
    out.a[i] = make_float4(r7[i], r7[N + i], r7[2 * N + i], r7[6 * N + i]);
    out.b[i] = make_float4(r7[3 * N + i], r7[4 * N + i], r7[5 * N + i], 0.f);
}
__global__ __launch_bounds__(256) void k_unpack_hits(HitStream h, uint32_t n, float *t, int32_t *prim, float *bary3) {
    const uint32_t i = blockIdx.x * blockDim.x + threadIdx.x;
    if (i >= n) return;
    const float4 a = hit_load(h, i);
    t[i] = hit_t(hit_load_aux(h, i)); prim[i] = hit_prim(hit_word(a));
    if (bary3) { const size_t N = n; bary3[i] = hit_b0(a); bary3[N + i] = hit_b1(a); bary3[2 * N + i] = hit_b2(a); }
}
__global__ __launch_bounds__(256) void k_pixel_stats(const uint4 *rayStats, const float4 *ids, const uint32_t *queue, const uint32_t *countPtr,
                                                     uint32_t countImm, uint32_t nPix, int anyHit, uint32_t *pix) {
    const uint32_t n = countPtr ? *countPtr : countImm;
    const uint32_t i = blockIdx.x * blockDim.x + threadIdx.x;
    if (i >= n) return;
    const uint32_t slot = queue ? queue[i] : i;
    const uint4 c = rayStats[slot];
    const uint32_t p = (ids ? __float_as_uint(ids[slot].w) : slot) % nPix;
    uint32_t *base = pix + (anyHit ? nPix : 0u) + p;
    if (c.z) atomicAdd(base, c.z);
    if (c.y) atomicAdd(base + 2 * (size_t)nPix, c.y);
    if (c.x) atomicAdd(base + 4 * (size_t)nPix, c.x);
}
void LaunchPixelStats(hipStream_t st, const uint4 *rayStats, const float4 *ids, const uint32_t *queue, const uint32_t *countPtr,
                      uint32_t countImm, uint32_t gridItems, uint32_t nPix, bool anyHit, uint32_t *pix) {
    if (gridItems) hipLaunchKernelGGL(k_pixel_stats, dim3(blocks_for(gridItems, 256)), dim3(256), 0, st, rayStats, ids, queue, countPtr, countImm, nPix, anyHit ? 1 : 0, pix);
}
__global__ __launch_bounds__(256) void k_pixel_stats_to_film(const uint32_t *pix, const uint32_t *pixelXY, uint32_t nPix, uint32_t spp, int cx0, int cy0,
                                                             int width, unsigned long long *out7) {
    const uint32_t p = blockIdx.x * blockDim.x + threadIdx.x;
    if (p >= nPix) return;
    const uint32_t pxy = pixelXY[p];
    const size_t f = (size_t)((int)(pxy >> 16) - cy0) * (size_t)width + (size_t)((int)(pxy & 0xffffu) - cx0);
    unsigned long long *o = out7 + 7 * f;
    o[0] = spp;
    for (int k = 0; k < 6; ++k) o[1 + k] = pix[(size_t)k * nPix + p];
}
void LaunchPixelStatsToFilm(hipStream_t st, const uint32_t *pix, const uint32_t *pixelXY, uint32_t nPix, uint32_t spp, int cx0, int cy0, int width,
                            unsigned long long *out7) {
    if (nPix) hipLaunchKernelGGL(k_pixel_stats_to_film, dim3(blocks_for(nPix, 256)), dim3(256), 0, st, pix, pixelXY, nPix, spp, cx0, cy0, width, out7);
}
__global__ __launch_bounds__(256) void k_capture_rays(const uint32_t *queue, uint32_t n, RayStream rays, float *out7, uint32_t cap) {
    const uint32_t i = blockIdx.x * blockDim.x + threadIdx.x;
    if (i >= n) return;
    const uint32_t s = queue ? queue[i] : i;
    const float4 a = rays.a[s], b = rays.b[s];
    const size_t N = cap;
    out7[i] = a.x; out7[N + i] = a.y; out7[2 * N + i] = a.z; out7[3 * N + i] = b.x; out7[4 * N + i] = b.y; out7[5 * N + i] = b.z; out7[6 * N + i] = a.w;
}
void LaunchCaptureRays(hipStream_t st, const uint32_t *queue, uint32_t n, const RayStream &rays, float *out7, uint32_t cap) {
    n = std::min(n, cap);
    if (n) hipLaunchKernelGGL(k_capture_rays, dim3(blocks_for(n, 256)), dim3(256), 0, st, queue, n, rays, out7, cap);
}
__global__ __launch_bounds__(256) void k_stream_copy(const float4 *__restrict__ src, float4 *__restrict__ dst, size_t n) {
    const size_t base = (size_t)blockIdx.x * 1024u + threadIdx.x;
    float4 v[4];
#pragma unroll
    for (int k = 0; k < 4; ++k) if (base + k * 256u < n) v[k] = src[base + k * 256u];
#pragma unroll
    for (int k = 0; k < 4; ++k) if (base + k * 256u < n) dst[base + k * 256u] = v[k];
}
void LaunchStreamCopy(hipStream_t st, const float4 *src, float4 *dst, size_t n) {
    if (n) hipLaunchKernelGGL(k_stream_copy, dim3((uint32_t)((n + 1023) / 1024)), dim3(256), 0, st, src, dst, n);
}
__global__ __launch_bounds__(256, 6) void k_gather_probe(const uint4 *__restrict__ rec, uint32_t mask, uint32_t levels, int iters, uint32_t *out) {
    __shared__ uint32_t occupancyPad[6144];
    uint32_t idx = (blockIdx.x * 256u + threadIdx.x) * 2654435761u, acc = 0;
    if (threadIdx.x == 999u) occupancyPad[0] = 1u;
    for (int it = 0; it < iters; ++it) {
        idx = idx * 1664525u + 1013904223u;
        const uint32_t l = (idx >> 3) % levels;
        const uint32_t r = ((1u << l) | ((idx >> 8) & ((1u << l) - 1u))) & mask;
        const uint4 a = rec[4 * r], b = rec[4 * r + 1], c = rec[4 * r + 2], d = rec[4 * r + 3];
        acc += a.x ^ b.y ^ c.z ^ d.w;
        idx ^= a.x;
    }
    if (acc == 0x12345678u) out[0] = acc + occupancyPad[threadIdx.x];
}
void LaunchGatherProbe(hipStream_t st, const uint4 *records, uint32_t log2Records, int itersPerLane, uint32_t blocks, uint32_t *sink) {
    hipLaunchKernelGGL(k_gather_probe, dim3(blocks), dim3(256), 0, st, records, (1u << log2Records) - 1u, log2Records, itersPerLane, sink);
}
void LaunchPackRays(hipStream_t st, const float *rays7, uint32_t n, const RayStream &out) {
    if (n) hipLaunchKernelGGL(k_pack_rays, dim3(blocks_for(n, 256)), dim3(256), 0, st, rays7, n, out);
}
void LaunchUnpackHits(hipStream_t st, const HitStream &hits, uint32_t n, float *t, int32_t *prim, float *bary3) {
    if (n) hipLaunchKernelGGL(k_unpack_hits, dim3(blocks_for(n, 256)), dim3(256), 0, st, hits, n, t, prim, bary3);
}
void LaunchFindIrregular(hipStream_t st, const DevScene &sc, const RenderParams &rp, const FilmGeom &fg, uint32_t spp, uint32_t *count,
                         uint32_t capacity, IrregularSample *out) {
    const size_t total = (size_t)rp.nPix * spp;
    if (total) hipLaunchKernelGGL(k_find_irregular, dim3(blocks_for(total, 256)), dim3(256), 0, st, sc, rp, fg, spp, count, capacity, out);
}
void LaunchFilmOwn(hipStream_t st, const RenderParams &rp, const FilmGeom &fg, const float *LallR, const float *LallG, const float *LallB,
                   uint32_t spp, const FilmExtras &ex, float *film) {
    if (rp.nPix) hipLaunchKernelGGL(k_film_own, dim3(blocks_for(rp.nPix, 256)), dim3(256), 0, st, rp, fg, LallR, LallG, LallB, spp, ex, film);
}
void LaunchFilmForeign(hipStream_t st, const RenderParams &rp, const FilmGeom &fg, const float *LallR, const float *LallG,
                       const float *LallB, const FilmExtras &ex, float *film) {
    if (ex.nForeignDest) hipLaunchKernelGGL(k_film_foreign, dim3(blocks_for(ex.nForeignDest, 64)), dim3(64), 0, st, rp, fg, LallR, LallG, LallB, ex, film);
}
void LaunchVoxelDistributions(hipStream_t st, const DevScene &sc, const float *ri, uint32_t nVox, float *func, float *cdf, float *funcInt) {
    const size_t total = (size_t)nVox * sc.nLights;
    if (!total) return;
    hipLaunchKernelGGL(k_voxel_contrib, dim3(blocks_for(total, 256)), dim3(256), 0, st, sc, ri, nVox, func, (const uint32_t *)nullptr);
    hipLaunchKernelGGL(k_voxel_dist, dim3(blocks_for(nVox, 256)), dim3(256), 0, st, sc.nLights, nVox, func, cdf, funcInt);
}
__global__ __launch_bounds__(256) void k_voxel_assign(const uint32_t *voxList, uint32_t n, uint32_t rowBase, int32_t *voxSlot) {
    const uint32_t k = blockIdx.x * blockDim.x + threadIdx.x;
    if (k < n) voxSlot[voxList[k]] = (int32_t)(rowBase + k);
}
void LaunchVoxelFill(hipStream_t st, const DevScene &sc, const float *ri, uint32_t n, uint32_t rowBase, float *func, float *cdf, float *funcInt) {
    if (!n) return;
    const size_t total = (size_t)n * sc.nLights;
    hipLaunchKernelGGL(k_voxel_contrib, dim3(blocks_for(total, 256)), dim3(256), 0, st, sc, ri, n, func + (size_t)rowBase * sc.nLights, (const uint32_t *)sc.voxRequest);
    hipLaunchKernelGGL(k_voxel_dist, dim3(blocks_for(n, 256)), dim3(256), 0, st, sc.nLights, n, func + (size_t)rowBase * sc.nLights, cdf + (size_t)rowBase * (sc.nLights + 1), funcInt + rowBase);
    hipLaunchKernelGGL(k_voxel_assign, dim3(blocks_for(n, 256)), dim3(256), 0, st, (const uint32_t *)sc.voxRequest, n, rowBase, sc.voxSlot);
}
void LaunchFilmForeignExport(hipStream_t st, const RenderParams &rp, const FilmGeom &fg, const float *LallR, const float *LallG,
                             const float *LallB, const FilmExtras &ex, uint32_t nGroups, const uint32_t *groupDest, const uint32_t *groupTile,
                             FilmRecord *out) {
    if (nGroups) hipLaunchKernelGGL(k_film_foreign_export, dim3(blocks_for(nGroups, 64)), dim3(64), 0, st, rp, fg, LallR, LallG, LallB, ex, nGroups, groupDest, groupTile, out);
}
void LaunchFilmApplyRecords(hipStream_t st, const FilmRecord *rec, const uint32_t *destBegin, uint32_t nDest, float *film) {
    if (nDest) hipLaunchKernelGGL(k_film_apply_records, dim3(blocks_for(nDest, 64)), dim3(64), 0, st, rec, destBegin, nDest, film);
}

}
```

Before: 6230 Mrays/s.

## Fold speculative light repair into next-bounce bin and shade kernels

The per-bounce repair kernel over all shadow rays is replaced. Paths that continue now carry a fold mark in the ray flags and a double-buffered pending record, and the next bounce's bin and shade kernels pick the dark radiance when the shadow ray was occluded. A repair pass still runs, but only over the new 'end' queue of paths that terminated this bounce. This removes a full pass over shadow slots each bounce, in exchange for an extra queue, an extra pending buffer, and more loads and branches in the bin and shade kernels. The repair kernel itself also handles four items per thread.

```diff
diff --git a/thesis-pbrt-v3_amd/csrc/capi_device.hip b/thesis-pbrt-v3_amd/csrc/capi_device.hip
--- a/thesis-pbrt-v3_amd/csrc/capi_device.hip
+++ b/thesis-pbrt-v3_amd/csrc/capi_device.hip
@@ -42,9 +42,10 @@
     PathStream path[2];
     HitStream hit;
     VertexStreams vs;
+    float4 *pend[2];
     float4 *Lfinal;
 };
-const size_t kPlaneBytesPerSlot = 16 * (2 * 4 + 1 + 2 + 2 + 1 + 3 + 1) + 1, kInstancePlaneBytesPerSlot = 8 + 8;
+const size_t kPlaneBytesPerSlot = 16 * (2 * 4 + 1 + 2 + 2 + 1 + 4 + 1) + 1, kInstancePlaneBytesPerSlot = 8 + 8;
 size_t PlaneBytesPerSlot(bool instances) { return kPlaneBytesPerSlot + (instances ? kInstancePlaneBytesPerSlot : 0); }
 size_t PlaneBytes(size_t n, bool instances) { return n * PlaneBytesPerSlot(instances) + 32 * 256; }
 
@@ -55,7 +56,9 @@
     w->hit.a = a.take<float4>(n); w->hit.b = instances ? a.take<float2>(n) : nullptr;
     rays(w->vs.shadow); w->vs.occluded = a.take<uint8_t>(n);
     rays(w->vs.mis); w->vs.misHit.a = a.take<float4>(n); w->vs.misHit.b = instances ? a.take<float2>(n) : nullptr;
-    w->vs.pendLight = a.take<float4>(n); w->vs.pendMis = a.take<float4>(n); w->vs.pendBeta = a.take<float4>(n);
+    w->vs.pendLight = a.take<float4>(n); w->vs.pendMis = a.take<float4>(n);
+    for (int k = 0; k < 2; ++k) w->pend[k] = a.take<float4>(n);
+    w->vs.pendBeta = w->pend[0]; w->vs.pendPrev = w->pend[1];
     w->Lfinal = a.take<float4>(n);
 }
 
@@ -242,6 +245,12 @@
     return g_speculateLight < 0 ? fromEnv : g_speculateLight != 0;
 }
 __attribute__((visibility("default"))) int hprt_debug_speculate_light(int on) { const int was = SpeculateLightEnabled() ? 1 : 0; g_speculateLight = on; return was; }
+static int g_foldRepair = -1;
+static bool FoldRepairEnabled() {
+    static const bool fromEnv = [] { const char *e = getenv("HPRT_FOLD_REPAIR"); return !(e && atoi(e) == 0); }();
+    return g_foldRepair < 0 ? fromEnv : g_foldRepair != 0;
+}
+__attribute__((visibility("default"))) int hprt_debug_fold_repair(int on) { const int was = FoldRepairEnabled() ? 1 : 0; g_foldRepair = on; return was; }
 __attribute__((visibility("default"))) int hprt_debug_poison_workspace(HprtScene *s, int byte) { if (!s) return HPRT_E_INVALID; s->poisonByte = byte < 0 ? -1 : (byte & 255); return HPRT_OK; }
 __attribute__((visibility("default"))) int hprt_debug_capture_rays(HprtScene *s, int bounce, int kind, float *d_out7, size_t cap) {
     if (!s || kind < 0 || kind > 2 || cap > 0x7fffffffull) return HPRT_E_INVALID;
@@ -793,6 +802,7 @@
     RenderParams rp = rpIn;
     rp.speculate = SpeculateLightEnabled() && !pixelStats && !rayStats && nSlots <= SPEC_MAX_PATHS ? 1 : 0;
     assert(!rp.speculate || nSlots <= SPEC_MAX_PATHS);
+    rp.foldRepair = rp.speculate && FoldRepairEnabled() && !s->shadeCountsOn ? 1 : 0;
     uint32_t *specCounts = rp.speculate && s->shadeCountsOn ? s->queueCounts.as<uint32_t>() + kSpecCountsAt : nullptr;
     if (specCounts) HIP_TRY(hipMemsetAsync(specCounts, 0, 2 * sizeof(uint32_t), st));
     uint32_t *pixelKd = pixelStats && CountsKdShare(s) ? s->pixelKdLocal.as<uint32_t>() : nullptr;
@@ -818,15 +828,17 @@
     for (int bounce = 0; active > 0; ++bounce) {
         const QueueSet &cur = q[bounce & 1];
         const PathStream &in = w.path[bounce & 1], &out = w.path[(bounce + 1) & 1];
+        VertexStreams vs = w.vs;
+        vs.pendBeta = w.pend[bounce & 1]; vs.pendPrev = w.pend[(bounce + 1) & 1];
         HIP_TRY(hipMemsetAsync(cur.nextCount, 0, 256 * sizeof(uint32_t), st));
         HIP_TRY(hipMemsetAsync(bins.count, 0, 8 * BIN_STRIDE * sizeof(uint32_t), st));
-        LaunchBin(st, s->dev, in, w.hit, activeQ, nullptr, active, active, rp.maxDepth, bounce, bins, w.Lfinal);
+        LaunchBin(st, s->dev, in, w.hit, activeQ, nullptr, active, active, rp.maxDepth, bounce, bins, w.Lfinal, vs, rp.foldRepair != 0);
         HIP_TRY(hipMemcpyAsync(bins.count + 5 * BIN_STRIDE, bins.count + 2 * BIN_STRIDE, sizeof(uint32_t), hipMemcpyDeviceToDevice, st));
         static const int order[5] = {BIN_MATTE, BIN_PLASTIC, BIN_SUBSTRATE, BIN_GENERIC, BIN_TEXTURED};
         for (int k = 0; k < (s->dev.textures ? 5 : 4); ++k) {
             const int mode = order[k];
             if (mode == (int)BIN_SUBSTRATE && !s->hasSubstrateBin) continue;
-            LaunchShade(st, mode, s->dev, rp, in, w.hit, active, s0, out, w.vs, cur, bins, w.Lfinal, bounce == 0);
+            LaunchShade(st, mode, s->dev, rp, in, w.hit, active, s0, out, vs, cur, bins, w.Lfinal, bounce == 0);
         }
         HIP_TRY(hipMemcpyAsync(s->hostCounts + 4096, cur.nextCount, 256 * sizeof(uint32_t), hipMemcpyDeviceToHost, st));
         if (s->shadeCountsOn) {
@@ -847,17 +859,18 @@
                 s->voxRowsUsed += nReq;
                 HIP_TRY(hipMemsetAsync(s->dev.voxRequestCount, 0, sizeof(uint32_t), st));
                 for (int r = 0; r < 2; ++r)
-                    if (nRetry[r]) LaunchShade(st, 2 + r, s->dev, rp, in, w.hit, nRetry[r], s0, out, w.vs, cur, bins, w.Lfinal, bounce == 0, true);
+                    if (nRetry[r]) LaunchShade(st, 2 + r, s->dev, rp, in, w.hit, nRetry[r], s0, out, vs, cur, bins, w.Lfinal, bounce == 0, true);
                 HIP_TRY(hipMemcpyAsync(s->hostCounts + 4096, cur.nextCount, 256 * sizeof(uint32_t), hipMemcpyDeviceToHost, st));
             }
         }
         HIP_TRY(hipStreamSynchronize(st));
         if (s->shadeCountsOn) s->shadeDeferred += s->hostCounts[12] - s->hostCounts[13];
         const uint32_t nNext = s->hostCounts[4096], nShadow = s->hostCounts[4096 + 64], nMis = s->hostCounts[4096 + 128], nResolve = s->hostCounts[4096 + 192];
+        const uint32_t nEnd = s->hostCounts[4096 + 32];
         if (s->capture.out7 && s->capture.bounce == bounce && s0 == 0) {
             const uint32_t *cq = s->capture.kind == 0 ? cur.next : s->capture.kind == 1 ? cur.shadow : cur.mis;
             const uint32_t cn = s->capture.kind == 0 ? nNext : s->capture.kind == 1 ? nShadow : nMis;
-            const RayStream &cs = s->capture.kind == 0 ? out.ray : s->capture.kind == 1 ? w.vs.shadow : w.vs.mis;
+            const RayStream &cs = s->capture.kind == 0 ? out.ray : s->capture.kind == 1 ? vs.shadow : vs.mis;
             LaunchCaptureRays(st, cq, cn, cs, s->capture.out7, (uint32_t)s->capture.cap);
             s->capture.n = std::min<size_t>(cn, s->capture.cap);
         }
@@ -865,9 +878,9 @@
             hipEvent_t a = ev.get(), b = ev.get();
             HIP_TRY(hipEventRecord(a, st));
             HitStream none; none.a = nullptr; none.b = nullptr;
-            Trace(s, st, true, count, cur.shadow, nullptr, nShadow, nShadow, w.vs.shadow, none, w.vs.occluded, ctr, wcPath, rayStats);
-            if (pixelStats) LaunchPixelStats(st, rayStats, w.vs.pendBeta, cur.shadow, nullptr, nShadow, nShadow, rp.nPix, true, pixelStats);
-            if (pixelKd) LaunchPixelKdStats(st, rayStats, w.vs.pendBeta, cur.shadow, nullptr, nShadow, nShadow, rp.nPix, true, pixelKd);
+            Trace(s, st, true, count, cur.shadow, nullptr, nShadow, nShadow, vs.shadow, none, vs.occluded, ctr, wcPath, rayStats);
+            if (pixelStats) LaunchPixelStats(st, rayStats, vs.pendBeta, cur.shadow, nullptr, nShadow, nShadow, rp.nPix, true, pixelStats);
+            if (pixelKd) LaunchPixelKdStats(st, rayStats, vs.pendBeta, cur.shadow, nullptr, nShadow, nShadow, rp.nPix, true, pixelKd);
             HIP_TRY(hipEventRecord(b, st));
             evOcc.push_back({a, b}); bt->occludedRays += nShadow; ++bt->occludedLaunches;
             stats->shadow_rays += nShadow;
@@ -875,17 +888,18 @@
         if (nMis) {
             hipEvent_t a = ev.get(), b = ev.get();
             HIP_TRY(hipEventRecord(a, st));
-            Trace(s, st, false, count, cur.mis, nullptr, nMis, nMis, w.vs.mis, w.vs.misHit, nullptr, ctr, wcPath, rayStats);
-            if (pixelStats) LaunchPixelStats(st, rayStats, w.vs.pendBeta, cur.mis, nullptr, nMis, nMis, rp.nPix, false, pixelStats);
-            if (pixelKd) LaunchPixelKdStats(st, rayStats, w.vs.pendBeta, cur.mis, nullptr, nMis, nMis, rp.nPix, false, pixelKd);
+            Trace(s, st, false, count, cur.mis, nullptr, nMis, nMis, vs.mis, vs.misHit, nullptr, ctr, wcPath, rayStats);
+            if (pixelStats) LaunchPixelStats(st, rayStats, vs.pendBeta, cur.mis, nullptr, nMis, nMis, rp.nPix, false, pixelStats);
+            if (pixelKd) LaunchPixelKdStats(st, rayStats, vs.pendBeta, cur.mis, nullptr, nMis, nMis, rp.nPix, false, pixelKd);
             HIP_TRY(hipEventRecord(b, st));
             evExt.push_back({a, b}); bt->extendRays += nMis; ++bt->extendLaunches;
             stats->rays += nMis;
         }
         activeQ = cur.next; active = nNext;
         if (active > 0 && bounce > rp.maxDepth) return SetError(HPRT_E_DEVICE, "internal error: paths are still active beyond maxdepth");
-        if (nResolve) LaunchResolve(st, s->dev, w.vs, out.L, w.Lfinal, cur.resolve, cur.resolveCount, nResolve);
-        if (rp.speculate && nShadow) LaunchRepair(st, w.vs, out.L, w.Lfinal, cur.shadow, nShadow, specCounts);
+        if (nResolve) LaunchResolve(st, s->dev, vs, out.L, w.Lfinal, cur.resolve, cur.resolveCount, nResolve);
+        if (rp.foldRepair) { if (nEnd) LaunchRepair(st, vs, out.L, w.Lfinal, cur.end, nEnd, nullptr); }
+        else if (rp.speculate && nShadow) LaunchRepair(st, vs, out.L, w.Lfinal, cur.shadow, nShadow, specCounts);
         if (s->shadeCountsOn) s->shadeFull += nResolve;
         if (active > 0) { int rc = tracePath(bounce + 1); if (rc != HPRT_OK) return rc; }
     }
@@ -899,7 +913,7 @@
     return HPRT_OK;
 }
 
-constexpr size_t kQueueWordsPerSlot = 8 + 1 + 2 * N_BINS;
+constexpr size_t kQueueWordsPerSlot = 10 + 1 + 2 * N_BINS;
 int EnsureWorkspace(HprtScene *s, size_t nSlots, Workspace *ps, QueueSet *qa, QueueSet *qb, BinSet *bins) {
     const bool instances = s->dev.nInstances != 0u;
     HIP_TRY(s->planes.alloc(PlaneBytes(nSlots, instances)));
@@ -909,12 +923,13 @@
     uint32_t *qbase = s->queues.as<uint32_t>(), *cbase = s->queueCounts.as<uint32_t>();
     QueueSet *qs[2] = {qa, qb};
     for (int k = 0; k < 2; ++k) {
-        qs[k]->next = qbase + (4 * k + 0) * nSlots; qs[k]->shadow = qbase + (4 * k + 1) * nSlots;
-        qs[k]->mis = qbase + (4 * k + 2) * nSlots; qs[k]->resolve = qbase + (4 * k + 3) * nSlots;
+        qs[k]->next = qbase + (5 * k + 0) * nSlots; qs[k]->shadow = qbase + (5 * k + 1) * nSlots;
+        qs[k]->mis = qbase + (5 * k + 2) * nSlots; qs[k]->resolve = qbase + (5 * k + 3) * nSlots; qs[k]->end = qbase + (5 * k + 4) * nSlots;
         qs[k]->nextCount = cbase + 256 * k; qs[k]->shadowCount = cbase + 256 * k + 64; qs[k]->misCount = cbase + 256 * k + 128; qs[k]->resolveCount = cbase + 256 * k + 192;
-    }
-    bins->aux = qbase + 8 * nSlots;
-    for (int k = 0; k < (int)N_BINS; ++k) bins->q[k] = reinterpret_cast<uint2 *>(qbase + (9 + 2 * k) * nSlots + (nSlots & 1u));
+        qs[k]->endCount = cbase + 256 * k + 32;
+    }
+    bins->aux = qbase + 10 * nSlots;
+    for (int k = 0; k < (int)N_BINS; ++k) bins->q[k] = reinterpret_cast<uint2 *>(qbase + (11 + 2 * k) * nSlots + (nSlots & 1u));
     bins->count = cbase + 512;
     bins->retry[0] = bins->retry[1] = nullptr;
     if (s->dev.voxSlot) {
@@ -1009,7 +1024,7 @@
     rp.invSqrtSpp = 1 / std::sqrt((float)spp);
     const bool wantPixelStats = (desc->flags & HPRT_RENDER_PIXEL_STATS) != 0;
     const bool count = (desc->flags & HPRT_RENDER_COUNT_WORK) != 0 || wantPixelStats;
-    rp.speculate = 0;
+    rp.speculate = rp.foldRepair = 0;
     rp.cullMis = (!count || (desc->flags & HPRT_RENDER_COUNT_TRACED) != 0) && !(desc->flags & HPRT_RENDER_TRACE_ALL) ? 1 : 0;
     uint32_t *pixelStats = nullptr;
     if (wantPixelStats) {
@@ -1244,7 +1259,7 @@
     rp.hal.samplePixelCenter = opt->sample_pixel_center;
     rp.pixelXY = s->pixelXY.as<uint32_t>(); rp.pixelOffset = s->pixelOffset.as<uint64_t>(); rp.nPix = (uint32_t)n;
     rp.maxDepth = opt->max_depth; rp.rrThreshold = opt->rr_threshold;
-    rp.invSqrtSpp = 1 / std::sqrt((float)std::max(1, opt->spp)); rp.cullMis = 1; rp.speculate = 0;
+    rp.invSqrtSpp = 1 / std::sqrt((float)std::max(1, opt->spp)); rp.cullMis = 1; rp.speculate = rp.foldRepair = 0;
     EventTimer ev; BatchTimers bt; HprtRenderStats stats; memset(&stats, 0, sizeof(stats));
     rc = RunBatch(s, nullptr, rp, ps, qa, qb, bins, 0, (uint32_t)n, false, ev, &bt, &stats);
     if (rc != HPRT_OK) return rc;
diff --git a/thesis-pbrt-v3_amd/csrc/device/kernels.h b/thesis-pbrt-v3_amd/csrc/device/kernels.h
--- a/thesis-pbrt-v3_amd/csrc/device/kernels.h
+++ b/thesis-pbrt-v3_amd/csrc/device/kernels.h
@@ -27,17 +27,19 @@
     float4 *beta;
     float4 *L;
 };
+enum : uint32_t { RAY_DIM_MASK = 0xffffu, RAY_BOUNCE_SHIFT = 16u, RAY_BOUNCE_MASK = 0x3fffu, RAY_FOLD_MARK = 0x40000000u, RAY_SPECULAR = 0x80000000u };
 struct VertexStreams {
     RayStream shadow; uint8_t *occluded;
     RayStream mis; HitStream misHit;
     float4 *pendLight;
     float4 *pendMis;
     float4 *pendBeta;
+    const float4 *pendPrev;
 };
 enum : uint32_t { SPEC_RECORD = 0x80000000u, SPEC_END = 0x40000000u, SPEC_ID_MASK = 0x0fffffffu, SPEC_MAX_PATHS = 1u << 28 };
 struct QueueSet {
-    uint32_t *next, *shadow, *mis, *resolve;
-    uint32_t *nextCount, *shadowCount, *misCount, *resolveCount;
+    uint32_t *next, *shadow, *mis, *resolve, *end;
+    uint32_t *nextCount, *shadowCount, *misCount, *resolveCount, *endCount;
 };
 enum : uint32_t { BIN_STRIDE = 64u };
 struct BinSet { uint2 *q[5]; uint32_t *aux; uint32_t *count; uint2 *retry[2]; };
@@ -52,6 +54,7 @@
     float invSqrtSpp;
     int32_t cullMis;
     int32_t speculate;
+    int32_t foldRepair;
 };
 struct FilmGeom {
     int32_t cx0, cy0, cx1, cy1;
@@ -92,7 +95,7 @@
                     const IrregularSink *irr = nullptr);
 void LaunchBin(hipStream_t st, const DevScene &sc, const PathStream &in, const HitStream &hit, const uint32_t *queue,
                const uint32_t *countPtr, uint32_t countImm, uint32_t gridItems, int32_t maxDepth, int32_t bounces, const BinSet &bins,
-               float4 *Lfinal);
+               float4 *Lfinal, const VertexStreams &vs, bool foldRepair);
 void LaunchShade(hipStream_t st, int mode, const DevScene &sc, const RenderParams &rp, const PathStream &in, const HitStream &hit,
                  uint32_t gridItems, uint32_t s0, const PathStream &out, const VertexStreams &vs, const QueueSet &q,
                  const BinSet &bins, float4 *Lfinal, bool firstBounce, bool retryPass = false);
diff --git a/thesis-pbrt-v3_amd/csrc/device/kernels.hip b/thesis-pbrt-v3_amd/csrc/device/kernels.hip
--- a/thesis-pbrt-v3_amd/csrc/device/kernels.hip
+++ b/thesis-pbrt-v3_amd/csrc/device/kernels.hip
@@ -42,7 +42,7 @@
     return base + prefix;
 }
 
-struct BlockAppendLds { uint32_t waveCount[4][16]; uint32_t base[4]; };
+struct BlockAppendLds { uint32_t waveCount[5][16]; uint32_t base[5]; };
 template <int NQ>
 __device__ __forceinline__ void block_append(BlockAppendLds *lds, uint32_t *const counter[NQ], const bool pred[NQ], uint32_t pos[NQ]) {
     const uint32_t lane = __lane_id(), wave = threadIdx.x >> 6, nWaves = (blockDim.x + 63) >> 6;
@@ -873,7 +873,8 @@
 
 #define HPRT_BIN_ITEMS 4
 __global__ __launch_bounds__(1024) void k_bin(DevScene sc, PathStream in, HitStream hit, const uint32_t *queue, const uint32_t *countPtr,
-                                              uint32_t countImm, int32_t maxDepth, int32_t bounces, BinSet bins, float4 *Lfinal) {
+                                              uint32_t countImm, int32_t maxDepth, int32_t bounces, BinSet bins, float4 *Lfinal,
+                                              const uint8_t *occluded, const float4 *pendPrev) {
     __shared__ uint32_t waveCount[N_BINS][HPRT_BIN_ITEMS * 16];
     __shared__ uint32_t binBase[N_BINS];
     const uint32_t n = countPtr ? *countPtr : countImm;
@@ -912,7 +913,12 @@
                 else {
                     const float4 b4 = in.beta[slot[k]];
                     float4 L4 = in.L[slot[k]];
-                    if (word >= 0 && (__float_as_uint(in.ray.b[slot[k]].w) >> 31)) { L4.x += b4.x * 0.f; L4.y += b4.y * 0.f; L4.z += b4.z * 0.f; }
+                    const uint32_t st = (occluded || word >= 0) ? __float_as_uint(in.ray.b[slot[k]].w) : 0u;
+                    if (occluded && (st & RAY_FOLD_MARK) && occluded[slot[k]] != 0) {
+                        const float4 rec = pendPrev[slot[k]];
+                        L4.x = rec.x; L4.y = rec.y; L4.z = rec.z;
+                    }
+                    if (word >= 0 && (st >> 31)) { L4.x += b4.x * 0.f; L4.y += b4.y * 0.f; L4.z += b4.z * 0.f; }
                     Lfinal[__float_as_uint(b4.w)] = L4;
                 }
             }
@@ -955,6 +961,7 @@
 #ifndef HPRT_SHADE_WAVES_SUBSTRATE
 #define HPRT_SHADE_WAVES_SUBSTRATE 4
 #endif
+__device__ float4 kFreshPathL = {0.f, 0.f, 0.f, 1.f};
 template <int MODE, int BS, bool TEX = false, bool INSTS = false>
 __global__ __launch_bounds__(BS, MODE == 0 ? HPRT_SHADE_WAVES_MATTE : MODE == 1 ? HPRT_SHADE_WAVES_PLASTIC : MODE == 3 ? HPRT_SHADE_WAVES_SUBSTRATE : HPRT_SHADE_WAVES_GENERIC) void k_shade(DevScene sc, RenderParams rp, PathStream in, HitStream hit, uint32_t s0,
                                                PathStream out, VertexStreams vs, QueueSet q, BinSet bins, float4 *Lfinal, uint32_t firstBounce, uint32_t retryPass) {
@@ -973,9 +980,10 @@
     bool speculated = false;
     uint32_t slot = 0;
     uint32_t j = 0;
-    float4 rayA = make_float4(0.f, 0.f, 0.f, 0.f), rayB = rayA, hitA = rayA, beta4 = rayA, L4 = rayA, tv0 = rayA, tv1 = rayA, tv2 = rayA;
+    float4 rayA = make_float4(0.f, 0.f, 0.f, 0.f), rayB = rayA, hitA = rayA, beta4 = rayA, tv0 = rayA, tv1 = rayA, tv2 = rayA;
     float2 hitB = hit_no_aux();
     int32_t word = -1;
+    uint32_t occ = 0u;
     const bool oneLight = sc.nLights == 1u && !sc.spatial;
     DevLight light0 = {};
     if (oneLight) light0 = sc.lights[0];
@@ -995,14 +1003,18 @@
         hitA = hit_load(hit, slot); rayA = in.ray.a[slot]; rayB = in.ray.b[slot];
         if ((MODE == 2 || INSTS) && hit.b) hitB = hit_load_aux(hit, slot);
         beta4 = firstBounce ? make_float4(1.f, 1.f, 1.f, __uint_as_float(slot)) : in.beta[slot];
-        L4 = firstBounce ? make_float4(0.f, 0.f, 0.f, 1.f) : in.L[slot];
+        if (!firstBounce && rp.foldRepair) occ = vs.occluded[slot];
     }
     halton_lds_load(sc, &hl);
     if (i < n) {
         SP_MARK(6);
         const uint32_t st = __float_as_uint(rayB.w);
-        int dim = (int)(st & 0xffffu);
-        const int bounces = (int)((st >> 16) & 0x7fffu);
+        const bool dark = rp.foldRepair && (st & RAY_FOLD_MARK) && occ != 0u;
+        const float4 *const Lstored = firstBounce ? &kFreshPathL : in.L + slot;
+        const float *const Lrgb = reinterpret_cast<const float *>(dark ? vs.pendPrev + slot : Lstored);
+        const float4 L4 = make_float4(Lrgb[0], Lrgb[1], Lrgb[2], Lstored->w);
+        int dim = (int)(st & RAY_DIM_MASK);
+        const int bounces = (int)((st >> RAY_BOUNCE_SHIFT) & RAY_BOUNCE_MASK);
         const bool specularBounce = (st >> 31) != 0u;
         const uint32_t pathId = __float_as_uint(beta4.w);
         const uint32_t pix = pathId % rp.nPix, sIdx = pathId / rp.nPix;
@@ -1013,6 +1025,8 @@
         rgb beta(beta4.x, beta4.y, beta4.z);
         rgb L(L4.x, L4.y, L4.z), Ldark(0.f);
         float etaScale = L4.w;
+        bool zeroTerm = false;
+        auto added_zero_term = [&] { if (MODE != 2 && zeroTerm) { L = rgb(L.r + beta.r * 0.f, L.g + beta.g * 0.f, L.b + beta.b * 0.f); zeroTerm = false; } };
         const bool found = prim >= 0;
         DevSI si;
         DevTexGeom tg;
@@ -1059,7 +1073,7 @@
                 } else if (specularBounce) {
                     L = rgb(L.r + beta.r * 0.f, L.g + beta.g * 0.f, L.b + beta.b * 0.f);
                 }
-            } else if (MODE != 2 && specularBounce) L = rgb(L.r + beta.r * 0.f, L.g + beta.g * 0.f, L.b + beta.b * 0.f);
+            } else if (MODE != 2 && specularBounce) zeroTerm = true;
         }
         SP_MARK(0);
         if (MODE == 2 && !found && (bounces == 0 || specularBounce))
@@ -1167,6 +1181,7 @@
                             }
                         }
                     }
+                    added_zero_term();
                     if (rp.speculate && wantShadow && !wantMis) {
                         rgb LdLit(0.f);
                         LdLit = LdLit + pendLight;
@@ -1184,6 +1199,7 @@
                     }
                 }
             }
+            added_zero_term();
             if (!defer && !wantResolve && !speculated && bsdf_num(bsdf) > 0) L = rgb(L.r + beta.r * 0.f, L.g + beta.g * 0.f, L.b + beta.b * 0.f);
             SP_MARK(4);
             if (!defer) {
@@ -1211,13 +1227,14 @@
                 if (rp.cullMis && bounces + 1 >= rp.maxDepth && !(flags & BX_SPECULAR)) alive = false;
                 if (alive) {
                     out.ray.a[j] = make_float4(o.x, o.y, o.z, HPRT_INF);
-                    out.ray.b[j] = make_float4(wi.x, wi.y, wi.z, __uint_as_float((uint32_t)dim | ((uint32_t)(bounces + 1) << 16) | ((flags & BX_SPECULAR) ? 0x80000000u : 0u)));
+                    out.ray.b[j] = make_float4(wi.x, wi.y, wi.z, __uint_as_float((uint32_t)dim | ((uint32_t)(bounces + 1) << RAY_BOUNCE_SHIFT) | (speculated && rp.foldRepair ? RAY_FOLD_MARK : 0u) | ((flags & BX_SPECULAR) ? RAY_SPECULAR : 0u)));
                     out.beta[j] = make_float4(beta.r, beta.g, beta.b, beta4.w);
                     wantNext = true;
                 }
             }
             }
         }
+        added_zero_term();
         if (!defer) {
             if (speculated) vs.pendBeta[j] = make_float4(Ldark.r, Ldark.g, Ldark.b, __uint_as_float(pathId | SPEC_RECORD | (wantNext ? 0u : SPEC_END)));
             if (wantNext || wantResolve) out.L[j] = make_float4(L.r, L.g, L.b, wantNext ? etaScale : 0.f);
@@ -1243,14 +1260,16 @@
         const uint32_t pr = wave_append(bins.count + (6 + RETRY) * BIN_STRIDE, voxelMiss && !retryPass);
         if (voxelMiss && !retryPass) bins.retry[RETRY][pr] = make_uint2(slot, j);
     }
-    uint32_t *const ctr[4] = {q.nextCount, q.shadowCount, q.misCount, q.resolveCount};
-    const bool pred[4] = {wantNext, wantShadow, wantMis, wantResolve};
-    uint32_t pos[4];
-    block_append<4>(&al, ctr, pred, pos);
+    const bool wantEnd = speculated && !wantNext && rp.foldRepair;
+    uint32_t *const ctr[5] = {q.nextCount, q.shadowCount, q.misCount, q.resolveCount, q.endCount};
+    const bool pred[5] = {wantNext, wantShadow, wantMis, wantResolve, wantEnd};
+    uint32_t pos[5];
+    block_append<5>(&al, ctr, pred, pos);
     if (wantNext) q.next[pos[0]] = j;
     if (wantShadow) q.shadow[pos[1]] = j;
     if (wantMis) q.mis[pos[2]] = j;
     if (wantResolve) q.resolve[pos[3]] = j;
+    if (wantEnd) q.end[pos[4]] = j;
 }
 
 __global__ __launch_bounds__(256) void k_resolve(DevScene sc, VertexStreams vs, float4 *Lio, float4 *Lfinal, const uint32_t *queue,
@@ -1289,23 +1308,34 @@
     else Lfinal[__float_as_uint(pb.w)] = Lnew;
 }
 
+#define HPRT_REPAIR_ITEMS 4
 template <bool COUNT>
 __global__ __launch_bounds__(256) void k_repair(VertexStreams vs, float4 *Lio, float4 *Lfinal, const uint32_t *queue, uint32_t n, uint32_t *counts) {
-    const uint32_t i = blockIdx.x * blockDim.x + threadIdx.x;
-    if (i >= n) return;
-    const uint32_t j = queue[i];
-    const bool occluded = vs.occluded[j] != 0;
-    if (!COUNT && !occluded) return;
-    const float4 rec = vs.pendBeta[j];
-    const uint32_t w = __float_as_uint(rec.w);
-    if (!(w & SPEC_RECORD)) return;
-    if (COUNT) atomicAdd(counts, 1u);
-    if (!occluded) return;
-    if (COUNT) atomicAdd(counts + 1, 1u);
-    if (w & SPEC_END) Lfinal[w & SPEC_ID_MASK] = make_float4(rec.x, rec.y, rec.z, 0.f);
-    else {
-        float *const Lj = reinterpret_cast<float *>(Lio + j);
-        Lj[0] = rec.x; Lj[1] = rec.y; Lj[2] = rec.z;
+    const uint32_t first = blockIdx.x * (HPRT_REPAIR_ITEMS * 256u) + threadIdx.x;
+    uint32_t j[HPRT_REPAIR_ITEMS];
+    bool occluded[HPRT_REPAIR_ITEMS], want[HPRT_REPAIR_ITEMS];
+    float4 rec[HPRT_REPAIR_ITEMS];
+#pragma unroll
+    for (int k = 0; k < HPRT_REPAIR_ITEMS; ++k) { const uint32_t i = first + k * 256u; want[k] = i < n; j[k] = want[k] ? queue[i] : 0u; }
+#pragma unroll
+    for (int k = 0; k < HPRT_REPAIR_ITEMS; ++k) {
+        occluded[k] = want[k] && vs.occluded[j[k]] != 0;
+        if (!COUNT) want[k] = occluded[k];
+    }
+#pragma unroll
+    for (int k = 0; k < HPRT_REPAIR_ITEMS; ++k) rec[k] = want[k] ? vs.pendBeta[j[k]] : make_float4(0.f, 0.f, 0.f, 0.f);
+#pragma unroll
+    for (int k = 0; k < HPRT_REPAIR_ITEMS; ++k) {
+        const uint32_t w = __float_as_uint(rec[k].w);
+        if (!want[k] || !(w & SPEC_RECORD)) continue;
+        if (COUNT) atomicAdd(counts, 1u);
+        if (!occluded[k]) continue;
+        if (COUNT) atomicAdd(counts + 1, 1u);
+        if (w & SPEC_END) Lfinal[w & SPEC_ID_MASK] = make_float4(rec[k].x, rec[k].y, rec[k].z, 0.f);
+        else {
+            float *const Lj = reinterpret_cast<float *>(Lio + j[k]);
+            Lj[0] = rec[k].x; Lj[1] = rec[k].y; Lj[2] = rec[k].z;
+        }
     }
 }
 
@@ -1574,8 +1604,10 @@
 }
 void LaunchBin(hipStream_t st, const DevScene &sc, const PathStream &in, const HitStream &hit, const uint32_t *queue,
                const uint32_t *countPtr, uint32_t countImm, uint32_t gridItems, int32_t maxDepth, int32_t bounces, const BinSet &bins,
-               float4 *Lfinal) {
-    if (gridItems) hipLaunchKernelGGL(k_bin, dim3(blocks_for(gridItems, HPRT_BIN_ITEMS * 1024)), dim3(1024), 0, st, sc, in, hit, queue, countPtr, countImm, maxDepth, bounces, bins, Lfinal);
+               float4 *Lfinal, const VertexStreams &vs, bool foldRepair) {
+    const uint8_t *occluded = foldRepair ? vs.occluded : nullptr;
+    const float4 *pendPrev = foldRepair ? vs.pendPrev : nullptr;
+    if (gridItems) hipLaunchKernelGGL(k_bin, dim3(blocks_for(gridItems, HPRT_BIN_ITEMS * 1024)), dim3(1024), 0, st, sc, in, hit, queue, countPtr, countImm, maxDepth, bounces, bins, Lfinal, occluded, pendPrev);
 }
 void LaunchShade(hipStream_t st, int mode, const DevScene &sc, const RenderParams &rp, const PathStream &in, const HitStream &hit,
                  uint32_t gridItems, uint32_t s0, const PathStream &out, const VertexStreams &vs, const QueueSet &q,
@@ -1606,8 +1638,8 @@
 }
 void LaunchRepair(hipStream_t st, const VertexStreams &vs, float4 *L, float4 *Lfinal, const uint32_t *queue, uint32_t n, uint32_t *counts) {
     if (n == 0) return;
-    if (counts) hipLaunchKernelGGL(k_repair<true>, dim3(blocks_for(n, 256)), dim3(256), 0, st, vs, L, Lfinal, queue, n, counts);
-    else hipLaunchKernelGGL(k_repair<false>, dim3(blocks_for(n, 256)), dim3(256), 0, st, vs, L, Lfinal, queue, n, counts);
+    if (counts) hipLaunchKernelGGL(k_repair<true>, dim3(blocks_for(n, HPRT_REPAIR_ITEMS * 256)), dim3(256), 0, st, vs, L, Lfinal, queue, n, counts);
+    else hipLaunchKernelGGL(k_repair<false>, dim3(blocks_for(n, HPRT_REPAIR_ITEMS * 256)), dim3(256), 0, st, vs, L, Lfinal, queue, n, counts);
 }
 void LaunchStoreRadiance(hipStream_t st, const float4 *Lfinal, float *LallR, float *LallG, float *LallB, uint32_t nPix, uint32_t s0,
                          uint32_t nSlots) {
```

Result: faster. 6341 Mrays/s, median of 6 (+1.8%).
